# osmr/pytorchcv

Hardware: AMD Instinct MI355X
Metric: images/sec @224x224 (resnet50 bs=256/GPU) (higher is better)
Workload: dtype bf16; 1 GPU; resnet50_bs256; per_gpu_batch=256, global_batch=256, input=fp32 NCHW 224x224 resident in HBM, parallelism=batch-sharded replicas x1, launcher_choice=timed at capture on this GPU

## Files before the change

### include/pcv_amd.h

```cpp
#ifndef PCV_AMD_H
#define PCV_AMD_H

#include <stddef.h>
#include <stdint.h>

#ifdef __cplusplus
extern "C" {
#endif

#define PCV_ABI_VERSION 5

typedef struct pcv_ctx pcv_ctx;

typedef enum pcv_status {
    PCV_OK = 0,
    PCV_ERR_INVALID = -1,
    PCV_ERR_HIP = -2,
    PCV_ERR_NO_DEVICE = -3,
    PCV_ERR_TOO_LARGE = -4
} pcv_status;

typedef enum pcv_dtype { PCV_F32 = 0, PCV_BF16 = 1, PCV_F16 = 2 } pcv_dtype;

typedef enum pcv_act {
    PCV_ACT_NONE = 0, PCV_ACT_RELU = 1, PCV_ACT_RELU6 = 2, PCV_ACT_SIGMOID = 3,
    PCV_ACT_SWISH = 4, PCV_ACT_HSIGMOID = 5, PCV_ACT_HSWISH = 6, PCV_ACT_CLAMP01 = 7
} pcv_act;

typedef struct pcv_conv_desc {
    int32_t struct_size;
    int32_t N, H, W;
    int32_t Cin, Cout;
    int32_t kh, kw;
    int32_t stride_h, stride_w;
    int32_t pad_t, pad_l, pad_b, pad_r;
    int32_t dil_h, dil_w;
    int32_t groups;
    int32_t act;
    int32_t post_act;
    int32_t has_residual;
    int32_t dtype;
    int32_t out_dtype;
    int32_t x_cpitch;
    int32_t x_wpitch;
    int32_t y_cpitch;
} pcv_conv_desc;

int pcv_abi_version(void);
size_t pcv_conv_desc_size(void);
int pcv_create(pcv_ctx** out, int device);
int pcv_destroy(pcv_ctx* ctx);
const char* pcv_last_error(const pcv_ctx* ctx);
int pcv_set_tuning(pcv_ctx* ctx, const char* key, int value);

int pcv_fp16_guard_begin(pcv_ctx* ctx, unsigned* slot, void* stream);
int pcv_fp16_guard_end(pcv_ctx* ctx, const unsigned* slot, float* y, long count, void* stream);
int pcv_fp16_overflow_count(pcv_ctx* ctx, unsigned* count, void* stream);

int pcv_nchw_to_nhwc(pcv_ctx* ctx, const float* x, void* y, int N, int C, int H, int W,
                     int cpitch, int wpitch, int dtype, void* stream);
int pcv_nhwc_to_nchw(pcv_ctx* ctx, const void* x, float* y, int N, int C, int H, int W, int cpitch, int dtype,
                     void* stream);

int pcv_preprocess_u8(pcv_ctx* ctx, const unsigned char* x, void* y, int N, int Hs, int Ws, int C, int top, int left,
                      int H, int W, int wpitch, const float* mean, const float* inv_std, int dtype, void* stream);

int pcv_resize_plan_bytes(int N, const int* hs, const int* ws, int C, int size, int H, int W, size_t* bytes);
int pcv_resize_plan(const void* const* frames, int N, const int* hs, const int* ws, int C, int size, int H, int W, void* blob,
                    size_t bytes);
int pcv_resize_crop_u8(pcv_ctx* ctx, const void* plan_host, const void* plan_dev, size_t bytes, void* y, int wpitch,
                       const float* mean, const float* inv_std, int dtype, void* stream);

int pcv_classify_f32(pcv_ctx* ctx, const float* logits, int N, int J, int k,
                     int* top_idx, float* top_val, float* top_prob,
                     const long long* labels, int* rank, float* nll,
                     void* stream);

int pcv_conv_packed_bytes(const pcv_conv_desc* d, size_t* bytes);
int pcv_conv_pack(pcv_ctx* ctx, const pcv_conv_desc* d, const float* w, void* packed, void* stream);
int pcv_dwconv_packed_bytes(const pcv_conv_desc* d, size_t* bytes);
int pcv_dwconv_pack(pcv_ctx* ctx, const pcv_conv_desc* d, const float* w, void* packed, void* stream);
int pcv_bn_fold(pcv_ctx* ctx, int C, const float* gamma, const float* beta, const float* mean, const float* var,
                float eps, const float* conv_bias, float* scale, float* shift, void* stream);

int pcv_conv2d_fused(pcv_ctx* ctx, const pcv_conv_desc* d, const void* x, const void* packed,
                     const float* scale, const float* shift, const void* residual, void* y, void* stream);

int pcv_conv2d_gated_fused(pcv_ctx* ctx, const pcv_conv_desc* d, const void* x, const void* packed, const float* scale,
                           const float* shift, const float* gate, const void* residual, void* y, void* stream);
int pcv_fc_f32(pcv_ctx* ctx, const float* in, const float* w, const float* b, float* out, int N, int K, int J, int act,
               void* stream);
int pcv_conv2d_maxpool_supported(const pcv_conv_desc* d, int k, int s, int p, int ceil_mode);
int pcv_conv2d_maxpool_fused(pcv_ctx* ctx, const pcv_conv_desc* d, const void* x, const void* packed, const float* scale,
                             const float* shift, void* y, int k, int s, int p, int ceil_mode, void* stream);

int pcv_conv2d_nchw_stem_supported(const pcv_conv_desc* d, int pool);
int pcv_conv2d_nchw_stem_fused(pcv_ctx* ctx, const pcv_conv_desc* d, const float* x_nchw, const void* packed, const float* scale,
                               const float* shift, void* y, int pool, void* stream);
int pcv_dwconv2d_fused(pcv_ctx* ctx, const pcv_conv_desc* d, const void* x, const void* packed,
                       const float* scale, const float* shift, const void* residual, void* y, void* stream);
int pcv_mixconv_packed_bytes(const pcv_conv_desc* d, const int* kernels, int nk, size_t* bytes);
int pcv_mixconv_pack(pcv_ctx* ctx, const pcv_conv_desc* d, const int* kernels, int nk, const float* const* w, void* packed,
                     void* stream);
int pcv_mixconv2d_fused(pcv_ctx* ctx, const pcv_conv_desc* d, const int* kernels, int nk, const void* x, const void* packed,
                        const float* scale, const float* shift, void* y, void* stream);
int pcv_ghost_supported(const pcv_conv_desc* d);
int pcv_ghost_dw_fused(pcv_ctx* ctx, const pcv_conv_desc* d, const void* m, const void* packed, const float* scale,
                       const float* shift, const void* residual, void* y, void* stream);
int pcv_gconvx_supported(const pcv_conv_desc* d);
int pcv_maxpool2d(pcv_ctx* ctx, const void* x, void* y, int N, int H, int W, int C, int k, int s, int p,
                  int ceil_mode, int dtype, void* stream);
int pcv_channel_slice(pcv_ctx* ctx, const void* x, void* y, long rows, int C, int offset, int x_cpitch, int y_cpitch,
                      int dtype, void* stream);
int pcv_channel_interleave2(pcv_ctx* ctx, const void* a, const void* b, void* y, long rows, int Ch, int a_cpitch,
                            int b_cpitch, int y_cpitch, int dtype, void* stream);
int pcv_channel_concat(pcv_ctx* ctx, const void* x, void* y, long rows, int C, int x_cpitch, int y_cpitch, int y_offset,
                       int dtype, void* stream);
int pcv_interpolate(pcv_ctx* ctx, const void* x, void* y, int N, int H, int W, int C, int Ho, int Wo, int bilinear,
                    int align_corners, int dtype, void* stream);
int pcv_hr_fuse_supported(int nsrc, const int* shift, int N, int H, int W, int C, int act, int dtype);
int pcv_hr_fuse(pcv_ctx* ctx, const void* const* src, const int* shift, int nsrc, void* y, int N, int H, int W, int C, int act,
                int dtype, void* stream);
int pcv_avgpool2d(pcv_ctx* ctx, const void* x, void* y, int N, int H, int W, int C, int k, int s,
                  int dtype, int out_dtype, void* stream);
int pcv_global_avgpool(pcv_ctx* ctx, const void* x, void* y, int N, int HW, int C, int dtype, int out_dtype,
                       void* stream);
int pcv_gemm_bias(pcv_ctx* ctx, const void* x, const void* packed, const float* bias, void* y,
                  int N, int Cin, int Cout, int dtype, int out_dtype, void* stream);
int pcv_se_squeeze(pcv_ctx* ctx, const void* x, float* mean, int N, int HW, int C, int dtype, void* stream);
int pcv_se_excite(pcv_ctx* ctx, const float* mean, const float* w1, const float* b1, const float* w2,
                  const float* b2, float* mid, float* gate, int N, int C, int M, int mid_act, int out_act,
                  void* stream);
int pcv_se_scale(pcv_ctx* ctx, const void* x, const float* gate, const void* residual, void* y,
                 int N, int HW, int C, int post_act, int dtype, void* stream);

int pcv_splat_squeeze(pcv_ctx* ctx, const void* x, float* s, int N, int HW, int C, int radix, int dtype, void* stream);
int pcv_splat_excite(pcv_ctx* ctx, const float* s, const float* w1, const float* b1, const float* w2, const float* b2, float* mid,
                     float* logits, float* att, int N, int C, int M, int radix, int groups, void* stream);
int pcv_splat_combine(pcv_ctx* ctx, const void* x, const float* att, const void* residual, void* y, int N, int HW, int C, int radix,
                      int post_act, int dtype, void* stream);
int pcv_avgpool2d_pad(pcv_ctx* ctx, const void* x, void* y, int N, int H, int W, int C, int k, int s, int p, int ceil_mode,
                      int count_include_pad, int dtype, int out_dtype, void* stream);

int pcv_cbam_pool(pcv_ctx* ctx, const void* x, float* s, int N, int HW, int C, int dtype, void* stream);
int pcv_cbam_excite(pcv_ctx* ctx, const float* s, const float* w1, const float* b1, const float* w2, const float* b2, float* mid,
                    float* gate, int N, int C, int M, void* stream);
int pcv_cbam_spatial_pool(pcv_ctx* ctx, const void* x, const float* gate, float* p, int N, int HW, int C, int dtype, void* stream);
int pcv_cbam_apply(pcv_ctx* ctx, const void* x, const float* gate, const float* p, const float* w7, const float* scale,
                   const float* shift, const void* residual, void* y, int N, int H, int W, int C, int post_act, int dtype,
                   void* stream);

int pcv_conv1x1_pair_supported(const pcv_conv_desc* d1, const pcv_conv_desc* d2);
int pcv_conv1x1_pair_fused(pcv_ctx* ctx, const pcv_conv_desc* d1, const pcv_conv_desc* d2, const void* x,
                           const void* packed1, const float* scale1, const float* shift1, const void* residual, void* y1,
                           const void* packed2, const float* scale2, const float* shift2, void* y2, void* stream);

int pcv_conv1x1_pair_gated_supported(const pcv_conv_desc* d1, const pcv_conv_desc* d2);
int pcv_conv1x1_pair_gated_fused(pcv_ctx* ctx, const pcv_conv_desc* d1, const pcv_conv_desc* d2, const void* x,
                                 const void* packed1, const float* scale1, const float* shift1, const float* gate,
                                 const void* residual, void* y1, const void* packed2, const float* scale2, const float* shift2,
                                 void* y2, void* stream);

int pcv_conv1x1_pair_idconv_supported(const pcv_conv_desc* d_id, const pcv_conv_desc* d1, const pcv_conv_desc* d2);
int pcv_conv1x1_pair_idconv_fused(pcv_ctx* ctx, const pcv_conv_desc* d_id, const pcv_conv_desc* d1, const pcv_conv_desc* d2,
                                  const void* x0, const void* packed_id, const float* scale_id, const float* shift_id,
                                  const void* x, const void* packed1, const float* scale1, const float* shift1, void* y1,
                                  const void* packed2, const float* scale2, const float* shift2, void* y2, void* stream);

int pcv_bottleneck_supported(const pcv_conv_desc* d1, const pcv_conv_desc* d2, const pcv_conv_desc* d3, const pcv_conv_desc* d_id);
int pcv_bottleneck_fused(pcv_ctx* ctx, const pcv_conv_desc* d1, const pcv_conv_desc* d2, const pcv_conv_desc* d3,
                         const pcv_conv_desc* d_id, const void* x, const void* packed1, const float* scale1, const float* shift1,
                         const void* packed2, const float* scale2, const float* shift2, const void* packed3, const float* scale3,
                         const float* shift3, const void* packed_id, const float* scale_id, const float* shift_id, void* y,
                         void* stream);

int pcv_mbconv_supported(const pcv_conv_desc* d_exp, const pcv_conv_desc* d_dw, const pcv_conv_desc* d_proj);
int pcv_mbconv_fused(pcv_ctx* ctx, const pcv_conv_desc* d_exp, const pcv_conv_desc* d_dw, const pcv_conv_desc* d_proj,
                     const void* x, const void* packed_exp, const float* scale_e, const float* shift_e,
                     const void* packed_dw, const float* scale_d, const float* shift_d, const void* packed_proj,
                     const float* scale_p, const float* shift_p, const void* residual, void* y, void* stream);

int pcv_bn_act(pcv_ctx* ctx, const void* x, const float* scale, const float* shift, void* y, long rows, int C,
               int x_cpitch, int act, int dtype, void* stream);

int pcv_instnorm_workspace_bytes(int N, int Cn, size_t* bytes);
int pcv_instnorm_act(pcv_ctx* ctx, const void* x, const float* gamma, const float* beta, void* y, void* workspace, int N, int HW,
                     int C, int Cn, int x_cpitch, float eps, int act, int dtype, void* stream);

int pcv_rccl_available(void);
int pcv_rccl_broadcast(pcv_ctx* ctx, void* comm, void* const* bufs, const size_t* bytes, int count, int root, void* stream);
int pcv_rccl_allgather(pcv_ctx* ctx, void* comm, const void* send, void* recv, size_t bytes_per_rank, void* stream);

#ifdef __cplusplus
}
#endif
#endif
```

### pytorchcv_amd/_lib.py

```python

__all__ = ['lib', 'ctx_for', 'check', 'ConvDesc', 'LIB_PATH', 'PcvError', 'PCV_ERR_TOO_LARGE']

import os
import ctypes
import threading

LIB_PATH = os.path.join(os.path.dirname(os.path.abspath(__file__)), "csrc", "libpcv_amd.so")
PCV_ERR_TOO_LARGE = -4

_c = ctypes
_VP = ctypes.c_void_p
_I = ctypes.c_int


class PcvError(RuntimeError):
    def __init__(self, code, msg):
        super(PcvError, self).__init__("pcv_amd error {}: {}".format(code, msg))
        self.code = code


PCV_ABI_VERSION = 5


class ConvDesc(ctypes.Structure):
    _fields_ = [(n, ctypes.c_int32) for n in (
        "struct_size", "N", "H", "W", "Cin", "Cout", "kh", "kw", "stride_h", "stride_w", "pad_t", "pad_l", "pad_b", "pad_r",
        "dil_h", "dil_w", "groups", "act", "post_act", "has_residual", "dtype", "out_dtype", "x_cpitch", "x_wpitch",
        "y_cpitch")]


    def __init__(self, *args, **kw):
        super(ConvDesc, self).__init__(*args, **kw)
        self.struct_size = ctypes.sizeof(ConvDesc)


_SIGS = {
    "pcv_abi_version": (_I, []),
    "pcv_conv_desc_size": (ctypes.c_size_t, []),
    "pcv_create": (_I, [ctypes.POINTER(_VP), _I]),
    "pcv_destroy": (_I, [_VP]),
    "pcv_last_error": (ctypes.c_char_p, [_VP]),
    "pcv_set_tuning": (_I, [_VP, ctypes.c_char_p, _I]),
    "pcv_fp16_guard_begin": (_I, [_VP, _VP, _VP]),
    "pcv_fp16_guard_end": (_I, [_VP, _VP, _VP, ctypes.c_long, _VP]),
    "pcv_fp16_overflow_count": (_I, [_VP, ctypes.POINTER(ctypes.c_uint), _VP]),
    "pcv_rccl_available": (_I, []),
    "pcv_rccl_broadcast": (_I, [_VP, _VP, ctypes.POINTER(_VP), ctypes.POINTER(ctypes.c_size_t), _I, _I, _VP]),
    "pcv_rccl_allgather": (_I, [_VP, _VP, _VP, _VP, ctypes.c_size_t, _VP]),
    "pcv_nchw_to_nhwc": (_I, [_VP, _VP, _VP, _I, _I, _I, _I, _I, _I, _I, _VP]),
    "pcv_nhwc_to_nchw": (_I, [_VP, _VP, _VP, _I, _I, _I, _I, _I, _I, _VP]),
    "pcv_preprocess_u8": (_I, [_VP, _VP, _VP, _I, _I, _I, _I, _I, _I, _I, _I, _I, _VP, _VP, _I, _VP]),
    "pcv_resize_plan_bytes": (_I, [_I, ctypes.POINTER(_I), ctypes.POINTER(_I), _I, _I, _I, _I, ctypes.POINTER(ctypes.c_size_t)]),
    "pcv_resize_plan": (_I, [ctypes.POINTER(_VP), _I, ctypes.POINTER(_I), ctypes.POINTER(_I), _I, _I, _I, _I, _VP, ctypes.c_size_t]),
    "pcv_resize_crop_u8": (_I, [_VP, _VP, _VP, ctypes.c_size_t, _VP, _I, _VP, _VP, _I, _VP]),
    "pcv_classify_f32": (_I, [_VP, _VP, _I, _I, _I, _VP, _VP, _VP, _VP, _VP, _VP, _VP]),
    "pcv_conv_packed_bytes": (_I, [ctypes.POINTER(ConvDesc), ctypes.POINTER(ctypes.c_size_t)]),
    "pcv_conv_pack": (_I, [_VP, ctypes.POINTER(ConvDesc), _VP, _VP, _VP]),
    "pcv_dwconv_packed_bytes": (_I, [ctypes.POINTER(ConvDesc), ctypes.POINTER(ctypes.c_size_t)]),
    "pcv_dwconv_pack": (_I, [_VP, ctypes.POINTER(ConvDesc), _VP, _VP, _VP]),
    "pcv_bn_fold": (_I, [_VP, _I, _VP, _VP, _VP, _VP, ctypes.c_float, _VP, _VP, _VP, _VP]),
    "pcv_conv2d_fused": (_I, [_VP, ctypes.POINTER(ConvDesc), _VP, _VP, _VP, _VP, _VP, _VP, _VP]),
    "pcv_dwconv2d_fused": (_I, [_VP, ctypes.POINTER(ConvDesc), _VP, _VP, _VP, _VP, _VP, _VP, _VP]),
    "pcv_mixconv_packed_bytes": (_I, [ctypes.POINTER(ConvDesc), ctypes.POINTER(_I), _I, ctypes.POINTER(ctypes.c_size_t)]),
    "pcv_mixconv_pack": (_I, [_VP, ctypes.POINTER(ConvDesc), ctypes.POINTER(_I), _I, ctypes.POINTER(_VP), _VP, _VP]),
    "pcv_mixconv2d_fused": (_I, [_VP, ctypes.POINTER(ConvDesc), ctypes.POINTER(_I), _I, _VP, _VP, _VP, _VP, _VP, _VP]),
    "pcv_ghost_supported": (_I, [ctypes.POINTER(ConvDesc)]),
    "pcv_ghost_dw_fused": (_I, [_VP, ctypes.POINTER(ConvDesc), _VP, _VP, _VP, _VP, _VP, _VP, _VP]),
    "pcv_gconvx_supported": (_I, [ctypes.POINTER(ConvDesc)]),
    "pcv_hr_fuse_supported": (_I, [_I, ctypes.POINTER(_I), _I, _I, _I, _I, _I, _I]),
    "pcv_hr_fuse": (_I, [_VP, ctypes.POINTER(_VP), ctypes.POINTER(_I), _I, _VP, _I, _I, _I, _I, _I, _I, _VP]),
    "pcv_maxpool2d": (_I, [_VP, _VP, _VP, _I, _I, _I, _I, _I, _I, _I, _I, _I, _VP]),
    "pcv_channel_slice": (_I, [_VP, _VP, _VP, ctypes.c_long, _I, _I, _I, _I, _I, _VP]),
    "pcv_channel_interleave2": (_I, [_VP, _VP, _VP, _VP, ctypes.c_long, _I, _I, _I, _I, _I, _VP]),
    "pcv_channel_concat": (_I, [_VP, _VP, _VP, ctypes.c_long, _I, _I, _I, _I, _I, _VP]),
    "pcv_interpolate": (_I, [_VP, _VP, _VP, _I, _I, _I, _I, _I, _I, _I, _I, _I, _VP]),
    "pcv_avgpool2d": (_I, [_VP, _VP, _VP, _I, _I, _I, _I, _I, _I, _I, _I, _VP]),
    "pcv_global_avgpool": (_I, [_VP, _VP, _VP, _I, _I, _I, _I, _I, _VP]),
    "pcv_gemm_bias": (_I, [_VP, _VP, _VP, _VP, _VP, _I, _I, _I, _I, _I, _VP]),
    "pcv_se_squeeze": (_I, [_VP, _VP, _VP, _I, _I, _I, _I, _VP]),
    "pcv_se_excite": (_I, [_VP, _VP, _VP, _VP, _VP, _VP, _VP, _VP, _I, _I, _I, _I, _I, _VP]),
    "pcv_conv2d_gated_fused": (_I, [_VP, ctypes.POINTER(ConvDesc), _VP, _VP, _VP, _VP, _VP, _VP, _VP, _VP]),
    "pcv_fc_f32": (_I, [_VP, _VP, _VP, _VP, _VP, _I, _I, _I, _I, _VP]),
    "pcv_conv2d_maxpool_supported": (_I, [ctypes.POINTER(ConvDesc), _I, _I, _I, _I]),
    "pcv_conv2d_maxpool_fused": (_I, [_VP, ctypes.POINTER(ConvDesc), _VP, _VP, _VP, _VP, _VP, _I, _I, _I, _I, _VP]),
    "pcv_conv2d_nchw_stem_supported": (_I, [ctypes.POINTER(ConvDesc), _I]),
    "pcv_conv2d_nchw_stem_fused": (_I, [_VP, ctypes.POINTER(ConvDesc), _VP, _VP, _VP, _VP, _VP, _I, _VP]),
    "pcv_conv1x1_pair_supported": (_I, [ctypes.POINTER(ConvDesc), ctypes.POINTER(ConvDesc)]),
    "pcv_conv1x1_pair_fused": (_I, [_VP, ctypes.POINTER(ConvDesc), ctypes.POINTER(ConvDesc), _VP, _VP, _VP, _VP, _VP, _VP, _VP,
                                    _VP, _VP, _VP, _VP]),
    "pcv_conv1x1_pair_gated_supported": (_I, [ctypes.POINTER(ConvDesc), ctypes.POINTER(ConvDesc)]),
    "pcv_conv1x1_pair_gated_fused": (_I, [_VP, ctypes.POINTER(ConvDesc), ctypes.POINTER(ConvDesc), _VP, _VP, _VP, _VP, _VP, _VP, _VP,
                                          _VP, _VP, _VP, _VP, _VP]),
    "pcv_conv1x1_pair_idconv_supported": (_I, [ctypes.POINTER(ConvDesc), ctypes.POINTER(ConvDesc), ctypes.POINTER(ConvDesc)]),
    "pcv_conv1x1_pair_idconv_fused": (_I, [_VP, ctypes.POINTER(ConvDesc), ctypes.POINTER(ConvDesc), ctypes.POINTER(ConvDesc),
                                           _VP, _VP, _VP, _VP, _VP, _VP, _VP, _VP, _VP, _VP, _VP, _VP, _VP, _VP]),
    "pcv_bottleneck_supported": (_I, [ctypes.POINTER(ConvDesc), ctypes.POINTER(ConvDesc), ctypes.POINTER(ConvDesc), ctypes.POINTER(ConvDesc)]),
    "pcv_bottleneck_fused": (_I, [_VP, ctypes.POINTER(ConvDesc), ctypes.POINTER(ConvDesc), ctypes.POINTER(ConvDesc), ctypes.POINTER(ConvDesc),
                                  _VP, _VP, _VP, _VP, _VP, _VP, _VP, _VP, _VP, _VP, _VP, _VP, _VP, _VP, _VP]),
    "pcv_mbconv_supported": (_I, [ctypes.POINTER(ConvDesc), ctypes.POINTER(ConvDesc), ctypes.POINTER(ConvDesc)]),
    "pcv_mbconv_fused": (_I, [_VP, ctypes.POINTER(ConvDesc), ctypes.POINTER(ConvDesc), ctypes.POINTER(ConvDesc), _VP, _VP, _VP, _VP,
                              _VP, _VP, _VP, _VP, _VP, _VP, _VP, _VP, _VP]),
    "pcv_bn_act": (_I, [_VP, _VP, _VP, _VP, _VP, ctypes.c_long, _I, _I, _I, _I, _VP]),
    "pcv_instnorm_workspace_bytes": (_I, [_I, _I, ctypes.POINTER(ctypes.c_size_t)]),
    "pcv_instnorm_act": (_I, [_VP, _VP, _VP, _VP, _VP, _VP, _I, _I, _I, _I, _I, ctypes.c_float, _I, _I, _VP]),
    "pcv_se_scale": (_I, [_VP, _VP, _VP, _VP, _VP, _I, _I, _I, _I, _I, _VP]),
    "pcv_splat_squeeze": (_I, [_VP, _VP, _VP, _I, _I, _I, _I, _I, _VP]),
    "pcv_splat_excite": (_I, [_VP, _VP, _VP, _VP, _VP, _VP, _VP, _VP, _VP, _I, _I, _I, _I, _I, _VP]),
    "pcv_splat_combine": (_I, [_VP, _VP, _VP, _VP, _VP, _I, _I, _I, _I, _I, _I, _VP]),
    "pcv_avgpool2d_pad": (_I, [_VP, _VP, _VP, _I, _I, _I, _I, _I, _I, _I, _I, _I, _I, _I, _VP]),
    "pcv_cbam_pool": (_I, [_VP, _VP, _VP, _I, _I, _I, _I, _VP]),
    "pcv_cbam_excite": (_I, [_VP, _VP, _VP, _VP, _VP, _VP, _VP, _VP, _I, _I, _I, _VP]),
    "pcv_cbam_spatial_pool": (_I, [_VP, _VP, _VP, _VP, _I, _I, _I, _I, _VP]),
    "pcv_cbam_apply": (_I, [_VP, _VP, _VP, _VP, _VP, _VP, _VP, _VP, _VP, _I, _I, _I, _I, _I, _I, _VP]),
}

_lib = None
_ctxs = {}
_lock = threading.RLock()


def lib():
    global _lib
    if _lib is None:
        with _lock:
            if _lib is None:
                if not os.path.exists(LIB_PATH):
                    raise RuntimeError(
                        "pytorchcv_amd: HIP extension {} is missing - build it with `python -c 'import __graft_entry__ as g; "
                        "g.build()'` or `make -C pytorchcv_amd/csrc`. There is no CPU fallback.".format(LIB_PATH))
                L = ctypes.CDLL(LIB_PATH)
                for name, (res, args) in _SIGS.items():
                    fn = getattr(L, name)
                    fn.restype = res
                    fn.argtypes = args
                if L.pcv_abi_version() != PCV_ABI_VERSION or L.pcv_conv_desc_size() != ctypes.sizeof(ConvDesc):
                    raise RuntimeError("pytorchcv_amd: {} has ABI version {} / a {}-byte pcv_conv_desc, this binding expects "
                                       "version {} / {} bytes - rebuild the library".format(
                                           LIB_PATH, L.pcv_abi_version(), L.pcv_conv_desc_size(), PCV_ABI_VERSION,
                                           ctypes.sizeof(ConvDesc)))
                _lib = L
    return _lib


def exported_symbols():
    return sorted(_SIGS.keys())


def ctx_for(device_index: int):
    c = _ctxs.get(device_index)
    if c is None:
        with _lock:
            c = _ctxs.get(device_index)
            if c is None:
                L = lib()
                h = _VP()
                rc = L.pcv_create(ctypes.byref(h), int(device_index))
                if rc != 0:
                    raise PcvError(rc, (L.pcv_last_error(None) or b"").decode())
                c = h
                _ctxs[device_index] = c
    return c


def check(rc: int, ctx):
    if rc != 0:
        raise PcvError(rc, (lib().pcv_last_error(ctx) or b"").decode())
```

### pytorchcv_amd/csrc/conv_device.hpp

```cpp
#pragma once
#include "pcv_common.hpp"

struct D3Params {
    const void* x;
    const void* w;
    const void* res;
    void* y;
    const float* scale;
    const float* shift;
    uint32_t x_bytes, w_bytes, y_bytes, res_bytes;
    int M;
    int Cout, Ypitch;
    int H, W, Cin, HW;
    FastDiv div_hw, div_w;
    int nk;
    int slices;
    int Kpad;
    int act, post_act;
    int nChTiles, nTiles;
    uint32_t* dbg;
    int stride, Hin, Win;
    uint32_t* ovf;
    int tailN;
    int dbgflags;
};

#if defined(__HIP_DEVICE_COMPILE__)
struct D3Tiles {
    int tile0, tend, tstride, nMine;
};
__device__ __forceinline__ D3Tiles d3q_tiles(const D3Params& p) {
    D3Tiles t;
    const int perXcd = (p.nTiles + 7) >> 3;
    const int xcd = blockIdx.x & 7;
    t.tstride = gridDim.x >> 3;
    t.tile0 = xcd * perXcd + (int)(blockIdx.x >> 3);
    t.tend = min(p.nTiles, (xcd + 1) * perXcd);
    t.nMine = t.tile0 < t.tend ? (t.tend - t.tile0 + t.tstride - 1) / t.tstride : 0;
    return t;
}
__device__ __forceinline__ void d3q_sync() {
    __builtin_amdgcn_sched_barrier(0);
    __builtin_amdgcn_s_barrier();
    __builtin_amdgcn_sched_barrier(0);
}

struct EpiBounds {
    float alo, ahi, plo, phi, clo, chi;
};
__device__ __forceinline__ EpiBounds make_epi_bounds(int act, int post_act) {
    EpiBounds b;
    b.alo = (act == PCV_ACT_RELU || act == PCV_ACT_RELU6) ? 0.f : -INFINITY;
    b.ahi = act == PCV_ACT_RELU6 ? 6.f : INFINITY;
    b.plo = (post_act == PCV_ACT_RELU || post_act == PCV_ACT_RELU6) ? 0.f : -INFINITY;
    b.phi = post_act == PCV_ACT_RELU6 ? 6.f : INFINITY;
    b.clo = b.alo > b.plo ? b.alo : b.plo;
    b.chi = b.ahi < b.phi ? b.ahi : b.phi;
    return b;
}
__device__ __forceinline__ float clamp_nan(float v, float lo, float hi) {
    return __builtin_elementwise_minimum(__builtin_elementwise_maximum(v, lo), hi);
}
template <typename F> __device__ __forceinline__ void epi_dispatch(bool has_res, bool relu_only, F&& f) {
    if (has_res) { if (relu_only) f(std::true_type{}, std::true_type{}); else f(std::true_type{}, std::false_type{}); }
    else { if (relu_only) f(std::false_type{}, std::true_type{}); else f(std::false_type{}, std::false_type{}); }
}

template <int DT, bool HR, bool RO>
__device__ __forceinline__ uint32_t epi2(float v0, float v1, uint32_t skip, const EpiBounds& b, F16Guard<DT>& guard) {
    if constexpr (RO) {
        if constexpr (HR) {
            float lo, hi;
            unpack2<DT>(skip, lo, hi);
            v0 += lo;
            v1 += hi;
        }
        v0 = __builtin_elementwise_maximum(v0, 0.f);
        v1 = __builtin_elementwise_maximum(v1, 0.f);
    } else if constexpr (HR) {
        v0 = clamp_nan(v0, b.alo, b.ahi);
        v1 = clamp_nan(v1, b.alo, b.ahi);
        float lo, hi;
        unpack2<DT>(skip, lo, hi);
        v0 += lo;
        v1 += hi;
        v0 = clamp_nan(v0, b.plo, b.phi);
        v1 = clamp_nan(v1, b.plo, b.phi);
    } else {
        v0 = clamp_nan(v0, b.clo, b.chi);
        v1 = clamp_nan(v1, b.clo, b.chi);
    }
    guard.see2(v0, v1);
    return pack2<DT>(v0, v1);
}

__device__ __forceinline__ void load_bn8(const D3Params& p, int chl, f32x4& s0, f32x4& s1, f32x4& h0, f32x4& h1) {
    s0 = *reinterpret_cast<const f32x4*>(p.scale + chl); s1 = *reinterpret_cast<const f32x4*>(p.scale + chl + 4);
    h0 = *reinterpret_cast<const f32x4*>(p.shift + chl); h1 = *reinterpret_cast<const f32x4*>(p.shift + chl + 4);
}

template <int ROWS> __device__ __forceinline__ void d3r_tile_pos(const D3Params& p, int tilesPerImage, int t, int& chTile, int& n, int& y0) {
    chTile = t % p.nChTiles;
    const int pt = t / p.nChTiles;
    n = pt / tilesPerImage;
    y0 = (pt - n * tilesPerImage) * ROWS;
}
#endif
```

### pytorchcv_amd/csrc/p1r_16bit.hip

```cpp
#include "p1r_conv.hpp"
#define P1R_INST(CW, CIN)                                                   \
    template __global__ void p1r_kernel<PCV_BF16, CW, CIN>(const D3Params); \
    template __global__ void p1r_kernel<PCV_F16, CW, CIN>(const D3Params);
P1R_INST(64, 256)
P1R_INST(32, 512)
P1R_INST(32, 256)
```

### pytorchcv_amd/csrc/p1r_conv.hpp

```cpp
#pragma once
#include "conv_device.hpp"

template <int CW_, int CIN_>
struct P1RCfg {
    static constexpr int CW = CW_;
    static constexpr int CIN = CIN_;
    static constexpr int CWB = CW / 16;
    static constexpr int KH = CIN / 32;
    static constexpr int AREGS = CWB * KH * 4;
    static constexpr int NW = 8;
    static constexpr int THREADS = 64 * NW;
    static constexpr int CG = NW * CW;
    static constexpr int BM = CG;
    static constexpr int UNITB = 16 * CIN * 2;
    static constexpr int SLOT = 65536;
    static constexpr int TP = SLOT / UNITB;
    static constexpr int BP = 16 * TP;
    static constexpr int PPU = CIN / 32;
    static constexpr int NPW = 64 / NW;
    static constexpr int SSOFF = 2 * SLOT;
    static constexpr int LDS = SSOFF + 2 * CG * 4;
    static constexpr int NSTEP = TP * KH;
    static constexpr int NSTORE = TP * (CWB / 2);
    static constexpr bool RES = CW == 32;
    static_assert((CW == 64 && CIN == 256) || (CW == 32 && CIN == 512) || (CW == 32 && CIN == 256), "three configurations");
    static_assert(NSTEP == 64 && TP * PPU == 64 && PPU % NW == 0 && KH % NPW == 0, "tile geometry");
};

#if defined(__HIP_DEVICE_COMPILE__)
template <int DT, int CW, int CIN>
__device__ __forceinline__ void p1r_body(const D3Params& p, char* smem) {
    typedef P1RCfg<CW, CIN> G;
    typedef typename Mma<DT>::frag frag;
    typedef __attribute__((address_space(3))) char lds_char;
    typedef const __attribute__((address_space(3))) frag* lds_fptr;
    constexpr int KH = G::KH, CWB = G::CWB, TP = G::TP;
    const int lane = threadIdx.x & 63;
    const int wave = __builtin_amdgcn_readfirstlane(threadIdx.x >> 6);
    const int fr = lane & 15, fq = lane >> 4;
    const int lrow = lane >> 3;
    const uint32_t lds0 = (uint32_t)__builtin_amdgcn_readfirstlane((int)(uint32_t)(size_t)PCV_LDS(smem));
    const D3Tiles T = d3q_tiles(p);
    if (T.nMine == 0) return;
#ifdef P1R_CYCLES
    const uint64_t cstart__ = __builtin_amdgcn_s_memtime();
#endif

    const __amdgpu_buffer_rsrc_t wrsrc = buffer_rsrc(p.w, p.w_bytes);
    const __amdgpu_buffer_rsrc_t xrsrc = buffer_rsrc(p.x, p.x_bytes);
    const __amdgpu_buffer_rsrc_t yrsrc = buffer_rsrc(p.y, p.y_bytes);
    const bool has_res = p.res != nullptr;
    const __amdgpu_buffer_rsrc_t rrsrc = buffer_rsrc(p.res, has_res ? p.res_bytes : 0u);

    frag A[KH][CWB];
    const uint32_t ssaddr = lds0 + (uint32_t)(G::SSOFF + (wave * CW + 8 * fq) * 4);
    auto load_weights = [&](int cg) __attribute__((always_inline)) {
#pragma unroll
        for (int kh = 0; kh < KH; ++kh)
#pragma unroll
            for (int i = 0; i < CWB; ++i) {
                const uint32_t row = (uint32_t)(cg * G::CG + wave * CW + i * 16 + fr);
                const uint32_t off = (row * (uint32_t)p.Kpad + (uint32_t)((kh >> 1) * 64 + (fq + 4 * (kh & 1)) * 8)) * 2u;
                const u32x4 v = __builtin_amdgcn_raw_buffer_load_b128(wrsrc, off, 0, 0);
                A[kh][i] = __builtin_bit_cast(frag, v);
            }
        if (lane < CW) {
            const int ch = cg * G::CG + wave * CW + lane;
            const float sc = ch < p.Cout ? p.scale[ch] : 0.f, sh = ch < p.Cout ? p.shift[ch] : 0.f;
            *reinterpret_cast<__attribute__((address_space(3))) float*>((size_t)(lds0 + (uint32_t)(G::SSOFF + (wave * CW + lane) * 4))) = sc;
            *reinterpret_cast<__attribute__((address_space(3))) float*>((size_t)(lds0 + (uint32_t)(G::SSOFF + (G::CG + wave * CW + lane) * 4))) = sh;
        }
    };

    const uint32_t fbase = lds0 + (uint32_t)(fr * 128 + ((fq ^ (fr & 7)) << 4));

    const int half8 = wave & 1;
    const uint32_t lanesrc = (uint32_t)((((lane & 7) ^ lrow) << 4));
    int tileP0N = 0;
    bool moreN = false;
    bool pseudoN = false;
    uint32_t pixoff = 0x80000000u;
    auto unit_src = [&](int unit) __attribute__((always_inline)) {
        const int m = tileP0N + unit * 16 + half8 * 8 + lrow;
        uint32_t mi = (uint32_t)m;
        if (p.stride != 1) {
            const uint32_t n = fastdiv((uint32_t)m, p.div_hw);
            const uint32_t rem = (uint32_t)m - n * (uint32_t)p.HW;
            const uint32_t ho = fastdiv(rem, p.div_w);
            const uint32_t wo = rem - ho * (uint32_t)p.W;
            mi = (n * (uint32_t)p.Hin + ho * (uint32_t)p.stride) * (uint32_t)p.Win + wo * (uint32_t)p.stride;
        }
        pixoff = (moreN && m < p.M && !(pseudoN && unit > 0)) ? mi * (uint32_t)(G::CIN * 2) + lanesrc : 0x80000000u;
    };
    auto dma_piece = [&](auto Ic, int slot) __attribute__((always_inline)) {
        constexpr int I = decltype(Ic)::value;
        constexpr int unit = (G::NW * I) / G::PPU, in0 = (G::NW * I) % G::PPU;
        constexpr int sl0 = in0 / 2;
        if constexpr (in0 == 0) unit_src(unit);
        const int slice = (wave >> 1) + sl0;
        const uint32_t dst = lds0 + (uint32_t)(slot * G::SLOT + unit * G::UNITB + slice * 2048 + half8 * 1024);
        __builtin_amdgcn_raw_ptr_buffer_load_lds(xrsrc, (lds_char*)(size_t)dst, 16, pixoff, slice * 128, 0, 0);
    };

    constexpr int RD = 3, RING = 6, KEEP = RING - RD - 1, NSTEP = G::NSTEP;
    f32x4 cacc[2][CWB];
    frag bq[RING];
    uint32_t fs0 = 0, fs1 = 0;
    auto rd = [&](auto STc) __attribute__((always_inline)) {
        constexpr int st = decltype(STc)::value;
        constexpr int u = st / KH, kh = st - KH * u, s = kh >> 1, h = kh & 1;
        bq[st % RING] = *reinterpret_cast<lds_fptr>((size_t)(h ? fs1 : fs0) + (size_t)(u * G::UNITB + s * 2048));
    };
    const EpiBounds B = make_epi_bounds(p.act, p.post_act);
    constexpr int NRR = G::RES ? TP * (CWB / 2) : 1;
    u32x4 rrq[NRR];
    u32x4 opend;
    f32x4 scA, shA, scB, shB;
    typedef const __attribute__((address_space(3))) f32x4* lds_f4ptr;
    auto ss_read = [&](auto IPc, auto Hc) __attribute__((always_inline)) {
        constexpr int ip = decltype(IPc)::value, half = decltype(Hc)::value;
        const f32x4 a = *reinterpret_cast<lds_f4ptr>((size_t)ssaddr + (size_t)((ip * 32 + 4 * half) * 4));
        const f32x4 b = *reinterpret_cast<lds_f4ptr>((size_t)ssaddr + (size_t)((G::CG + ip * 32 + 4 * half) * 4));
        if constexpr (half == 0) { scA = a; shA = b; } else { scB = a; shB = b; }
        __builtin_amdgcn_sched_barrier(0);
    };
    auto epi_part = [&](auto Mc, auto Uc, auto Pc, F16Guard<DT>& guard) __attribute__((always_inline)) {
        constexpr int MODE = decltype(Mc)::value;
        constexpr bool HR = (MODE & 1) != 0, PRE = (MODE & 2) != 0, HI = (MODE & 4) != 0;
        constexpr int u = decltype(Uc)::value, P = decltype(Pc)::value;
        constexpr int ip = P >> 2, e = P & 3, half = e >> 1, k0 = 2 * (e & 1);
        const f32x4& scv = half == 0 ? scA : scB;
        const f32x4& shv = half == 0 ? shA : shB;
        const f32x4& c = cacc[u & 1][2 * ip + half];
        f32x2 v = (f32x2){c[k0], c[k0 + 1]} * (f32x2){scv[k0], scv[k0 + 1]} + (f32x2){shv[k0], shv[k0 + 1]};
        if constexpr (HR) {
            if constexpr (PRE) {
                v[0] = __builtin_elementwise_maximum(v[0], B.alo); v[1] = __builtin_elementwise_maximum(v[1], B.alo);
                if constexpr (HI) { v[0] = __builtin_elementwise_minimum(v[0], B.ahi); v[1] = __builtin_elementwise_minimum(v[1], B.ahi); }
            }
            float lo, hi;
            unpack2<DT>(rrq[(u * (CWB / 2) + ip) % NRR][e], lo, hi);
            v += (f32x2){lo, hi};
            v[0] = __builtin_elementwise_maximum(v[0], B.plo); v[1] = __builtin_elementwise_maximum(v[1], B.plo);
            if constexpr (HI) { v[0] = __builtin_elementwise_minimum(v[0], B.phi); v[1] = __builtin_elementwise_minimum(v[1], B.phi); }
        } else {
            v[0] = __builtin_elementwise_maximum(v[0], B.clo); v[1] = __builtin_elementwise_maximum(v[1], B.clo);
            if constexpr (HI) { v[0] = __builtin_elementwise_minimum(v[0], B.chi); v[1] = __builtin_elementwise_minimum(v[1], B.chi); }
        }
        guard.see2(v[0], v[1]);
        opend[e] = pack2<DT>(v[0], v[1]);
    };
    uint32_t yb[CWB / 2], rb[CWB / 2];
    auto epi_store = [&](int u, int ip) __attribute__((always_inline)) {
        __builtin_amdgcn_raw_buffer_store_b128(opend, yrsrc, yb[ip] + (uint32_t)(u * 32 * p.Ypitch), 0, 0);
    };
    auto tile_steps = [&](auto HRc, auto ONEc, int slot, int ch0, int mTile) __attribute__((always_inline)) {
        constexpr bool ONE = decltype(ONEc)::value;
        constexpr bool HR = (decltype(HRc)::value & 1) != 0;
        F16Guard<DT> guard;
#pragma unroll
        for (int ip = 0; ip < CWB / 2; ++ip) {
            const bool chok = ch0 + 32 * ip < p.Cout;
            yb[ip] = chok ? (uint32_t)(((mTile + fr) * p.Ypitch + ch0 + 32 * ip) * 2) : 0x80000000u;
            if constexpr (HR) rb[ip] = chok ? (uint32_t)(((mTile + fr) * p.Cout + ch0 + 32 * ip) * 2) : 0x80000000u;
        }
        if constexpr (HR) {
#pragma unroll
            for (int u = 0; u < (ONE ? 1 : TP); ++u)
#pragma unroll
                for (int ip = 0; ip < CWB / 2; ++ip) {
                    rrq[(u * (CWB / 2) + ip) % NRR] = __builtin_amdgcn_raw_buffer_load_b128(rrsrc, rb[ip] + (uint32_t)(u * 32 * p.Cout), 0, 0);
                }
        }
        rd(std::integral_constant<int, 0>{}); rd(std::integral_constant<int, 1>{}); rd(std::integral_constant<int, 2>{});
        static_assert(RD == 3, "the three reads above");
        auto step = [&](auto STc) __attribute__((always_inline)) {
            constexpr int st = decltype(STc)::value;
            constexpr int u = st / KH, kh = st - KH * u;
            if constexpr (st + RD < NSTEP) rd(std::integral_constant<int, st + RD>{});
            if constexpr (u == 0 && (kh % (KH / G::NPW)) == 0) dma_piece(std::integral_constant<int, kh / (KH / G::NPW)>{}, slot ^ 1);
#pragma unroll
            for (int i = 0; i < CWB; ++i) {
                if constexpr (kh == 0) cacc[u & 1][i] = Mma<DT>::run(A[0][i], bq[st % RING], (f32x4){0.f, 0.f, 0.f, 0.f});
                else cacc[u & 1][i] = Mma<DT>::run(A[kh][i], bq[st % RING], cacc[u & 1][i]);
            }
            if constexpr (st >= KEEP) asm volatile("" ::"v"(bq[(st - KEEP) % RING]), "v"(cacc[u & 1][CWB - 1]));
            if constexpr (u >= 1) {
                typedef std::integral_constant<int, u - 1> UP;
                typedef std::integral_constant<int, 0> I0;
                typedef std::integral_constant<int, 1> I1;
                auto part = [&](auto Pc) __attribute__((always_inline)) { epi_part(HRc, UP{}, Pc, guard); };
                typedef std::integral_constant<int, 2> I2; typedef std::integral_constant<int, 3> I3; typedef std::integral_constant<int, 4> I4;
                typedef std::integral_constant<int, 5> I5; typedef std::integral_constant<int, 6> I6; typedef std::integral_constant<int, 7> I7;
                if constexpr (CWB == 4 && KH == 8) {
                    if constexpr (kh == 0) { ss_read(I0{}, I0{}); ss_read(I0{}, I1{}); }
                    if constexpr (kh == 2) { part(I0{}); part(I1{}); ss_read(I1{}, I0{}); }
                    if constexpr (kh == 3) { part(I2{}); part(I3{}); ss_read(I1{}, I1{}); epi_store(u - 1, 0); }
                    if constexpr (kh == 5) { part(I4{}); part(I5{}); }
                    if constexpr (kh == 6) { part(I6{}); part(I7{}); }
                    if constexpr (kh == 7) epi_store(u - 1, 1);
                } else if constexpr (KH == 8) {
                    if constexpr (kh == 0) { ss_read(I0{}, I0{}); ss_read(I0{}, I1{}); }
                    if constexpr (kh == 2) part(I0{});
                    if constexpr (kh == 3) part(I1{});
                    if constexpr (kh == 5) part(I2{});
                    if constexpr (kh == 6) part(I3{});
                    if constexpr (kh == 7) epi_store(u - 1, 0);
                } else {
                    if constexpr (kh == 0) { ss_read(I0{}, I0{}); ss_read(I0{}, I1{}); }
                    if constexpr (kh == 3) part(I0{});
                    if constexpr (kh == 5) part(I1{});
                    if constexpr (kh == 8) part(I2{});
                    if constexpr (kh == 10) part(I3{});
                    if constexpr (kh == 12) epi_store(u - 1, 0);
                }
            }
        };
        auto run = [&](auto... Sc) __attribute__((always_inline)) { (step(Sc), ...); };
        auto eight = [&](auto Bc) __attribute__((always_inline)) {
            constexpr int B0 = decltype(Bc)::value * 8;
            run(std::integral_constant<int, B0>{}, std::integral_constant<int, B0 + 1>{}, std::integral_constant<int, B0 + 2>{},
                std::integral_constant<int, B0 + 3>{}, std::integral_constant<int, B0 + 4>{}, std::integral_constant<int, B0 + 5>{},
                std::integral_constant<int, B0 + 6>{}, std::integral_constant<int, B0 + 7>{});
        };
        auto last_epilogue = [&](auto ULc) __attribute__((always_inline)) {
            typedef decltype(ULc) UL;
            constexpr int ul = UL::value;
            ss_read(std::integral_constant<int, 0>{}, std::integral_constant<int, 0>{}); ss_read(std::integral_constant<int, 0>{}, std::integral_constant<int, 1>{});
            epi_part(HRc, UL{}, std::integral_constant<int, 0>{}, guard); epi_part(HRc, UL{}, std::integral_constant<int, 1>{}, guard);
            epi_part(HRc, UL{}, std::integral_constant<int, 2>{}, guard); epi_part(HRc, UL{}, std::integral_constant<int, 3>{}, guard);
            epi_store(ul, 0);
            if constexpr (CWB == 4) {
                ss_read(std::integral_constant<int, 1>{}, std::integral_constant<int, 0>{}); ss_read(std::integral_constant<int, 1>{}, std::integral_constant<int, 1>{});
                epi_part(HRc, UL{}, std::integral_constant<int, 4>{}, guard); epi_part(HRc, UL{}, std::integral_constant<int, 5>{}, guard);
                epi_part(HRc, UL{}, std::integral_constant<int, 6>{}, guard); epi_part(HRc, UL{}, std::integral_constant<int, 7>{}, guard);
                epi_store(ul, 1);
            }
        };
        eight(std::integral_constant<int, 0>{});
        if constexpr (KH == 16) eight(std::integral_constant<int, 1>{});
        if constexpr (ONE) last_epilogue(std::integral_constant<int, 0>{});
        else {
            if constexpr (KH == 8) eight(std::integral_constant<int, 1>{});
            eight(std::integral_constant<int, 2>{});
            eight(std::integral_constant<int, 3>{}); eight(std::integral_constant<int, 4>{}); eight(std::integral_constant<int, 5>{});
            eight(std::integral_constant<int, 6>{}); eight(std::integral_constant<int, 7>{});
            last_epilogue(std::integral_constant<int, TP - 1>{});
        }
        guard.commit(p.ovf);
    };

    int cg = T.tile0 % p.nChTiles;
    int tileP0 = (T.tile0 / p.nChTiles) * G::BP;
    tileP0N = tileP0; moreN = true;
    {
        auto all = [&](auto... Ic) __attribute__((always_inline)) { (dma_piece(Ic, 0), ...); };
        auto eight = [&](auto Bc) __attribute__((always_inline)) {
            constexpr int B0 = decltype(Bc)::value;
            all(std::integral_constant<int, B0>{}, std::integral_constant<int, B0 + 1>{}, std::integral_constant<int, B0 + 2>{},
                std::integral_constant<int, B0 + 3>{}, std::integral_constant<int, B0 + 4>{}, std::integral_constant<int, B0 + 5>{},
                std::integral_constant<int, B0 + 6>{}, std::integral_constant<int, B0 + 7>{});
        };
        eight(std::integral_constant<int, 0>{});
    }

    int tailP0 = -1;
    if (p.tailN > 0) {
        const int nCG = p.nChTiles, B = gridDim.x >> 3, j = blockIdx.x >> 3, xcd = blockIdx.x & 7;
        const int r = xcd * (B / nCG) + j / nCG, k = r / TP, u = r - k * TP;
        if (k < p.tailN / nCG) tailP0 = (p.nTiles / nCG + k) * G::BP + 16 * u;
    }
    bool pseudo = false;
    int slot = 0, t = T.tile0;
    while (t < T.tend) {
#ifdef P1R_CYCLES
        const uint64_t p0__ = __builtin_amdgcn_s_memtime();
#endif
        load_weights(cg);
#ifdef P1R_CYCLES
        const uint64_t p1__ = __builtin_amdgcn_s_memtime();
#endif
        __builtin_amdgcn_s_waitcnt(0x0070);
#ifdef P1R_CYCLES
        const uint64_t p2__ = __builtin_amdgcn_s_memtime();
#endif
        d3q_sync();
#ifdef P1R_CYCLES
        if (p.dbg != nullptr && t == T.tile0 && lane == 0 && wave == 0) {
            uint32_t* e = p.dbg + 256 * 8 * 4 + blockIdx.x * 32 + 30;
            e[0] = (uint32_t)(p0__ - cstart__) | ((uint32_t)(p1__ - p0__) << 16);
            e[1] = (uint32_t)(p2__ - p1__) | ((uint32_t)(__builtin_amdgcn_s_memtime() - p2__) << 16);
        }
#endif
        bool same;
        do {
            const int tn = t + T.tstride;
            moreN = tn < T.tend;
            int cgN = moreN ? tn % p.nChTiles : cg;
            tileP0N = moreN ? (tn / p.nChTiles) * G::BP : 0;
            pseudoN = !moreN && !pseudo && tailP0 >= 0;
            if (pseudoN) { moreN = true; cgN = cg; tileP0N = tailP0; }
            fs0 = fbase + (uint32_t)(slot * G::SLOT);
            fs1 = fs0 ^ 64u;
#ifdef P1R_CYCLES
            const bool stamp__ = p.dbg != nullptr;
            const int tl__ = (t - T.tile0) / T.tstride;
            uint64_t c0__ = 0, c1__ = 0, c2__ = 0;
            if (stamp__) c0__ = __builtin_amdgcn_s_memtime();
#endif
            {
                const int ch0 = cg * G::CG + wave * CW + 8 * fq;
                const bool hi = p.act == PCV_ACT_RELU6 || p.post_act == PCV_ACT_RELU6, pre = p.act != PCV_ACT_NONE;
                auto modes = [&](auto ONEc) __attribute__((always_inline)) {
                    if constexpr (G::RES) {
                        if (has_res) {
                            if (!hi && !pre) tile_steps(std::integral_constant<int, 1>{}, ONEc, slot, ch0, tileP0);
                            else tile_steps(std::integral_constant<int, 7>{}, ONEc, slot, ch0, tileP0);
                        } else if (!hi) tile_steps(std::integral_constant<int, 0>{}, ONEc, slot, ch0, tileP0);
                        else tile_steps(std::integral_constant<int, 4>{}, ONEc, slot, ch0, tileP0);
                    } else {
                        if (!hi) tile_steps(std::integral_constant<int, 0>{}, ONEc, slot, ch0, tileP0);
                        else tile_steps(std::integral_constant<int, 4>{}, ONEc, slot, ch0, tileP0);
                    }
                };
                if (pseudo) modes(std::true_type{});
                else modes(std::false_type{});
            }
#ifdef P1R_CYCLES
            if (stamp__) c1__ = __builtin_amdgcn_s_memtime();
#endif
            if constexpr (G::NSTORE == 16) asm volatile("s_waitcnt vmcnt(16)" ::: "memory");
            else if constexpr (G::NSTORE == 8) asm volatile("s_waitcnt vmcnt(8)" ::: "memory");
            else asm volatile("s_waitcnt vmcnt(4)" ::: "memory");
#ifdef P1R_CYCLES
            if (stamp__) c2__ = __builtin_amdgcn_s_memtime();
#endif
            d3q_sync();
#ifdef P1R_CYCLES
            if (stamp__ && lane == 0) {
                const uint64_t c3 = __builtin_amdgcn_s_memtime();
                if (tl__ == 2) {
                    uint32_t* d = p.dbg + (blockIdx.x * 8 + wave) * 4;
                    d[0] = (uint32_t)(c1__ - c0__); d[1] = (uint32_t)(c2__ - c1__); d[2] = (uint32_t)(c3 - c2__); d[3] = 1u;
                }
                if (wave == 0 && tl__ < 15) {
                    uint32_t* e = p.dbg + 256 * 8 * 4 + blockIdx.x * 32 + 2 * tl__;
                    e[0] = (uint32_t)(c0__ - cstart__); e[1] = (uint32_t)(c3 - c0__);
                }
            }
#endif
            same = moreN && cgN == cg;
            cg = cgN; tileP0 = tileP0N;
            pseudo = pseudoN;
            slot ^= 1;
            t = tn;
        } while (same);
    }
    asm volatile("s_waitcnt vmcnt(0)" ::: "memory");
}
#endif

template <int DT, int CW, int CIN>
__global__ __launch_bounds__((P1RCfg<CW, CIN>::THREADS), 1) void p1r_kernel(const D3Params p) {
#if defined(__HIP_DEVICE_COMPILE__)
    extern __shared__ __attribute__((aligned(16))) char smem[];
    p1r_body<DT, CW, CIN>(p, smem);
#endif
}
```

### pytorchcv_amd/csrc/pcv_api.hip

```cpp
#include <hip/hip_runtime.h>
#include <string>
#include <type_traits>
#include <vector>
#include <cstring>
#include <algorithm>
#include <cstdio>
#include <cstdlib>
#include <dlfcn.h>
#include "pcv_common.hpp"
#include "igemm_inst.hpp"
#include "d3q_inst.hpp"
#include "d3w_inst.hpp"
#include "d3c_conv.hpp"
#include "d3k_conv.hpp"
#include "d3i_conv.hpp"
#include "d1i_conv.hpp"
#include "p1r_conv.hpp"
#include "stem_conv.hpp"
#include "pair1x1.hpp"
#include "wpair1x1.hpp"
#include "bnu.hpp"
#include "gconv3x3.hpp"
#include "gconv3x3r.hpp"
#include "gconvx.hpp"
GCONVX_INSTANCES(GCONVX_DECLARE, PCV_BF16)
GCONVX_INSTANCES(GCONVX_DECLARE, PCV_F16)
#include "mbconv.hpp"
#include "mbw_inst.hpp"
#include "mbr_inst.hpp"
MBW_SHAPES(MBW_DECLARE, PCV_BF16)
MBW_SHAPES(MBW_DECLARE, PCV_F16)
MBW2_SHAPES(MBW2_DECLARE, PCV_BF16)
MBW2_SHAPES(MBW2_DECLARE, PCV_F16)
MBW3_SHAPES(MBW3_DECLARE, PCV_BF16)
MBW3_SHAPES(MBW3_DECLARE, PCV_F16)
MBR_SHAPES(MBR_DECLARE, PCV_BF16)
MBR_SHAPES(MBR_DECLARE, PCV_F16)
#include "dwconv.hpp"
#include "mixconv.hpp"
MIX_INSTANCES(MIX_DECLARE, PCV_F32)
MIX_INSTANCES(MIX_DECLARE, PCV_BF16)
MIX_INSTANCES(MIX_DECLARE, PCV_F16)
#include "ghost.hpp"
GHOST_INSTANCES(GHOST_DECLARE, PCV_F32)
GHOST_INSTANCES(GHOST_DECLARE, PCV_BF16)
GHOST_INSTANCES(GHOST_DECLARE, PCV_F16)
#include "aux_kernels.hpp"
#include "cbam_kernels.hpp"
#include "instnorm.hpp"
#include "hrfuse.hpp"
#include "resize_kernel.hpp"
#include "classify_kernel.hpp"
#include "head_gemm.hpp"


IGEMM_INSTANCES(IGEMM_DECLARE, PCV_BF16)
IGEMM_INSTANCES(IGEMM_DECLARE, PCV_F16)
IGEMM_INSTANCES_SAMETYPE(IGEMM_DECLARE, PCV_F32)
D3Q_SHAPES(D3Q_DECLARE, PCV_BF16)
D3Q_SHAPES(D3Q_DECLARE, PCV_F16)
D3Q1_SHAPES(D3Q1_DECLARE, PCV_BF16)
D3Q1_SHAPES(D3Q1_DECLARE, PCV_F16)
D3W_SHAPES(D3W_DECLARE, PCV_BF16)
D3W_SHAPES(D3W_DECLARE, PCV_F16)
D3WT_SHAPES(D3WT_DECLARE, PCV_BF16)
D3WT_SHAPES(D3WT_DECLARE, PCV_F16)
extern template __global__ void d3c_kernel<PCV_BF16>(const D3Params);
extern template __global__ void d3c_kernel<PCV_F16>(const D3Params);
extern template __global__ void d3k_kernel<PCV_BF16>(const D3Params);
extern template __global__ void d3k_kernel<PCV_F16>(const D3Params);
extern template __global__ void d3i_kernel<PCV_BF16, 256>(const D3Params);
extern template __global__ void d3i_kernel<PCV_F16, 256>(const D3Params);
extern template __global__ void d3i_kernel<PCV_BF16, 512>(const D3Params);
extern template __global__ void d3i_kernel<PCV_F16, 512>(const D3Params);
extern template __global__ void d1i_kernel<PCV_BF16, 1024>(const D3Params);
extern template __global__ void d1i_kernel<PCV_F16, 1024>(const D3Params);
extern template __global__ void d1i_kernel<PCV_BF16, 2048>(const D3Params);
extern template __global__ void d1i_kernel<PCV_F16, 2048>(const D3Params);
#define P1R_DECLARE(CW, CIN)                                                       \
    extern template __global__ void p1r_kernel<PCV_BF16, CW, CIN>(const D3Params); \
    extern template __global__ void p1r_kernel<PCV_F16, CW, CIN>(const D3Params);
P1R_DECLARE(64, 256)
P1R_DECLARE(32, 512)
P1R_DECLARE(32, 256)
#define BNU_DECLARE(DT)                                                          \
    extern template __global__ void bnu_kernel<DT, false>(const BnuParams);      \
    extern template __global__ void bnu_kernel<DT, true>(const BnuParams);
BNU_DECLARE(PCV_BF16)
BNU_DECLARE(PCV_F16)

enum TileCfg { TILE_C32 = 0, TILE_C64 = 1, TILE_C128 = 2, TILE_C256 = 3, TILE_C64S = 4, TILE_C128S = 5, TILE_COUNT = 6 };

struct pcv_ctx {
    int device = 0;
    std::string err;
    int num_cu = 256;
    int persist_mode = 1;
    int force_tile = -1;
    int use_wstat = 1;
    int use_mbr = 1;
    int use_mbr_xl = 1;
    int use_mbw = 1;
    int use_gconvr = 1;
    int use_gconvx = 1;
    int use_d1x1 = -1;
    int use_head = 1;
    int use_stem32 = 1;
    int use_d3x3 = -1;
    unsigned long long dbg_ptr = 0;
    int use_p1r = -1;
    int use_d3k = -1;
    int use_d3i = -1;
    int use_d1i = -1;
    int use_d3c = -1;
    int use_d3w = -1;
    int dbg_flags = 0;
    int dw_flags = 0;
    int dw_th = 0;
    int max_blocks = 0;
    int bnu_band = 0;
    int pair_pb = 2;
    int persist_max_nk = 4;
    uint32_t* ovf = nullptr;
    int igemm_bpc[3][2][TILE_COUNT][3] = {};
    int gconv_bpc[3] = {2, 2, 2};
    int gconvx_bpc[2] = {2, 2};
    int stem_bpc[2] = {1, 1};
    int pair_bpc[2] = {1, 1};
    int pair_idc_bpc = 1;
    int wpair_bpc[4] = {1, 1, 1, 1};
};

static thread_local std::string g_create_err;

static int fail(pcv_ctx* ctx, int code, const std::string& msg) {
    if (ctx) ctx->err = msg; else g_create_err = msg;
    return code;
}
#define HIP_TRY(ctx, expr)                                                                          \
    do {                                                                                            \
        hipError_t e__ = (expr);                                                                    \
        if (e__ != hipSuccess)                                                                      \
            return fail(ctx, PCV_ERR_HIP, std::string(#expr) + ": " + hipGetErrorString(e__));      \
    } while (0)

struct DeviceGuard {
    int prev = -1;
    bool switched = false;
    explicit DeviceGuard(int want) {
        if (hipGetDevice(&prev) == hipSuccess && prev != want) switched = hipSetDevice(want) == hipSuccess;
    }
    ~DeviceGuard() {
        if (switched) (void)hipSetDevice(prev);
    }
};

#define PCV_ENTER(ctx)                       \
    if (!(ctx)) return PCV_ERR_INVALID;      \
    DeviceGuard device_guard((ctx)->device)
static int launched(pcv_ctx* ctx) {
    HIP_TRY(ctx, hipGetLastError());
    return PCV_OK;
}

static inline int round_up(int v, int m) { return (v + m - 1) / m * m; }
static inline long long cap_blocks(const pcv_ctx* ctx, long long blocks) {
    return (ctx->max_blocks > 0 && blocks > ctx->max_blocks) ? ctx->max_blocks : blocks;
}
static inline long long block_slots(const pcv_ctx* ctx, int per_cu) { return cap_blocks(ctx, (long long)ctx->num_cu * per_cu); }
static inline int esize(int dt) { return dt == PCV_F32 ? 4 : 2; }
static inline bool dtype_ok(int dt) { return dt == PCV_F32 || dt == PCV_BF16 || dt == PCV_F16; }
static inline bool aligned16(const void* p) { return (reinterpret_cast<uintptr_t>(p) & 15u) == 0; }
static inline bool in_window(unsigned long long bytes) { return bytes < 0x80000000ull; }
static int too_large(pcv_ctx* ctx, const char* fn, const char* what) {
    return fail(ctx, PCV_ERR_TOO_LARGE, std::string(fn) + ": " + what + " exceeds the 2 GiB window of one launch; split the batch");
}
static const char* const kTensorTooLarge = "tensor exceeds the 2 GiB window";
static int flat_grid(pcv_ctx* ctx, const char* fn, long long total, unsigned* grid, int per_block = 256) {
    const long long blocks = (total + per_block - 1) / per_block;
    if (total < 0 || blocks > 0x7fffffffll) return too_large(ctx, fn, "the grid");
    *grid = (unsigned)blocks;
    return PCV_OK;
}
static int stream_grid(pcv_ctx* ctx, const char* fn, long long total, unsigned* grid) {
    if (int rc = flat_grid(ctx, fn, total, grid)) return rc;
    *grid = (unsigned)cap_blocks(ctx, *grid);
    return PCV_OK;
}
template <int V> using dtype_tag = std::integral_constant<int, V>;
#define DT_OF(tag) decltype(tag)::value
template <class F> static void for_dtype(int dt, F&& f) {
    if (dt == PCV_BF16) f(dtype_tag<PCV_BF16>{});
    else if (dt == PCV_F16) f(dtype_tag<PCV_F16>{});
    else f(dtype_tag<PCV_F32>{});
}
template <class F> static void for_dtype16(int dt, F&& f) {
    if (dt == PCV_BF16) f(dtype_tag<PCV_BF16>{});
    else f(dtype_tag<PCV_F16>{});
}
template <class F> static void for_dtype_out(int dt, int ot, F&& f) {
    for_dtype(dt, [&](auto T) {
        if (ot == PCV_F32) f(T, dtype_tag<PCV_F32>{});
        else f(T, T);
    });
}

struct Kernel { const void* fn; int threads, lds, BM, BP; };
template <class F> static Kernel kernel_of(F* fn, int threads, int lds, int BM = 0, int BP = 0) {
    return Kernel{reinterpret_cast<const void*>(fn), threads, lds, BM, BP};
}
template <class Params> static int launch(pcv_ctx* ctx, const Kernel& k, unsigned grid, hipStream_t stream, Params& q) {
    void* args[] = {&q};
    HIP_TRY(ctx, hipLaunchKernel(k.fn, dim3(grid), dim3((unsigned)k.threads), args, (size_t)k.lds, stream));
    return PCV_OK;
}
static int blocks_per_cu(pcv_ctx* ctx, const Kernel& k, int* nb) {
    HIP_TRY(ctx, hipOccupancyMaxActiveBlocksPerMultiprocessor(nb, k.fn, k.threads, k.lds));
    if (*nb < 1) *nb = 1;
    return PCV_OK;
}

struct ConvPlan {
    bool stem = false;
    bool conv3 = false;
    int ES = 2, CE = 8;
    bool pair = false;
    int Ho = 0, Wo = 0;
    int ngb = 1;
    int Cg_in = 0, Cg_out = 0;
    int cin_blk = 0, cout_blk = 0;
    int nR = 1, nQ = 1;
    int dy[IGEMM_MAX_TAPS], dx[IGEMM_MAX_TAPS];
    int nchunks = 0, nk = 0, Kpad = 0;
    int wrows = 0;
// ... 178 lines not shown
                                P.ksrc[(size_t)j * P.CE + e] = (uint32_t)c | ((uint32_t)(r * d.kw + q) << 16);
                        }
                        put(cc * P.CE, r, q, P.dy[r], P.dx[q]);
                    }
        }
        while (j < P.nk * 8) put(0, 15, 0, 0, 0);
    }
    return nullptr;
}

struct TileInfo { int BM, BP, threads, lds; };
static const TileInfo kTiles[TILE_COUNT] = {
    {32, 256, 256, 2 * (32 + 256) * 128},
    {64, 256, 256, 2 * (64 + 256) * 128},
    {128, 128, 256, 2 * (128 + 128) * 128},
    {256, 64, 256, 2 * (256 + 64) * 128},
    {64, 128, 256, 2 * (64 + 128) * 128},
    {128, 64, 256, 2 * (128 + 64) * 128},
};
typedef void (*igemm_fn)(const IgemmParams);

template <int DT, int KHW> static igemm_fn igemm_for_tile(int tile) {
    switch (tile) {
        case TILE_C32: return igemm_conv_kernel<DT, DT, 2, 4, 1, 4, false, KHW>;
        case TILE_C64: return igemm_conv_kernel<DT, DT, 4, 4, 1, 4, false, KHW>;
        case TILE_C128: return igemm_conv_kernel<DT, DT, 4, 4, 2, 2, false, KHW>;
        case TILE_C256: return igemm_conv_kernel<DT, DT, 4, 4, 4, 1, false, KHW>;
        case TILE_C64S: if constexpr (KHW == 1) return igemm_conv_kernel<DT, DT, 4, 2, 1, 4, false, 1>; else return nullptr;
        case TILE_C128S: if constexpr (KHW == 1) return igemm_conv_kernel<DT, DT, 4, 2, 2, 2, false, 1>; else return nullptr;
        default: return nullptr;
    }
}
template <int DT> static igemm_fn igemm_for_taps(int tile, int khw) {
    if (khw == 1) return igemm_for_tile<DT, 1>(tile);
    if (khw == 9) return igemm_for_tile<DT, 9>(tile);
    return igemm_for_tile<DT, 0>(tile);
}
static igemm_fn igemm_fn_for(int dt, int ot, bool ragged, int tile, int khw) {
    if (!ragged && ot == dt) {
        if (dt == PCV_BF16) return igemm_for_taps<PCV_BF16>(tile, khw);
        if (dt == PCV_F16) return igemm_for_taps<PCV_F16>(tile, khw);
        return igemm_for_taps<PCV_F32>(tile, khw);
    }
    if (tile != TILE_C128) return nullptr;
    if (ot == PCV_F32) {
        if (dt == PCV_BF16) return igemm_conv_kernel<PCV_BF16, PCV_F32, 4, 4, 2, 2, true, 0>;
        if (dt == PCV_F16) return igemm_conv_kernel<PCV_F16, PCV_F32, 4, 4, 2, 2, true, 0>;
        return igemm_conv_kernel<PCV_F32, PCV_F32, 4, 4, 2, 2, true, 0>;
    }
    if (dt == PCV_BF16) return igemm_conv_kernel<PCV_BF16, PCV_BF16, 4, 4, 2, 2, true, 0>;
    if (dt == PCV_F16) return igemm_conv_kernel<PCV_F16, PCV_F16, 4, 4, 2, 2, true, 0>;
    return nullptr;
}

static Kernel igemm_kernel(int dt, int ot, bool ragged, int tile, int khw) {
    const TileInfo& T = kTiles[tile];
    return kernel_of(igemm_fn_for(dt, ot, ragged, tile, khw), T.threads, T.lds, T.BM, T.BP);
}
static inline int khw_slot(int khw) { return khw == 1 ? 1 : (khw == 9 ? 2 : 0); }

static inline int gconv_slot(int W) { return W + 1 <= 16 ? 0 : (W + 1 <= 32 ? 1 : 2); }
static Kernel gconv_kernel(int dt, int slot) {
    const bool bf = dt == PCV_BF16;
    if (slot == 0) return kernel_of(bf ? gconv3x3_kernel<PCV_BF16, 16> : gconv3x3_kernel<PCV_F16, 16>, 256, GConvCfg<16>::LDS);
    if (slot == 1) return kernel_of(bf ? gconv3x3_kernel<PCV_BF16, 32> : gconv3x3_kernel<PCV_F16, 32>, 256, GConvCfg<32>::LDS);
    return kernel_of(bf ? gconv3x3_kernel<PCV_BF16, 64> : gconv3x3_kernel<PCV_F16, 64>, 256, GConvCfg<64>::LDS);
}
static const int kGconvRMaxLds = 160 * 1024;
static Kernel gconvr_kernel(int dt, int stride, int kt, int lds = kGconvRMaxLds) {
    const bool bf = dt == PCV_BF16;
    if (stride == 2) {
        if (kt == 9) return kernel_of(bf ? gconv3x3r_kernel<PCV_BF16, 2, 9> : gconv3x3r_kernel<PCV_F16, 2, 9>, 256, lds);
        return kernel_of(bf ? gconv3x3r_kernel<PCV_BF16, 2, 5> : gconv3x3r_kernel<PCV_F16, 2, 5>, 256, lds);
    }
    return kernel_of(bf ? gconv3x3r_kernel<PCV_BF16, 1, 9> : gconv3x3r_kernel<PCV_F16, 1, 9>, 256, lds);
}
struct GConvRPlan { int R, XH, xl, win; };
static bool plan_gconvr(int stride, int H, int W, int Ho, int Wo, GConvRPlan& g) {
    if (stride == 2 && ((H | W) & 1)) return false;
    if (Wo > 64 || Ho <= 0) return false;
    for (int R = 64 / Wo; R >= 1; --R) {
        const int win = stride == 2 ? (2 * R + 1) * W + 2 : (R + 2) * W + 2;
        const int XH = stride == 2 ? ((win + 1) / 2 + 7) / 8 * 8 : 0;
        const int rows = ((stride == 2 ? 2 * XH : win) + 31) / 32 * 32;
        const int lds = 2 * rows * 128;
        if (lds * 2 <= kGconvRMaxLds || (R == 1 && lds <= kGconvRMaxLds)) {
            g.R = R; g.XH = XH; g.xl = rows / 32; g.win = win;
            return true;
        }
    }
    return false;
}
#define GCONVX_KROW(DT, S, PB)                                                                                               \
    {kernel_of(gconvx_kernel<DT, S, 8, PB>, 256, kGConvXMaxLds), kernel_of(gconvx_kernel<DT, S, 16, PB>, 256, kGConvXMaxLds),  \
     kernel_of(gconvx_kernel<DT, S, 24, PB>, 256, kGConvXMaxLds), kernel_of(gconvx_kernel<DT, S, 40, PB>, 256, kGConvXMaxLds), \
     kernel_of(gconvx_kernel<DT, S, 48, PB>, 256, kGConvXMaxLds), kernel_of(gconvx_kernel<DT, S, 56, PB>, 256, kGConvXMaxLds), \
     kernel_of(gconvx_kernel<DT, S, 64, PB>, 256, kGConvXMaxLds)}
#define GCONVX_KTYPE(DT) {{GCONVX_KROW(DT, 1, 4), GCONVX_KROW(DT, 1, 7)}, {GCONVX_KROW(DT, 2, 4), GCONVX_KROW(DT, 2, 7)}}
static const Kernel kGConvX[2][2][2][7] = {GCONVX_KTYPE(PCV_BF16), GCONVX_KTYPE(PCV_F16)};
struct GConvXPlan { int R, GB, pbi, win, pitch, lds; };
static bool plan_gconvx(int stride, int H, int W, int Ho, int Wo, int groups, int Cg, GConvXPlan& g) {
    if (stride == 2 && ((H | W) & 1)) return false;
    if (W > 112 || Ho <= 0 || Wo <= 0) return false;
    const int cpg = Cg / 8, sl = (Cg + 15) / 16;
    const int min_gb = std::min(groups, (4 + sl - 1) / sl);
    const int want_gb = std::min(groups, std::max(min_gb, 128 / Cg));
    for (int R = 16 * kGConvXPB[1] / Wo; R >= 1; --R) {
        const int win = stride == 2 ? (2 * R + 1) * W + 2 : (R + 2) * W + 2;
        int p16 = kGConvXMaxLds / (16 * win);
        if (p16 % 2 == 0) --p16;
        const int fit_gb = p16 / cpg;
        if (fit_gb < (R == 1 ? 1 : min_gb)) continue;
        int gb = std::min(want_gb, fit_gb);
        const int ncb = (groups + gb - 1) / gb;
        gb = (groups + ncb - 1) / ncb;
        g.R = R; g.GB = gb; g.pbi = R * Wo <= 16 * kGConvXPB[0] ? 0 : 1; g.win = win;
        g.pitch = 16 * ((gb * cpg) | 1);
        g.lds = win * g.pitch;
        return true;
    }
    return false;
}
template <class Cfg, class F> static Kernel tile_kernel(F* fn, int threads) { return kernel_of(fn, threads, Cfg::LDS, Cfg::BM, Cfg::BP); }
#define D3Q_ROW(DT, WC, WP, CBW, PBW, KS)                                                                   \
    {tile_kernel<D3Cfg<WC, WP, CBW, PBW, KS>>(d3q_kernel<PCV_BF16, WC, WP, CBW, PBW, KS>, 768),             \
     tile_kernel<D3Cfg<WC, WP, CBW, PBW, KS>>(d3q_kernel<PCV_F16, WC, WP, CBW, PBW, KS>, 768)},
static const Kernel kD3[][2] = {D3Q_SHAPES(D3Q_ROW, 0)};
static const int kD3Count = (int)(sizeof(kD3) / sizeof(kD3[0]));
#define D3Q1_ROW(DT, WC, WP, CBW, PBW, KS)                                                                  \
    {tile_kernel<D3Cfg<WC, WP, CBW, PBW, KS, true>>(d3q_kernel<PCV_BF16, WC, WP, CBW, PBW, KS, true>, 768), \
     tile_kernel<D3Cfg<WC, WP, CBW, PBW, KS, true>>(d3q_kernel<PCV_F16, WC, WP, CBW, PBW, KS, true>, 768)},
static const Kernel kD1[][2] = {D3Q1_SHAPES(D3Q1_ROW, 0)};
static const int kD1Count = (int)(sizeof(kD1) / sizeof(kD1[0]));
#define D3W_ROW(DT, WC, WP, CBW, PBW, KS, NSA)                                                              \
    {tile_kernel<D3WCfg<WC, WP, CBW, PBW, KS, NSA>>(d3w_kernel<PCV_BF16, WC, WP, CBW, PBW, KS, NSA>, 512),  \
     tile_kernel<D3WCfg<WC, WP, CBW, PBW, KS, NSA>>(d3w_kernel<PCV_F16, WC, WP, CBW, PBW, KS, NSA>, 512)},
#define D3WT_ROW(DT, WC, WP, CBW, PBW, KS, NSA, TRIM)                                                                   \
    {tile_kernel<D3WCfg<WC, WP, CBW, PBW, KS, NSA, TRIM>>(d3w_kernel<PCV_BF16, WC, WP, CBW, PBW, KS, NSA, TRIM>, 512),  \
     tile_kernel<D3WCfg<WC, WP, CBW, PBW, KS, NSA, TRIM>>(d3w_kernel<PCV_F16, WC, WP, CBW, PBW, KS, NSA, TRIM>, 512)},
static const Kernel kD3W[][2] = {D3W_SHAPES(D3W_ROW, 0) D3WT_SHAPES(D3WT_ROW, 0)};
static const int kD3WCount = (int)(sizeof(kD3W) / sizeof(kD3W[0]));
static const Kernel kD3C[1][2] = {{tile_kernel<D3CCfg>(d3c_kernel<PCV_BF16>, 256), tile_kernel<D3CCfg>(d3c_kernel<PCV_F16>, 256)}};
static const Kernel kD3K[1][2] = {{tile_kernel<D3KCfg>(d3k_kernel<PCV_BF16>, 256), tile_kernel<D3KCfg>(d3k_kernel<PCV_F16>, 256)}};
#define D3I_ROW(CIN)                                                                              \
    {kernel_of(d3i_kernel<PCV_BF16, CIN>, D3ICfg::THREADS, D3ICfgT<CIN>::LDS, D3ICfg::BM),        \
     kernel_of(d3i_kernel<PCV_F16, CIN>, D3ICfg::THREADS, D3ICfgT<CIN>::LDS, D3ICfg::BM)}
static const Kernel kD3I[2][2] = {D3I_ROW(256), D3I_ROW(512)};
static const Kernel kD1I[2][2] = {
    {tile_kernel<D1ICfgT<1024>>(d1i_kernel<PCV_BF16, 1024>, 256), tile_kernel<D1ICfgT<1024>>(d1i_kernel<PCV_F16, 1024>, 256)},
    {tile_kernel<D1ICfgT<1024>>(d1i_kernel<PCV_BF16, 2048>, 256), tile_kernel<D1ICfgT<1024>>(d1i_kernel<PCV_F16, 2048>, 256)}};
#define P1R_ROW(CW, CIN) \
    {tile_kernel<P1RCfg<CW, CIN>>(p1r_kernel<PCV_BF16, CW, CIN>, 512), tile_kernel<P1RCfg<CW, CIN>>(p1r_kernel<PCV_F16, CW, CIN>, 512)}
static const Kernel kP1R[3][2] = {P1R_ROW(64, 256), P1R_ROW(32, 512), P1R_ROW(32, 256)};
static const struct { const Kernel (*rows)[2]; int n; } kD3Tables[] = {{kD3, kD3Count}, {kD1, kD1Count}, {kD3W, kD3WCount}, {kD3C, 1},
                                                                       {kD3K, 1},       {kD3I, 2},       {kD1I, 2},         {kP1R, 3}};
static int pick_d1x1(long long M, int Cout, int Cin, long long slots) {
    if (Cin < 256 || Cout < 128) return -1;
    const int shape = Cout % 256 == 0 ? 1 : 0;
    const long long tiles = (long long)((Cout + kD1[shape][0].BM - 1) / kD1[shape][0].BM) * ((M + kD1[shape][0].BP - 1) / kD1[shape][0].BP);
    return tiles * 2 >= slots ? shape : -1;
}
static int pick_d3x3(long long M, int Cout, int nk, long long slots) {
    (void)nk;
    const int wide = Cout <= 64 ? 2 : 1, narrow = Cout <= 64 ? 5 : 4;
    auto tiles = [&](int i) { return ((Cout + kD3[i][0].BM - 1) / kD3[i][0].BM) * ((M + kD3[i][0].BP - 1) / kD3[i][0].BP); };
    if (Cout % 256 == 0 && tiles(0) * 2 >= slots) return 0;
    if (tiles(wide) * 2 >= slots) return wide;
    if (tiles(narrow) * 4 >= slots) return narrow;
    return -1;
}
static int pick_d3w(long long M, int Cout, long long slots) {
    const int shape = Cout % 256 == 0 ? 1 : (Cout % 128 == 0 ? 2 : -1);
    if (shape < 0) return -1;
    const long long tiles = (long long)(Cout / kD3W[shape][0].BM) * ((M + kD3W[shape][0].BP - 1) / kD3W[shape][0].BP);
    return tiles * 4 >= slots * 3 ? shape : -1;
}

static const int kStemLds = 7 * 64 * 64 + 2 * 768 * 16 + 3 * 2 * 64 * 16;
enum StemForm { STEM_PLAIN = 0, STEM_POOLED = 1, STEM_NARROW = 2 };
#define STEM_ROWS(DT)                                                                                                          \
    {{kernel_of(stem_conv_kernel<DT, false>, 256, kStemLds), kernel_of(stem_conv_kernel<DT, true>, 256, kStemLds),             \
      kernel_of(stem_conv_kernel<DT, false, false, 2>, 256, kStemLds)},                                                        \
     {kernel_of(stem_conv_kernel<DT, false, true>, 256, kStemLds + kStemStageBytes),                                           \
      kernel_of(stem_conv_kernel<DT, true, true>, 256, kStemLds + kStemStageBytes),                                            \
      kernel_of(stem_conv_kernel<DT, false, true, 2>, 256, kStemLds + kStemStageBytes)}}
static const Kernel kStem[2][2][3] = {STEM_ROWS(PCV_BF16), STEM_ROWS(PCV_F16)};

static int pair_lds(int pb, bool idc = false) { return (idc ? 6 : 3) * 16 * pb * 64 * 2 + 16 * 1024 * pb + (idc ? 4096 : 0); }
enum PairForm { PAIR_PB4 = 0, PAIR_PB2 = 1, PAIR_GATED = 2, PAIR_IDCONV = 3 };
#define PAIR_ROW(DT)                                                                                                          \
    {kernel_of(pair1x1_kernel<DT, 4>, 256, pair_lds(4)), kernel_of(pair1x1_kernel<DT, 2>, 256, pair_lds(2)),                  \
     kernel_of(pair1x1_kernel<DT, 2, false, true>, 256, pair_lds(2)), kernel_of(pair1x1_kernel<DT, 2, true>, 256, pair_lds(2, true))}
static const Kernel kPair[2][4] = {PAIR_ROW(PCV_BF16), PAIR_ROW(PCV_F16)};
#define BNU_ROW(DT) {kernel_of(bnu_kernel<DT, false>, 512, BnuCfg<false>::LDS), kernel_of(bnu_kernel<DT, true>, 512, BnuCfg<true>::LDS)}
static const Kernel kBnu[2][2] = {BNU_ROW(PCV_BF16), BNU_ROW(PCV_F16)};
static int g_bnu = -1;
static int g_wpair_mask = 3;
static int g_mbw_wide = 1;
struct WPairLaunch { Kernel k; int tileP; bool gate_in_lds; };
template <int CM, int C1> static WPairLaunch wpair_launch_for(int dt, bool gated) {
    typedef WPairCfg<CM, C1> G;
    const bool bf = dt == PCV_BF16;
    const int lds = gated ? G::LDS_GATED : G::LDS;
    const Kernel k = gated ? kernel_of(bf ? wpair1x1_kernel<PCV_BF16, CM, C1, true> : wpair1x1_kernel<PCV_F16, CM, C1, true>, 64 * G::NW, lds)
                           : kernel_of(bf ? wpair1x1_kernel<PCV_BF16, CM, C1, false> : wpair1x1_kernel<PCV_F16, CM, C1, false>, 64 * G::NW, lds);
    return WPairLaunch{k, G::P, gated && G::GATE_LDS};
}
static WPairLaunch wpair_launch(int cfg, int dt, bool gated = false) {
    switch (cfg) {
        case 0: return wpair_launch_for<128, 512>(dt, gated);
        case 1: return wpair_launch_for<256, 1024>(dt, gated);
        case 2: return wpair_launch_for<128, 256>(dt, gated);
        default: return wpair_launch_for<256, 512>(dt, gated);
    }
}
static int wpair_cfg(int cm, int c1) {
    if (cm == 128 && c1 == 512) return 0;
    if (cm == 256 && c1 == 1024) return 1;
    if (cm == 128 && c1 == 256) return 2;
    if (cm == 256 && c1 == 512) return 3;
    return -1;
}
static bool plain_1x1(const pcv_conv_desc& d) {
    return d.kh == 1 && d.kw == 1 && d.stride_h == 1 && d.stride_w == 1 && d.pad_t == 0 && d.pad_l == 0 && d.pad_b == 0 &&
           d.pad_r == 0 && d.groups == 1 && d.dil_h == 1 && d.dil_w == 1 && d.out_dtype == d.dtype &&
           (d.x_cpitch == 0 || d.x_cpitch == d.Cin) && (d.x_wpitch == 0 || d.x_wpitch == d.W) &&
           (d.y_cpitch == 0 || d.y_cpitch == d.Cout);
}
static const char* pair_unsupported(const pcv_conv_desc& a, const pcv_conv_desc& b) {
    if (desc_stale(a) || desc_stale(b)) return kStaleDesc;
    if (!plain_1x1(a) || !plain_1x1(b)) return "both convolutions must be plain 1x1 stride 1";
    if (a.dtype != b.dtype || (a.dtype != PCV_BF16 && a.dtype != PCV_F16)) return "16-bit storage only";
    if (a.N != b.N || a.H != b.H || a.W != b.W || a.Cout != b.Cin) return "shapes do not chain";
    const bool narrow = a.Cin == 64 && a.Cout == 256 && b.Cout == 64;
    const bool wide = ((a.Cin == 128 && (g_wpair_mask & 1)) || (a.Cin == 256 && (g_wpair_mask & 2))) &&
                      wpair_cfg(a.Cin, a.Cout) >= 0 && b.Cout == a.Cin;
    if (!narrow && !wide) return "only 64 -> 256 -> 64, 128 -> 512|256 -> 128 and 256 -> 1024|512 -> 256 are instantiated";
    if (!a.has_residual || b.has_residual || b.post_act != PCV_ACT_NONE) return "first conv must carry the residual, second must not";
    if ((long)a.N * a.H * a.W * a.Cout * 2 >= (1L << 31)) return kTensorTooLarge;
    return nullptr;
}

typedef void (*mbconv_fn)(const MbParams);
template <int DT> static mbconv_fn mbconv_for(int stride, bool expand) {
    if (stride == 1) return expand ? mbconv_kernel<DT, 1, true> : mbconv_kernel<DT, 1, false>;
    return expand ? mbconv_kernel<DT, 2, true> : mbconv_kernel<DT, 2, false>;
}
static const int kMbMaxLds = 150 * 1024, kMbwMaxLds = 160 * 1024;
static Kernel mbconv_kernel(int dt, int stride, bool expand, int lds = kMbMaxLds) {
    return kernel_of(dt == PCV_BF16 ? mbconv_for<PCV_BF16>(stride, expand) : mbconv_for<PCV_F16>(stride, expand), 256, lds);
}
struct MbwEntry { int dt, s, nrt, act, tw, ka, rb; mbconv_fn fn; };
#define MBW_ROW(DT, S, NRT, ACT, TW) {DT, S, NRT, ACT, TW, 1, 0, mbw_kernel<DT, S, NRT, ACT, TW>},
#define MBW2_ROW(DT, S, NRT, ACT, TW, KA) {DT, S, NRT, ACT, TW, KA, 0, mbw_kernel<DT, S, NRT, ACT, TW, KA>},
#define MBW3_ROW(DT, S, NRT, ACT, TW, KA, RB) {DT, S, NRT, ACT, TW, KA, RB, mbw_kernel<DT, S, NRT, ACT, TW, KA, RB>},
static const MbwEntry kMbw[] = {MBW_SHAPES(MBW_ROW, PCV_BF16) MBW_SHAPES(MBW_ROW, PCV_F16) MBW2_SHAPES(MBW2_ROW, PCV_BF16)
                                MBW2_SHAPES(MBW2_ROW, PCV_F16) MBW3_SHAPES(MBW3_ROW, PCV_BF16) MBW3_SHAPES(MBW3_ROW, PCV_F16)};
static const MbwEntry* pick_mbw(int dt, int stride, int nrt, int act, int tw, int ka, int rb) {
    if (act != PCV_ACT_RELU && act != PCV_ACT_RELU6) act = -1;
    for (const MbwEntry& e : kMbw)
        if (e.dt == dt && e.s == stride && e.nrt == nrt && e.act == act && e.tw == tw && e.ka == ka && e.rb == rb) return &e;
    return nullptr;
}
static Kernel mbw_kernel_of(const MbwEntry& e, int waves = 8, int lds = kMbwMaxLds) { return kernel_of(e.fn, 64 * waves, lds); }
struct MbrEntry { int dt, nrt, act, ro, s, ka; bool afl; int waves; bool wel, xl; mbconv_fn fn; };
#define MBR_ROW(DT, NRT, ACT, RO, S, KA, AFL, WV, WEL, XL) {DT, NRT, ACT, RO, S, KA, AFL, WV, WEL, XL, mbr_kernel<DT, NRT, ACT, RO, S, KA, AFL, WV, WEL, XL>},
static int mbr_entry_lds(const MbrEntry& e, int nChunks) {
    const int nr = e.s == 1 ? e.ro + 2 : 2 * e.ro + 1;
    return mbr_lds_layout(e.nrt, nChunks, e.ka, e.afl, e.wel, e.xl ? nr : 0, e.waves).total;
}
static const MbrEntry kMbr[] = {MBR_SHAPES(MBR_ROW, PCV_BF16) MBR_SHAPES(MBR_ROW, PCV_F16)};
static Kernel mbr_kernel_of(const MbrEntry& e, int lds = kMbwMaxLds) { return kernel_of(e.fn, 64 * e.waves, lds); }
static const MbrEntry* pick_mbr(const pcv_ctx* ctx, int dt, int nrt, int act, int stride, int ka, int nChunks) {
    if (act != PCV_ACT_RELU && act != PCV_ACT_RELU6) return nullptr;
    for (const MbrEntry& e : kMbr)
        if (e.dt == dt && e.nrt == nrt && e.act == act && e.s == stride && e.ka == ka &&
            mbr_entry_lds(e, nChunks) <= kMbwMaxLds && (!e.xl || ctx->use_mbr_xl))
            return &e;
    return nullptr;
}
static int mbw_waves(int stride, int nrt, int nChunks, int tw, int ka, int rb) {
    for (int nw = 8; nw >= 4; nw -= 2)
        if (mbw_lds_layout(stride, nrt, nChunks, nw, tw, ka, rb).total <= kMbwMaxLds) return nw;
    return 0;
}
static MbLds mbconv_plan(int stride, bool expand, int ka, int nChunks, int nRowT, int* nbufX) {
    MbLds two = mb_lds_layout(stride, expand, ka, nChunks, nRowT, 2);
    if (!expand || two.total <= 80 * 1024) { *nbufX = 2; return two; }
    MbLds one = mb_lds_layout(stride, expand, ka, nChunks, nRowT, 1);
    if (one.total <= 80 * 1024 || two.total > kMbMaxLds) { *nbufX = 1; return one; }
    *nbufX = 2;
    return two;
}

static int dt_index(int dtype) { return dtype == PCV_F32 ? 0 : (dtype == PCV_BF16 ? 1 : 2); }

#define DW_TYPE(DT)                                                                                                            \
    {{kernel_of(dwconv_kernel<DT, 3, 1, false>, 256, 0), kernel_of(dwconv_kernel<DT, 3, 1, true>, 256, 0)},                    \
     {kernel_of(dwconv_kernel<DT, 3, 2, false>, 256, 0), kernel_of(dwconv_kernel<DT, 3, 2, true>, 256, 0)},                    \
     {kernel_of(dwconv5_kernel<DT, 1, false>, 256, 0), kernel_of(dwconv5_kernel<DT, 1, true>, 256, 0)},                        \
     {kernel_of(dwconv5_kernel<DT, 2, false>, 256, 0), kernel_of(dwconv5_kernel<DT, 2, true>, 256, 0)}}
static const Kernel kDw[3][4][2] = {DW_TYPE(PCV_F32), DW_TYPE(PCV_BF16), DW_TYPE(PCV_F16)};

#define MIX_KERNEL(DT, S, FAST, G) kernel_of(mixdw_kernel<DT, S, FAST, G>, 256, 0)
#define MIX_ROW(DT, S, FAST) {MIX_KERNEL(DT, S, FAST, 2), MIX_KERNEL(DT, S, FAST, 3), MIX_KERNEL(DT, S, FAST, 4), MIX_KERNEL(DT, S, FAST, 5)}
#define MIX_TYPE(DT) {{MIX_ROW(DT, 1, false), MIX_ROW(DT, 1, true)}, {MIX_ROW(DT, 2, false), MIX_ROW(DT, 2, true)}}
static const Kernel kMix[3][2][2][4] = {MIX_TYPE(PCV_F32), MIX_TYPE(PCV_BF16), MIX_TYPE(PCV_F16)};

// ... 47 lines not shown
        for (int s = 0; s < 2; ++s)
            for (int pbi = 0; pbi < 2; ++pbi)
                for (int wi = 0; wi < 7; ++wi) on(kGConvX[t][s][pbi][wi], (t == 1 && s == 0 && wi == 6) ? &ctx->gconvx_bpc[pbi] : nullptr);
    for (int t = 0; t < 2; ++t)
        for (int nchw = 0; nchw < 2; ++nchw)
            for (int form = 0; form < 3; ++form) on(kStem[t][nchw][form], (nchw == 0 && form == STEM_PLAIN) ? &ctx->stem_bpc[t] : nullptr);
    for (int form = 0; form < 4; ++form) {
        on(kPair[0][form]);
        on(kPair[1][form], form == PAIR_GATED ? nullptr : form == PAIR_IDCONV ? &ctx->pair_idc_bpc : &ctx->pair_bpc[form]);
    }
    for (int t = 0; t < 2; ++t)
        for (int form = 0; form < 2; ++form) on(kBnu[t][form]);
    for (int cfg = 0; cfg < 4; ++cfg)
        for (int gated = 0; gated < 2; ++gated) {
            on(wpair_launch(cfg, PCV_BF16, gated != 0).k);
            on(wpair_launch(cfg, PCV_F16, gated != 0).k, gated ? nullptr : &ctx->wpair_bpc[cfg]);
        }
    for (int dt = PCV_BF16; dt <= PCV_F16; ++dt)
        for (int s = 1; s <= 2; ++s)
            for (int e = 0; e < 2; ++e) on(mbconv_kernel(dt, s, e != 0));
    for (const MbwEntry& e : kMbw) on(mbw_kernel_of(e));
    for (const MbrEntry& e : kMbr) on(mbr_kernel_of(e));
    on(classify_kernel_of(1024));
    on(classify_kernel_of(kClassifyMaxJ));
    return rc;
}
static bool mbw_shape(int Cin, int Cout, int stride, int H, int W, int* ka_out, int* nrt_out, int* rb_out = nullptr) {
    const int ka = (Cin + 31) / 32, nrt = Cout <= 32 ? 2 : (Cout <= 64 ? 4 : 6);
    if (ka_out) *ka_out = ka;
    if (nrt_out) *nrt_out = nrt;
    if (rb_out) *rb_out = nrt == 6 ? 2 : 0;
    if (H > 250 || W > 250 || Cout > 96) return false;
    if (nrt == 6) return g_mbw_wide != 0 && stride == 1 && (ka == 2 || ka == 3);
    return ka == 1 || (ka == 2 && stride == 1 && nrt == 4);
}
static const char* mbconv_unsupported(const pcv_conv_desc* de, const pcv_conv_desc& dd, const pcv_conv_desc& dp) {
    if ((de && desc_stale(*de)) || desc_stale(dd) || desc_stale(dp)) return kStaleDesc;
    if (dd.dtype != PCV_BF16 && dd.dtype != PCV_F16) return "16-bit storage only";
    if (dd.kh != 3 || dd.kw != 3 || dd.dil_h != 1 || dd.dil_w != 1 || dd.pad_t != 1 || dd.pad_l != 1 || dd.pad_b != 1 ||
        dd.pad_r != 1 || dd.stride_h != dd.stride_w || (dd.stride_h != 1 && dd.stride_h != 2) || dd.groups != dd.Cin ||
        dd.Cin != dd.Cout || dd.has_residual || dd.out_dtype != dd.dtype || (dd.x_cpitch != 0 && dd.x_cpitch != dd.Cin) ||
        (dd.x_wpitch != 0 && dd.x_wpitch != dd.W))
        return "depthwise stage must be 3x3, pad 1, stride 1 or 2, no residual";
    const int Cmid = dd.Cin;
    if (Cmid % 8 != 0) return "expanded channels must be a multiple of 8";
    if (!plain_1x1(dp) || dp.dtype != dd.dtype || dp.Cin != Cmid || dp.Cout % 8 != 0 || dp.Cout > 96) return "project stage must be a plain 1x1 with at most 96 channels";
    const bool wave_tiles = de && mbw_shape(de->Cin, dp.Cout, dd.stride_h, dd.H, dd.W, nullptr, nullptr);
    if (dp.Cout > (wave_tiles ? 96 : 32)) return "fused unit only pays for narrow projections";
    const int Ho = (dd.H - 1) / dd.stride_h + 1, Wo = (dd.W - 1) / dd.stride_w + 1;
    if (dp.N != dd.N || dp.H != Ho || dp.W != Wo) return "shapes do not chain";
    if (Wo < (wave_tiles ? 14 : 24) || Ho < 8) return "map too small for the fused unit to pay";
    int ka = 0;
    if (de) {
        if (!plain_1x1(*de) || de->dtype != dd.dtype || de->Cout != Cmid || de->Cin % 8 != 0 || de->has_residual ||
            de->N != dd.N || de->H != dd.H || de->W != dd.W)
            return "expand stage must be a plain 1x1 onto the depthwise input";
        ka = (de->Cin + 31) / 32;
        if (ka > 3) return "expand stage input wider than 96 channels";
    }
    int nbuf = 0;
    if (wave_tiles) {
        if (mbw_waves(dd.stride_h, dp.Cout <= 32 ? 2 : (dp.Cout <= 64 ? 4 : 6), (Cmid + 31) / 32, 16, ka, dp.Cout > 64 ? 2 : 0) == 0)
            return "tiles do not fit the LDS budget";
    } else if (mbconv_plan(dd.stride_h, de != nullptr, ka, (Cmid + 31) / 32, (dp.Cout + 31) / 32 * 2, &nbuf).total > kMbMaxLds)
        return "weights + tiles do not fit the LDS budget";
    const long cin = de ? de->Cin : Cmid;
    if ((long)dd.N * dd.H * dd.W * cin * 2 >= (1L << 31) || (long)dd.N * Ho * Wo * dp.Cout * 2 >= (1L << 31)) return kTensorTooLarge;
    return nullptr;
}

static void launch_mean(const void* x, void* y, int N, int HW, int C, int dt, int ot, hipStream_t s, int radix = 1) {
    dim3 grid((unsigned)N, (unsigned)((C / 8 + 511) / 512));
    for_dtype_out(dt, ot, [&](auto T, auto O) { spatial_mean_kernel<DT_OF(T), DT_OF(O)><<<grid, 512, 0, s>>>(x, y, HW, C, radix); });
}
static int launch_avg(pcv_ctx* ctx, const char* fn, const void* x, void* y, int N, int H, int W, int C, int Ho, int Wo, int k, int s,
                      int dt, int ot, hipStream_t st, int pad = 0, int count_pad = 1, uint32_t* ovf = nullptr) {
    unsigned grid = 0;
    if (int rc = flat_grid(ctx, fn, (long long)N * Ho * Wo * (C / 8), &grid)) return rc;
    for_dtype_out(dt, ot, [&](auto T, auto O) {
        avgpool_kernel<DT_OF(T), DT_OF(O)><<<grid, 256, 0, st>>>(x, y, N, H, W, C, Ho, Wo, k, s, pad, count_pad, ovf);
    });
    return launched(ctx);
}


extern "C" {

int pcv_abi_version(void) { return PCV_ABI_VERSION; }

size_t pcv_conv_desc_size(void) { return sizeof(pcv_conv_desc); }

const char* pcv_last_error(const pcv_ctx* ctx) { return ctx ? ctx->err.c_str() : g_create_err.c_str(); }

int pcv_create(pcv_ctx** out, int device) {
    if (out == nullptr) return fail(nullptr, PCV_ERR_INVALID, "pcv_create: out is NULL");
    *out = nullptr;
    int count = 0;
    if (hipGetDeviceCount(&count) != hipSuccess || count <= 0)
        return fail(nullptr, PCV_ERR_NO_DEVICE, "pcv_create: no HIP device visible");
    if (device < 0 || device >= count) return fail(nullptr, PCV_ERR_INVALID, "pcv_create: bad device index");
    hipDeviceProp_t prop;
    HIP_TRY(nullptr, hipGetDeviceProperties(&prop, device));
    if (std::strncmp(prop.gcnArchName, "gfx950", 6) != 0)
        return fail(nullptr, PCV_ERR_NO_DEVICE,
                    std::string("pcv_create: device is ") + prop.gcnArchName + ", this library is built for gfx950 only");
    int prev = 0;
    HIP_TRY(nullptr, hipGetDevice(&prev));
    HIP_TRY(nullptr, hipSetDevice(device));
    pcv_ctx* ctx = new (std::nothrow) pcv_ctx();
    if (ctx == nullptr) return fail(nullptr, PCV_ERR_INVALID, "pcv_create: out of host memory");
    ctx->device = device;
    ctx->num_cu = prop.multiProcessorCount;
    if (const char* e = std::getenv("PCV_AMD_PERSIST")) ctx->persist_mode = std::atoi(e);
    if (const char* e = std::getenv("PCV_AMD_PERSIST_NK")) ctx->persist_max_nk = std::atoi(e);
    int rc = enable_kernels(ctx);
    if (rc == PCV_OK) {
        hipError_t e = hipMalloc(reinterpret_cast<void**>(&ctx->ovf), 256);
        if (e == hipSuccess) e = hipMemset(ctx->ovf, 0, 256);
        if (e != hipSuccess) rc = fail(ctx, PCV_ERR_HIP, std::string("pcv_create: overflow counter: ") + hipGetErrorString(e));
    }
    if (rc != PCV_OK) {
        g_create_err = ctx->err;
        if (ctx->ovf) (void)hipFree(ctx->ovf);
        delete ctx;
        (void)hipSetDevice(prev);
        return rc;
    }
    (void)hipSetDevice(prev);
    *out = ctx;
    return PCV_OK;
}

static const struct { const char* key; int pcv_ctx::*field; } kTuningKeys[] = {
    {"persist", &pcv_ctx::persist_mode}, {"persist_nk", &pcv_ctx::persist_max_nk}, {"tile", &pcv_ctx::force_tile},
    {"pair_pb", &pcv_ctx::pair_pb},      {"max_blocks", &pcv_ctx::max_blocks},     {"d3x3", &pcv_ctx::use_d3x3},
    {"d3w", &pcv_ctx::use_d3w},          {"d3c", &pcv_ctx::use_d3c},               {"d3k", &pcv_ctx::use_d3k},
    {"d3i", &pcv_ctx::use_d3i},          {"d1i", &pcv_ctx::use_d1i},               {"p1r", &pcv_ctx::use_p1r},
    {"head", &pcv_ctx::use_head},        {"stem32", &pcv_ctx::use_stem32},         {"d1x1", &pcv_ctx::use_d1x1},
    {"gconvr", &pcv_ctx::use_gconvr},    {"mbw", &pcv_ctx::use_mbw},               {"mbr", &pcv_ctx::use_mbr},
    {"mbr_xl", &pcv_ctx::use_mbr_xl},    {"dw_th", &pcv_ctx::dw_th},               {"dw_flags", &pcv_ctx::dw_flags},
    {"wstat", &pcv_ctx::use_wstat},      {"bnu_band", &pcv_ctx::bnu_band},         {"gconvx", &pcv_ctx::use_gconvx},
};
int pcv_set_tuning(pcv_ctx* ctx, const char* key, int value) {
    if (!ctx || !key) return PCV_ERR_INVALID;
    const std::string k(key);
    for (const auto& t : kTuningKeys)
        if (k == t.key) {
            ctx->*t.field = value;
            return PCV_OK;
        }
    if (k == "mbw_wide") g_mbw_wide = value;
    else if (k == "wpair") g_wpair_mask = value;
    else if (k == "bnu") g_bnu = value;
    else if (k == "dbg") {
#ifdef PCV_DBG_FLAGS
        ctx->dbg_flags = value;
#else
        if (value != 0)
            return fail(ctx, PCV_ERR_INVALID, "pcv_set_tuning: \"dbg\" (timing experiments that produce wrong results) needs a -DPCV_DBG_FLAGS build");
#endif
    }
    else if (k == "dbg_lo") ctx->dbg_ptr = (ctx->dbg_ptr & 0xFFFFFFFF00000000ull) | (unsigned)value;
    else if (k == "dbg_hi") ctx->dbg_ptr = (ctx->dbg_ptr & 0xFFFFFFFFull) | ((unsigned long long)(unsigned)value << 32);
    else return fail(ctx, PCV_ERR_INVALID, "pcv_set_tuning: unknown key " + k);
    return PCV_OK;
}

int pcv_destroy(pcv_ctx* ctx) {
    if (ctx && ctx->ovf) {
        DeviceGuard device_guard(ctx->device);
        (void)hipFree(ctx->ovf);
    }
    delete ctx;
    return PCV_OK;
}

int pcv_fp16_guard_begin(pcv_ctx* ctx, unsigned* slot, void* stream) {
    PCV_ENTER(ctx);
    if (!slot) return fail(ctx, PCV_ERR_INVALID, "pcv_fp16_guard_begin: slot is NULL");
    f16_guard_begin_kernel<<<1, 1, 0, (hipStream_t)stream>>>(ctx->ovf, slot);
    return launched(ctx);
}

int pcv_fp16_guard_end(pcv_ctx* ctx, const unsigned* slot, float* y, long count, void* stream) {
    PCV_ENTER(ctx);
    if (!slot || !y || count <= 0) return fail(ctx, PCV_ERR_INVALID, "pcv_fp16_guard_end: bad argument");
    const unsigned grid = (unsigned)std::min<long>((count + 255) / 256, 1024);
    f16_guard_end_kernel<<<grid, 256, 0, (hipStream_t)stream>>>(ctx->ovf, slot, y, count);
    return launched(ctx);
}

extern "C++" {
namespace {
typedef int (*nccl_group_fn)(void);
typedef int (*nccl_bcast_fn)(const void*, void*, size_t, int, int, void*, hipStream_t);
typedef int (*nccl_gather_fn)(const void*, void*, size_t, int, void*, hipStream_t);
typedef const char* (*nccl_err_fn)(int);
struct RcclApi {
    nccl_group_fn group_start = nullptr, group_end = nullptr;
    nccl_bcast_fn broadcast = nullptr;
    nccl_gather_fn allgather = nullptr;
    nccl_err_fn error_string = nullptr;
    bool ok = false;
};
const RcclApi& rccl_api() {
    static const RcclApi api = [] {
        RcclApi a;
        void* h = dlopen("librccl.so.1", RTLD_NOW | RTLD_NOLOAD);
        if (!h) h = dlopen("librccl.so.1", RTLD_NOW);
        if (!h) h = dlopen("librccl.so", RTLD_NOW);
        if (!h) return a;
        a.group_start = reinterpret_cast<nccl_group_fn>(dlsym(h, "ncclGroupStart"));
        a.group_end = reinterpret_cast<nccl_group_fn>(dlsym(h, "ncclGroupEnd"));
        a.broadcast = reinterpret_cast<nccl_bcast_fn>(dlsym(h, "ncclBroadcast"));
        a.allgather = reinterpret_cast<nccl_gather_fn>(dlsym(h, "ncclAllGather"));
        a.error_string = reinterpret_cast<nccl_err_fn>(dlsym(h, "ncclGetErrorString"));
        a.ok = a.group_start && a.group_end && a.broadcast && a.allgather;
        return a;
    }();
    return api;
}
const int kNcclUint8 = 1;
int rccl_fail(pcv_ctx* ctx, const char* what, int rc) {
    const RcclApi& R = rccl_api();
    return fail(ctx, PCV_ERR_HIP, std::string(what) + ": " + (R.error_string ? R.error_string(rc) : "RCCL error") + " (" + std::to_string(rc) + ")");
}
}
}

int pcv_rccl_available(void) { return rccl_api().ok ? 1 : 0; }

int pcv_rccl_broadcast(pcv_ctx* ctx, void* comm, void* const* bufs, const size_t* bytes, int count, int root, void* stream) {
    PCV_ENTER(ctx);
    if (!comm || !bufs || !bytes || count <= 0 || root < 0) return fail(ctx, PCV_ERR_INVALID, "pcv_rccl_broadcast: bad argument");
    for (int i = 0; i < count; ++i)
        if (!bufs[i] || bytes[i] == 0) return fail(ctx, PCV_ERR_INVALID, "pcv_rccl_broadcast: NULL or empty buffer");
    const RcclApi& R = rccl_api();
    if (!R.ok) return fail(ctx, PCV_ERR_INVALID, "pcv_rccl_broadcast: no RCCL in this process (librccl.so.1 not found)");
    int rc = R.group_start();
    if (rc != 0) return rccl_fail(ctx, "ncclGroupStart", rc);
    for (int i = 0; i < count && rc == 0; ++i) rc = R.broadcast(bufs[i], bufs[i], bytes[i], kNcclUint8, root, comm, (hipStream_t)stream);
    const int rc_end = R.group_end();
    if (rc != 0) return rccl_fail(ctx, "ncclBroadcast", rc);
    if (rc_end != 0) return rccl_fail(ctx, "ncclGroupEnd", rc_end);
    return PCV_OK;
}

int pcv_rccl_allgather(pcv_ctx* ctx, void* comm, const void* send, void* recv, size_t bytes_per_rank, void* stream) {
    PCV_ENTER(ctx);
    if (!comm || !send || !recv || bytes_per_rank == 0) return fail(ctx, PCV_ERR_INVALID, "pcv_rccl_allgather: bad argument");
    const RcclApi& R = rccl_api();
    if (!R.ok) return fail(ctx, PCV_ERR_INVALID, "pcv_rccl_allgather: no RCCL in this process (librccl.so.1 not found)");
    const int rc = R.allgather(send, recv, bytes_per_rank, kNcclUint8, comm, (hipStream_t)stream);
    if (rc != 0) return rccl_fail(ctx, "ncclAllGather", rc);
    return PCV_OK;
}

int pcv_fp16_overflow_count(pcv_ctx* ctx, unsigned* count, void* stream) {
    PCV_ENTER(ctx);
    if (!count) return fail(ctx, PCV_ERR_INVALID, "pcv_fp16_overflow_count: count is NULL");
    HIP_TRY(ctx, hipMemcpyAsync(count, ctx->ovf, sizeof(unsigned), hipMemcpyDeviceToHost, (hipStream_t)stream));
    HIP_TRY(ctx, hipStreamSynchronize((hipStream_t)stream));
    return PCV_OK;
}

int pcv_nchw_to_nhwc(pcv_ctx* ctx, const float* x, void* y, int N, int C, int H, int W, int cpitch, int wpitch,
                     int dtype, void* stream) {
    PCV_ENTER(ctx);
    if (!x || !y || N <= 0 || C <= 0 || H <= 0 || W <= 0 || cpitch < C || wpitch < W || !dtype_ok(dtype))
        return fail(ctx, PCV_ERR_INVALID, "pcv_nchw_to_nhwc: bad argument");
    if (!(cpitch == 4 || cpitch % 8 == 0) && !(dtype == PCV_F32 && cpitch % 4 == 0))
        return fail(ctx, PCV_ERR_INVALID, "pcv_nchw_to_nhwc: cpitch must be 4 or a multiple of 8");
    dim3 grid(0, (unsigned)((cpitch + 7) / 8));
    if (int rc = flat_grid(ctx, "pcv_nchw_to_nhwc", (long long)N * H * wpitch, &grid.x)) return rc;
    hipStream_t s = (hipStream_t)stream;
    for_dtype(dtype, [&](auto T) { nchw_to_nhwc_kernel<DT_OF(T)><<<grid, 256, 0, s>>>(x, y, N, C, H, W, cpitch, wpitch, ctx->ovf); });
    return launched(ctx);
}

int pcv_nhwc_to_nchw(pcv_ctx* ctx, const void* x, float* y, int N, int C, int H, int W, int cpitch, int dtype, void* stream) {
    PCV_ENTER(ctx);
    if (cpitch <= 0) cpitch = C;
    if (!x || !y || N <= 0 || C <= 0 || H <= 0 || W <= 0 || cpitch < C || !dtype_ok(dtype))
        return fail(ctx, PCV_ERR_INVALID, "pcv_nhwc_to_nchw: bad argument");
    unsigned grid = 0;
    if (int rc = flat_grid(ctx, "pcv_nhwc_to_nchw", (long long)N * C * H * W, &grid)) return rc;
    hipStream_t s = (hipStream_t)stream;
    for_dtype(dtype, [&](auto T) { nhwc_to_nchw_kernel<DT_OF(T)><<<grid, 256, 0, s>>>(x, y, N, C, H, W, cpitch); });
    return launched(ctx);
}

int pcv_conv_packed_bytes(const pcv_conv_desc* d, size_t* bytes) {
    if (!d || !bytes) return PCV_ERR_INVALID;
    ConvPlan P;
    if (plan_conv(*d, P, false) != nullptr) return PCV_ERR_INVALID;
    *bytes = P.total_bytes;
    return PCV_OK;
}

int pcv_conv_pack(pcv_ctx* ctx, const pcv_conv_desc* d, const float* w, void* packed, void* stream) {
    PCV_ENTER(ctx);
    if (!d || !w || !packed) return fail(ctx, PCV_ERR_INVALID, "pcv_conv_pack: NULL argument");
    if (!aligned16(packed)) return fail(ctx, PCV_ERR_INVALID, "pcv_conv_pack: packed buffer must be 16-byte aligned");
    ConvPlan P;
    const char* why = plan_conv(*d, P, true);
    if (why) return fail(ctx, PCV_ERR_INVALID, std::string("pcv_conv_pack: ") + why);
// ... 1101 lines not shown
int pcv_avgpool2d_pad(pcv_ctx* ctx, const void* x, void* y, int N, int H, int W, int C, int k, int s, int p, int ceil_mode,
                      int count_include_pad, int dtype, int out_dtype, void* stream) {
    PCV_ENTER(ctx);
    if (!x || !y || N <= 0 || H <= 0 || W <= 0 || C <= 0 || C % 8 != 0 || k <= 0 || s <= 0 || p < 0 || 2 * p > k ||
        !dtype_ok(dtype) || (out_dtype != dtype && out_dtype != PCV_F32))
        return fail(ctx, PCV_ERR_INVALID, "pcv_avgpool2d_pad: bad argument (C must be a multiple of 8, pad <= k/2)");
    if (H + 2 * p < k || W + 2 * p < k) return fail(ctx, PCV_ERR_INVALID, "pcv_avgpool2d_pad: window wider than the padded map");
    const int Ho = pool_out(H, k, s, p, ceil_mode), Wo = pool_out(W, k, s, p, ceil_mode);
    if (Ho <= 0 || Wo <= 0) return fail(ctx, PCV_ERR_INVALID, "pcv_avgpool2d_pad: empty output");
    hipStream_t st = (hipStream_t)stream;
    const int cp = count_include_pad ? 1 : 0;
    return launch_avg(ctx, "pcv_avgpool2d_pad", x, y, N, H, W, C, Ho, Wo, k, s, dtype, out_dtype, st, p, cp, ctx->ovf);
}

int pcv_conv1x1_pair_supported(const pcv_conv_desc* d1, const pcv_conv_desc* d2) {
    return (d1 && d2 && pair_unsupported(*d1, *d2) == nullptr) ? 1 : 0;
}

static int pair_impl(pcv_ctx* ctx, const pcv_conv_desc* d1, const pcv_conv_desc* d2, const void* x, const void* packed1,
                     const float* scale1, const float* shift1, const float* gate, const void* residual, void* y1,
                     const void* packed2, const float* scale2, const float* shift2, void* y2, void* stream);

int pcv_conv1x1_pair_fused(pcv_ctx* ctx, const pcv_conv_desc* d1, const pcv_conv_desc* d2, const void* x, const void* packed1,
                           const float* scale1, const float* shift1, const void* residual, void* y1, const void* packed2,
                           const float* scale2, const float* shift2, void* y2, void* stream) {
    return pair_impl(ctx, d1, d2, x, packed1, scale1, shift1, nullptr, residual, y1, packed2, scale2, shift2, y2, stream);
}

int pcv_conv1x1_pair_gated_supported(const pcv_conv_desc* d1, const pcv_conv_desc* d2) {
    if (!d1 || !d2 || pair_unsupported(*d1, *d2) != nullptr) return 0;
    const int cfg = wpair_cfg(d1->Cin, d1->Cout);
    if (cfg >= 0 && wpair_launch(cfg, d1->dtype, true).gate_in_lds && d1->H * d1->W < wpair_launch(cfg, d1->dtype, true).tileP) return 0;
    return 1;
}

int pcv_conv1x1_pair_gated_fused(pcv_ctx* ctx, const pcv_conv_desc* d1, const pcv_conv_desc* d2, const void* x,
                                 const void* packed1, const float* scale1, const float* shift1, const float* gate,
                                 const void* residual, void* y1, const void* packed2, const float* scale2, const float* shift2,
                                 void* y2, void* stream) {
    if (!ctx) return PCV_ERR_INVALID;
    if (!gate || !aligned16(gate) || !pcv_conv1x1_pair_gated_supported(d1, d2))
        return fail(ctx, PCV_ERR_INVALID, "pcv_conv1x1_pair_gated_fused: unsupported pair or missing gate");
    return pair_impl(ctx, d1, d2, x, packed1, scale1, shift1, gate, residual, y1, packed2, scale2, shift2, y2, stream);
}

static int pair_impl(pcv_ctx* ctx, const pcv_conv_desc* d1, const pcv_conv_desc* d2, const void* x, const void* packed1,
                     const float* scale1, const float* shift1, const float* gate, const void* residual, void* y1,
                     const void* packed2, const float* scale2, const float* shift2, void* y2, void* stream) {
    PCV_ENTER(ctx);
    if (!d1 || !d2 || !x || !packed1 || !scale1 || !shift1 || !residual || !y1 || !packed2 || !scale2 || !shift2 || !y2)
        return fail(ctx, PCV_ERR_INVALID, "pcv_conv1x1_pair_fused: NULL argument");
    if (const char* why = pair_unsupported(*d1, *d2)) return fail(ctx, PCV_ERR_INVALID, std::string("pcv_conv1x1_pair_fused: ") + why);
    if (!aligned16(x) || !aligned16(packed1) || !aligned16(packed2) || !aligned16(residual) || !aligned16(y1) || !aligned16(y2))
        return fail(ctx, PCV_ERR_INVALID, "pcv_conv1x1_pair_fused: pointers must be 16-byte aligned");
    ConvPlan P1, P2;
    const char* why = plan_conv(*d1, P1, false);
    if (!why) why = plan_conv(*d2, P2, false);
    if (why) return fail(ctx, PCV_ERR_INVALID, std::string("pcv_conv1x1_pair_fused: ") + why);
    const long M = (long)d1->N * d1->H * d1->W;
    hipStream_t st = (hipStream_t)stream;
    if (d1->Cin >= 128) {
        const int CM = d1->Cin, C1 = d1->Cout, cfg = wpair_cfg(CM, C1);
        if (cfg < 0 || P1.wrows != C1 || P1.Kpad != CM || P2.wrows != CM || P2.Kpad != C1 || P1.ngb != 1 || P2.ngb != 1)
            return fail(ctx, PCV_ERR_INVALID, "pcv_conv1x1_pair_fused: unexpected packed layout");
        WPairParams q;
        std::memset(&q, 0, sizeof(q));
        q.x = x; q.res = residual; q.y1 = y1; q.y2 = y2; q.ovf = ctx->ovf;
        q.w1 = static_cast<const char*>(packed1) + P1.ktab_bytes;
        q.w2 = static_cast<const char*>(packed2) + P2.ktab_bytes;
        q.scale1 = scale1; q.shift1 = shift1; q.scale2 = scale2; q.shift2 = shift2;
        q.x_bytes = q.y2_bytes = (uint32_t)(M * CM * 2); q.res_bytes = q.y1_bytes = (uint32_t)(M * C1 * 2);
        q.w1_bytes = q.w2_bytes = (uint32_t)(C1 * CM * 2);
        const WPairLaunch L = wpair_launch(cfg, d1->dtype, gate != nullptr);
        q.gate = gate;
        q.div_hw = make_fastdiv((uint32_t)(d1->H * d1->W));
        q.hw = (uint32_t)(d1->H * d1->W);
        q.M = (int)M; q.nTiles = (int)((M + L.tileP - 1) / L.tileP);
        q.act1 = d1->act; q.post1 = d1->post_act; q.act2 = d2->act;
        const unsigned grid = (unsigned)std::min<long>(q.nTiles, (long)block_slots(ctx, ctx->wpair_bpc[cfg]));
        return launch(ctx, L.k, grid, st, q);
    }
    if (P1.wrows != 256 || P1.Kpad != 64 || P2.wrows != 64 || P2.Kpad != 256 || P1.ngb != 1 || P2.ngb != 1)
        return fail(ctx, PCV_ERR_INVALID, "pcv_conv1x1_pair_fused: unexpected packed layout");
    PairParams p;
    std::memset(&p, 0, sizeof(p));
    p.x = x; p.res = residual; p.y1 = y1; p.y2 = y2; p.ovf = ctx->ovf;
    p.w1 = static_cast<const char*>(packed1) + P1.ktab_bytes;
    p.w2 = static_cast<const char*>(packed2) + P2.ktab_bytes;
    p.scale1 = scale1; p.shift1 = shift1; p.scale2 = scale2; p.shift2 = shift2;
    p.x_bytes = (uint32_t)(M * 64 * 2); p.res_bytes = p.y1_bytes = (uint32_t)(M * 256 * 2); p.y2_bytes = (uint32_t)(M * 64 * 2);
    p.w1_bytes = 256 * 64 * 2; p.w2_bytes = 64 * 256 * 2;
    const int pb = ctx->pair_pb == 4 ? 4 : 2;
    p.M = (int)M; p.nTiles = (int)((M + 16 * pb - 1) / (16 * pb));
    p.act1 = d1->act; p.post1 = d1->post_act; p.act2 = d2->act;
    p.gate = gate;
    p.div_hw = make_fastdiv((uint32_t)(d1->H * d1->W));
    const PairForm form = gate ? PAIR_GATED : (pb == 4 ? PAIR_PB4 : PAIR_PB2);
    if (gate) p.nTiles = (int)((M + 31) / 32);
    const unsigned grid = (unsigned)std::min<long>(p.nTiles, (long)block_slots(ctx, ctx->pair_bpc[form == PAIR_PB4 ? 0 : 1]));
    return launch(ctx, kPair[d1->dtype == PCV_BF16 ? 0 : 1][form], grid, st, p);
}

static const char* pair_idconv_unsupported(const pcv_conv_desc& di, const pcv_conv_desc& a, const pcv_conv_desc& b) {
    if (desc_stale(di)) return kStaleDesc;
    if (const char* why = pair_unsupported(a, b)) return why;
    if (a.Cin != 64) return "identity-convolution variant: only the 64 -> 256 -> 64 pair is instantiated";
    if (!plain_1x1(di) || di.dtype != a.dtype) return "identity convolution must be a plain 1x1 stride 1 of the same dtype";
    if (di.N != a.N || di.H != a.H || di.W != a.W || di.Cin != 64 || di.Cout != a.Cout) return "identity convolution shapes do not match";
    if (di.act != PCV_ACT_NONE || di.has_residual || di.post_act != PCV_ACT_NONE) return "identity convolution must have no activation";
    return nullptr;
}

int pcv_conv1x1_pair_idconv_supported(const pcv_conv_desc* d_id, const pcv_conv_desc* d1, const pcv_conv_desc* d2) {
    return (d_id && d1 && d2 && pair_idconv_unsupported(*d_id, *d1, *d2) == nullptr) ? 1 : 0;
}

int pcv_conv1x1_pair_idconv_fused(pcv_ctx* ctx, const pcv_conv_desc* d_id, const pcv_conv_desc* d1, const pcv_conv_desc* d2,
                                  const void* x0, const void* packed_id, const float* scale_id, const float* shift_id,
                                  const void* x, const void* packed1, const float* scale1, const float* shift1, void* y1,
                                  const void* packed2, const float* scale2, const float* shift2, void* y2, void* stream) {
    PCV_ENTER(ctx);
    if (!d_id || !d1 || !d2 || !x0 || !packed_id || !scale_id || !shift_id || !x || !packed1 || !scale1 || !shift1 || !y1 ||
        !packed2 || !scale2 || !shift2 || !y2)
        return fail(ctx, PCV_ERR_INVALID, "pcv_conv1x1_pair_idconv_fused: NULL argument");
    if (const char* why = pair_idconv_unsupported(*d_id, *d1, *d2))
        return fail(ctx, PCV_ERR_INVALID, std::string("pcv_conv1x1_pair_idconv_fused: ") + why);
    if (!aligned16(x0) || !aligned16(packed_id) || !aligned16(x) || !aligned16(packed1) || !aligned16(packed2) || !aligned16(y1) ||
        !aligned16(y2))
        return fail(ctx, PCV_ERR_INVALID, "pcv_conv1x1_pair_idconv_fused: pointers must be 16-byte aligned");
    ConvPlan Pi, P1, P2;
    const char* why = plan_conv(*d_id, Pi, false);
    if (!why) why = plan_conv(*d1, P1, false);
    if (!why) why = plan_conv(*d2, P2, false);
    if (why) return fail(ctx, PCV_ERR_INVALID, std::string("pcv_conv1x1_pair_idconv_fused: ") + why);
    if (P1.wrows != 256 || P1.Kpad != 64 || P2.wrows != 64 || P2.Kpad != 256 || Pi.wrows != 256 || Pi.Kpad != 64 || P1.ngb != 1 ||
        P2.ngb != 1 || Pi.ngb != 1)
        return fail(ctx, PCV_ERR_INVALID, "pcv_conv1x1_pair_idconv_fused: unexpected packed layout");
    PairParams p;
    std::memset(&p, 0, sizeof(p));
    const long M = (long)d1->N * d1->H * d1->W;
    p.x = x; p.res = nullptr; p.y1 = y1; p.y2 = y2; p.x0 = x0; p.ovf = ctx->ovf;
    p.w1 = static_cast<const char*>(packed1) + P1.ktab_bytes;
    p.w2 = static_cast<const char*>(packed2) + P2.ktab_bytes;
    p.wid = static_cast<const char*>(packed_id) + Pi.ktab_bytes;
    p.scale1 = scale1; p.shift1 = shift1; p.scale2 = scale2; p.shift2 = shift2; p.scale_id = scale_id; p.shift_id = shift_id;
    p.x_bytes = p.x0_bytes = (uint32_t)(M * 64 * 2); p.res_bytes = 0; p.y1_bytes = (uint32_t)(M * 256 * 2); p.y2_bytes = (uint32_t)(M * 64 * 2);
    p.w1_bytes = p.wid_bytes = 256 * 64 * 2; p.w2_bytes = 64 * 256 * 2;
    p.M = (int)M; p.nTiles = (int)((M + 31) / 32);
    p.act1 = d1->act; p.post1 = d1->post_act; p.act2 = d2->act;
    const unsigned grid = (unsigned)std::min<long>(p.nTiles, (long)block_slots(ctx, ctx->pair_idc_bpc));
    return launch(ctx, kPair[d1->dtype == PCV_BF16 ? 0 : 1][PAIR_IDCONV], grid, (hipStream_t)stream, p);
}

static const char* bottleneck_unsupported(const pcv_conv_desc& a, const pcv_conv_desc& b, const pcv_conv_desc& c, const pcv_conv_desc* di) {
    if (desc_stale(a) || desc_stale(b) || desc_stale(c) || (di && desc_stale(*di))) return kStaleDesc;
    if (g_bnu == 0) return "switched off (pcv_set_tuning(\"bnu\", 0))";
    if (a.dtype != PCV_BF16 && a.dtype != PCV_F16) return "16-bit storage only";
    if (b.dtype != a.dtype || c.dtype != a.dtype || (di && di->dtype != a.dtype)) return "one storage type for the whole unit";
    if (!plain_1x1(a) || !plain_1x1(c) || (di && !plain_1x1(*di))) return "conv1, conv3 and the identity convolution must be plain 1x1 stride 1";
    const bool b3x3 = b.kh == 3 && b.kw == 3 && b.stride_h == 1 && b.stride_w == 1 && b.dil_h == 1 && b.dil_w == 1 && b.pad_t == 1 &&
                      b.pad_l == 1 && b.pad_b == 1 && b.pad_r == 1 && b.groups == 1 && b.out_dtype == b.dtype &&
                      (b.x_cpitch == 0 || b.x_cpitch == b.Cin) && (b.x_wpitch == 0 || b.x_wpitch == b.W) && (b.y_cpitch == 0 || b.y_cpitch == b.Cout);
    if (!b3x3) return "conv2 must be a dense 3x3, stride 1, pad 1";
    if (a.Cin != (di ? 64 : 256) || a.Cout != 64 || b.Cin != 64 || b.Cout != 64 || c.Cin != 64 || c.Cout != 256)
        return "only 256 -> 64 -> 64 -> 256 (64 -> .. with an identity convolution) is instantiated";
    if (a.W != BnuCfg<false>::W || a.N < 1 || a.H < 1) return "56-wide maps only";
    if (b.N != a.N || b.H != a.H || b.W != a.W || c.N != a.N || c.H != a.H || c.W != a.W) return "shapes do not chain";
    if (a.has_residual || a.post_act != PCV_ACT_NONE || b.has_residual || b.post_act != PCV_ACT_NONE || !c.has_residual)
        return "conv3 carries the skip add, conv1 and conv2 do not";
    if (a.act > PCV_ACT_RELU6 || b.act > PCV_ACT_RELU6 || c.act > PCV_ACT_RELU6 || c.post_act > PCV_ACT_RELU6 || a.act < 0 || b.act < 0 ||
        c.act < 0 || c.post_act < 0)
        return "clamp activations only (none / ReLU / ReLU6)";
    if (di) {
        if (di->N != a.N || di->H != a.H || di->W != a.W || di->Cin != 64 || di->Cout != 256) return "identity convolution shapes do not match";
        if (di->act != PCV_ACT_NONE || di->has_residual || di->post_act != PCV_ACT_NONE) return "identity convolution must have no activation";
    }
    if ((long)a.N * a.H * a.W * c.Cout * 2 >= (1L << 31)) return kTensorTooLarge;
    return nullptr;
}

int pcv_bottleneck_supported(const pcv_conv_desc* d1, const pcv_conv_desc* d2, const pcv_conv_desc* d3, const pcv_conv_desc* d_id) {
    return (d1 && d2 && d3 && bottleneck_unsupported(*d1, *d2, *d3, d_id) == nullptr) ? 1 : 0;
}

int pcv_bottleneck_fused(pcv_ctx* ctx, const pcv_conv_desc* d1, const pcv_conv_desc* d2, const pcv_conv_desc* d3, const pcv_conv_desc* d_id,
                         const void* x, const void* packed1, const float* scale1, const float* shift1, const void* packed2,
                         const float* scale2, const float* shift2, const void* packed3, const float* scale3, const float* shift3,
                         const void* packed_id, const float* scale_id, const float* shift_id, void* y, void* stream) {
    PCV_ENTER(ctx);
    if (!d1 || !d2 || !d3 || !x || !packed1 || !scale1 || !shift1 || !packed2 || !scale2 || !shift2 || !packed3 || !scale3 || !shift3 || !y ||
        (d_id && (!packed_id || !scale_id || !shift_id)))
        return fail(ctx, PCV_ERR_INVALID, "pcv_bottleneck_fused: NULL argument");
    if (const char* why = bottleneck_unsupported(*d1, *d2, *d3, d_id)) return fail(ctx, PCV_ERR_INVALID, std::string("pcv_bottleneck_fused: ") + why);
    if (!aligned16(x) || !aligned16(packed1) || !aligned16(packed2) || !aligned16(packed3) || !aligned16(y) || (d_id && !aligned16(packed_id)))
        return fail(ctx, PCV_ERR_INVALID, "pcv_bottleneck_fused: pointers must be 16-byte aligned");
    ConvPlan P1, P2, P3, Pi;
    const char* why = plan_conv(*d1, P1, false);
    if (!why) why = plan_conv(*d2, P2, false);
    if (!why) why = plan_conv(*d3, P3, false);
    if (!why && d_id) why = plan_conv(*d_id, Pi, false);
    if (why) return fail(ctx, PCV_ERR_INVALID, std::string("pcv_bottleneck_fused: ") + why);
    if (P1.wrows != 64 || P1.Kpad != d1->Cin || !P2.conv3 || P2.wrows != 64 || P2.Kpad != 9 * 64 || P3.wrows != 256 || P3.Kpad != 64 ||
        P1.ngb != 1 || P2.ngb != 1 || P3.ngb != 1 || (d_id && (Pi.wrows != 256 || Pi.Kpad != 64 || Pi.ngb != 1)))
        return fail(ctx, PCV_ERR_INVALID, "pcv_bottleneck_fused: unexpected packed layout");
    BnuParams p;
    std::memset(&p, 0, sizeof(p));
    p.x = x; p.y = y; p.ovf = ctx->ovf;
    p.w1 = static_cast<const char*>(packed1) + P1.ktab_bytes;
    p.w2 = static_cast<const char*>(packed2) + P2.ktab_bytes;
    p.w3 = static_cast<const char*>(packed3) + P3.ktab_bytes;
    p.scale1 = scale1; p.shift1 = shift1; p.scale2 = scale2; p.shift2 = shift2; p.scale3 = scale3; p.shift3 = shift3;
    p.w1_bytes = (uint32_t)(64 * d1->Cin * 2); p.w2_bytes = 64 * 9 * 64 * 2; p.w3_bytes = 256 * 64 * 2;
    if (d_id) {
        p.wid = static_cast<const char*>(packed_id) + Pi.ktab_bytes;
        p.wid_bytes = 256 * 64 * 2;
        p.scale_id = scale_id; p.shift_id = shift_id;
    }
    p.N = d1->N; p.H = d1->H;
    p.y_bytes = (uint32_t)((long)d1->N * d1->H * d1->W * 256 * 2);
    int band = d1->H;
    if (ctx->bnu_band > 0) band = std::min(ctx->bnu_band, d1->H);
    else if (d1->N < ctx->num_cu) {
        const int nb = std::max(1, std::min((d1->H + 3) / 4, (ctx->num_cu + d1->N - 1) / d1->N));
        band = (d1->H + nb - 1) / nb;
    }
    p.band = band; p.nBands = (d1->H + band - 1) / band;
    const long long items = (long long)d1->N * p.nBands;
    if (items >= 0x7FFFFFFFll) return fail(ctx, PCV_ERR_TOO_LARGE, "pcv_bottleneck_fused: too many items; split the batch");
    p.nItems = (int)items;
    p.act1 = d1->act; p.act2 = d2->act; p.act3 = d3->act; p.post3 = d3->post_act;
    const unsigned grid = (unsigned)std::min<long long>(items, block_slots(ctx, 1));
    return launch(ctx, kBnu[d1->dtype == PCV_BF16 ? 0 : 1][d_id ? 1 : 0], grid, (hipStream_t)stream, p);
}

int pcv_channel_slice(pcv_ctx* ctx, const void* x, void* y, long rows, int C, int offset, int x_cpitch, int y_cpitch, int dtype,
                      void* stream) {
    PCV_ENTER(ctx);
    if (!x || !y || rows <= 0 || C <= 0 || offset < 0 || x_cpitch < offset + C || y_cpitch < C || y_cpitch % 8 != 0 || !dtype_ok(dtype))
        return fail(ctx, PCV_ERR_INVALID, "pcv_channel_slice: bad argument (y_cpitch must be a multiple of 8 and hold C channels)");
    unsigned grid = 0;
    if (int rc = flat_grid(ctx, "pcv_channel_slice", (long long)rows * (y_cpitch / 8), &grid)) return rc;
    hipStream_t st = (hipStream_t)stream;
    for_dtype(dtype, [&](auto T) { channel_slice_kernel<DT_OF(T)><<<grid, 256, 0, st>>>(x, y, rows, C, offset, x_cpitch, y_cpitch); });
    return launched(ctx);
}

int pcv_channel_concat(pcv_ctx* ctx, const void* x, void* y, long rows, int C, int x_cpitch, int y_cpitch, int y_offset, int dtype,
                       void* stream) {
    PCV_ENTER(ctx);
    if (!x || !y || rows <= 0 || C <= 0 || C % 8 != 0 || x_cpitch < C || x_cpitch % 8 != 0 || y_offset < 0 || y_offset % 8 != 0 ||
        y_cpitch < y_offset + C || y_cpitch % 8 != 0 || !dtype_ok(dtype) || !aligned16(x) || !aligned16(y))
        return fail(ctx, PCV_ERR_INVALID, "pcv_channel_concat: bad argument (C, offset and pitches must be multiples of 8, y must hold the slice)");
    unsigned grid = 0;
    if (int rc = flat_grid(ctx, "pcv_channel_concat", (long long)rows * (C / 8), &grid)) return rc;
    hipStream_t st = (hipStream_t)stream;
    for_dtype(dtype, [&](auto T) { channel_concat_kernel<DT_OF(T)><<<grid, 256, 0, st>>>(x, y, rows, C, x_cpitch, y_cpitch, y_offset); });
    return launched(ctx);
}

int pcv_interpolate(pcv_ctx* ctx, const void* x, void* y, int N, int H, int W, int C, int Ho, int Wo, int bilinear,
                    int align_corners, int dtype, void* stream) {
    PCV_ENTER(ctx);
    if (!x || !y || N <= 0 || H <= 0 || W <= 0 || C <= 0 || C % 8 != 0 || Ho <= 0 || Wo <= 0 || !dtype_ok(dtype))
        return fail(ctx, PCV_ERR_INVALID, "pcv_interpolate: bad argument (C must be a multiple of 8)");
    unsigned grid = 0;
    if (int rc = flat_grid(ctx, "pcv_interpolate", (long long)N * Ho * Wo * (C / 8), &grid)) return rc;
    hipStream_t st = (hipStream_t)stream;
    for_dtype(dtype, [&](auto T) { interpolate_kernel<DT_OF(T)><<<grid, 256, 0, st>>>(x, y, N, H, W, C, Ho, Wo, bilinear, align_corners); });
    return launched(ctx);
}

static int check_hr_fuse(int nsrc, const int* shift, int N, int H, int W, int C, int act, int dtype, const char** why) {
    *why = nullptr;
    if (nsrc < 1 || nsrc > kHrMaxSrc) *why = "needs 1 .. 4 sources";
    else if (!shift) *why = "NULL shift array";
    else if (!dtype_ok(dtype)) *why = "unknown dtype";
    else if (act != PCV_ACT_NONE && act != PCV_ACT_RELU) *why = "the activation must be PCV_ACT_NONE or PCV_ACT_RELU";
    else if (N <= 0 || H <= 0 || W <= 0 || C <= 0) *why = "empty output";
    else if (C % 8 != 0) *why = "C (the physical channel pitch) must be a multiple of 8";
    if (*why) return PCV_ERR_INVALID;
    for (int t = 0; t < nsrc; ++t) {
        if (shift[t] < 0 || shift[t] > kHrMaxShift) { *why = "a shift must be in 0 .. 3"; return PCV_ERR_INVALID; }
        const int m = (1 << shift[t]) - 1;
        if ((H & m) != 0 || (W & m) != 0) { *why = "H and W must be exact multiples of 1 << shift (the size does not divide)"; return PCV_ERR_INVALID; }
    }
    unsigned long long ybytes = (unsigned long long)N * (unsigned long long)H;
    if (in_window(ybytes)) ybytes *= (unsigned long long)W;
    if (in_window(ybytes)) ybytes *= (unsigned long long)C * esize(dtype);
    if (!in_window(ybytes)) { *why = kTensorTooLarge; return PCV_ERR_TOO_LARGE; }
    return PCV_OK;
}

int pcv_hr_fuse_supported(int nsrc, const int* shift, int N, int H, int W, int C, int act, int dtype) {
    const char* why = nullptr;
    if (check_hr_fuse(nsrc, shift, N, H, W, C, act, dtype, &why) != PCV_OK) {
        fail(nullptr, PCV_ERR_INVALID, std::string("pcv_hr_fuse_supported: ") + why);
        return 0;
    }
    return 1;
}

int pcv_hr_fuse(pcv_ctx* ctx, const void* const* src, const int* shift, int nsrc, void* y, int N, int H, int W, int C, int act,
                int dtype, void* stream) {
    PCV_ENTER(ctx);
    const char* why = nullptr;
    if (int rc = check_hr_fuse(nsrc, shift, N, H, W, C, act, dtype, &why)) return fail(ctx, rc, std::string("pcv_hr_fuse: ") + why);
// ... 258 lines not shown
```

### pytorchcv_amd/engine.py

```python

__all__ = ['NHWC', 'DTYPES', 'default_dtype', 'set_compute_dtype', 'compute_dtype_of', 'Fp16Guard', 'fp16_overflow_count', 'from_nchw', 'to_nchw', 'ConvRunner',
           'MixConvRunner', 'ghost_dw', 'BnActRunner', 'IBNConvRunner', 'InstNormRunner', 'maxpool2d', 'avgpool2d', 'avgpool2d_pad', 'global_avgpool', 'se_excite', 'se_scale', 'se_forward', 'splat_forward', 'cbam_channel_gate', 'cbam_spatial', 'cbam_forward', 'channel_slice', 'cat_shuffle2', 'act_code',
           'boundary', 'round8', 'channel_concat_into', 'interpolate', 'add', 'hr_fuse', 'hr_fuse_supported', 'classify']

import os
import ctypes
import torch
import torch.nn as nn
import torch.nn.functional as F
from . import _lib
from ._lib import ConvDesc

DTYPES = {"fp32": (0, torch.float32), "bf16": (1, torch.bfloat16), "fp16": (2, torch.float16)}
_CODE_OF_TORCH = {torch.float32: 0, torch.bfloat16: 1, torch.float16: 2}
_NAME_OF_TORCH = {torch.float32: "fp32", torch.bfloat16: "bf16", torch.float16: "fp16"}


def default_dtype() -> str:
    d = os.environ.get("PCV_AMD_DTYPE", "auto")
    if d not in DTYPES and d != "auto":
        raise ValueError("PCV_AMD_DTYPE must be one of {}".format(sorted(DTYPES) + ["auto"]))
    return d


# ... 348 lines not shown
        if self.depthwise or self.pad4 is not None or x.src.numel() * 4 >= (1 << 31):
            return None
        d = self.desc(x, act, 0, False)
        if not _lib.lib().pcv_conv2d_nchw_stem_supported(ctypes.byref(d), 1 if pool else 0):
            return None
        self.prepare(x, d)
        Ho, Wo = _conv_out(d, x.H, x.W)
        if pool:
            Ho, Wo = (Ho + 2 - 3) // 2 + 1, (Wo + 2 - 3) // 2 + 1
        if Ho <= 0 or Wo <= 0:
            return None
        y = torch.empty((x.N, Ho, Wo, d.Cout), dtype=x.dtype, device=x.device)
        _call(x.device, "conv2d_nchw_stem_fused", ctypes.byref(d), _ptr(x.src), _ptr(self.packed), _ptr(self.scale), _ptr(self.shift),
              _ptr(y), 1 if pool else 0)
        return NHWC(y, x.N, Ho, Wo, self.conv.out_channels, cpitch=d.Cout)

    def run_maxpool(self, x: NHWC, act: int, k: int, s: int, p: int, ceil_mode: bool = False):
        if not FUSE_UNITS or self.depthwise or self.pad4 is not None:
            return None
        _require_eval(self)
        if isinstance(x, LazyNCHW) and not x.materialized and (k, s, p) == (3, 2, 1) and not ceil_mode:
            y = self._stem_from_nchw(x, act, pool=True)
            if y is not None:
                return y
        d = self.desc(x, act, 0, False)
        if not _lib.lib().pcv_conv2d_maxpool_supported(ctypes.byref(d), k, s, p, 1 if ceil_mode else 0):
            return None
        self.prepare(x, d)
        Ho, Wo = _conv_out(d, x.H, x.W)
        Hq, Wq = (Ho + 2 * p - k) // s + 1, (Wo + 2 * p - k) // s + 1
        if Hq <= 0 or Wq <= 0:
            return None
        y = torch.empty((x.N, Hq, Wq, d.Cout), dtype=x.dtype, device=x.device)
        _call(x.device, "conv2d_maxpool_fused", ctypes.byref(d), _ptr(x.t), _ptr(self.packed), _ptr(self.scale), _ptr(self.shift),
              _ptr(y), k, s, p, 1 if ceil_mode else 0)
        return NHWC(y, x.N, Hq, Wq, self.conv.out_channels, cpitch=d.Cout)

    def run_pair(self, x: NHWC, residual: NHWC, act: int, post_act: int, nxt: "ConvRunner", nxt_act: int, gate=None):
        if not FUSE_UNITS or residual is None or self.depthwise or nxt.depthwise or self.pad4 is not None or nxt.pad4 is not None:
            return None
        _require_eval(self, nxt)
        c = self.conv
        L = _lib.lib()
        d1 = self.desc(x, act, post_act, True)
        d2 = nxt.desc(_ShapeOnly(x.N, x.H, x.W, c.out_channels, x.dtype), nxt_act, 0, False)
        supported = L.pcv_conv1x1_pair_gated_supported if gate is not None else L.pcv_conv1x1_pair_supported
        if not supported(ctypes.byref(d1), ctypes.byref(d2)):
            return None
        if not residual.dense or residual.dtype != x.dtype or tuple(residual.t.shape) != (x.N, x.H, x.W, d1.Cout):
            raise RuntimeError("residual shape/dtype mismatch")
        if gate is not None and (gate.dtype != torch.float32 or tuple(gate.shape) != (x.N, d1.Cout) or not gate.is_contiguous()):
            raise RuntimeError("gate must be a contiguous fp32 [N, {}] tensor".format(d1.Cout))
        t1 = torch.empty((x.N, x.H, x.W, d1.Cout), dtype=x.dtype, device=x.device)
        t2 = torch.empty((x.N, x.H, x.W, d2.Cout), dtype=x.dtype, device=x.device)
        y1 = NHWC(t1, x.N, x.H, x.W, c.out_channels, cpitch=d1.Cout)
        self.prepare(x, d1)
        nxt.prepare(y1, d2)
        first = (ctypes.byref(d1), ctypes.byref(d2), _ptr(x.t), _ptr(self.packed), _ptr(self.scale), _ptr(self.shift))
        second = (_ptr(residual.t), _ptr(t1), _ptr(nxt.packed), _ptr(nxt.scale), _ptr(nxt.shift), _ptr(t2))
        if gate is not None:
            _call(x.device, "conv1x1_pair_gated_fused", *first, _ptr(gate), *second)
        else:
            _call(x.device, "conv1x1_pair_fused", *first, *second)
        return y1, NHWC(t2, x.N, x.H, x.W, nxt.conv.out_channels, cpitch=d2.Cout)

    def run_pair_idconv(self, x: NHWC, x0: NHWC, idr: "ConvRunner", act: int, post_act: int, nxt: "ConvRunner", nxt_act: int):
        if not FUSE_UNITS or any(r.depthwise or r.pad4 is not None for r in (self, idr, nxt)):
            return None
        _require_eval(self, idr, nxt)
        if not x0.dense or x0.dtype != x.dtype or (x0.N, x0.H, x0.W) != (x.N, x.H, x.W):
            return None
        c = self.conv
        di = idr.desc(x0, 0, 0, False)
        d1 = self.desc(x, act, post_act, True)
        d2 = nxt.desc(_ShapeOnly(x.N, x.H, x.W, c.out_channels, x.dtype), nxt_act, 0, False)
        if not _lib.lib().pcv_conv1x1_pair_idconv_supported(ctypes.byref(di), ctypes.byref(d1), ctypes.byref(d2)):
            return None
        t1 = torch.empty((x.N, x.H, x.W, d1.Cout), dtype=x.dtype, device=x.device)
        t2 = torch.empty((x.N, x.H, x.W, d2.Cout), dtype=x.dtype, device=x.device)
        y1 = NHWC(t1, x.N, x.H, x.W, c.out_channels, cpitch=d1.Cout)
        idr.prepare(x0, di)
        self.prepare(x, d1)
        nxt.prepare(y1, d2)
        _call(x.device, "conv1x1_pair_idconv_fused", ctypes.byref(di), ctypes.byref(d1), ctypes.byref(d2), _ptr(x0.t), _ptr(idr.packed),
              _ptr(idr.scale), _ptr(idr.shift), _ptr(x.t), _ptr(self.packed), _ptr(self.scale), _ptr(self.shift), _ptr(t1),
              _ptr(nxt.packed), _ptr(nxt.scale), _ptr(nxt.shift), _ptr(t2))
        return y1, NHWC(t2, x.N, x.H, x.W, nxt.conv.out_channels, cpitch=d2.Cout)

    def _launch(self, x: NHWC, d: ConvDesc, residual, out=None, gate=None):
        c = self.conv
        Ho, Wo = _conv_out(d, x.H, x.W)
        if Ho <= 0 or Wo <= 0:
            raise RuntimeError("convolution output would be empty")
        out_dt = torch.float32 if d.out_dtype == 0 else x.dtype
        if out is not None:
            buf, coff = out
            if self.depthwise or tuple(buf.shape[:3]) != (x.N, Ho, Wo) or buf.dtype != out_dt or not buf.is_contiguous() or \
                    coff % 8 != 0 or c.out_channels % 8 != 0 or coff + c.out_channels > buf.shape[3] or buf.device != x.device:
                raise RuntimeError("bad concatenation slice for a convolution output (channel counts must be multiples of 8)")
            d.y_cpitch = int(buf.shape[3])
            y = buf[:, :, :, coff:]
        else:
            y = torch.empty((x.N, Ho, Wo, d.Cout), dtype=out_dt, device=x.device)
        if residual is not None:
            if not residual.dense or tuple(residual.t.shape) != (x.N, Ho, Wo, d.Cout) or residual.dtype != x.dtype:
                raise RuntimeError("residual shape/dtype mismatch: {} vs {}".format(
                    tuple(residual.t.shape), (x.N, Ho, Wo, d.Cout)))
        if gate is not None:
            if self.depthwise or gate.dtype != torch.float32 or tuple(gate.shape) != (x.N, d.Cout) or not gate.is_contiguous():
                raise RuntimeError("gate must be a contiguous fp32 [N, {}] tensor of a dense convolution".format(d.Cout))
        self._launch_range(x, d, residual, y, 0, x.N, gate)
        return None if out is not None else NHWC(y, x.N, Ho, Wo, c.out_channels, cpitch=d.Cout)

    def _launch_range(self, x, d, residual, y, n0, n1, gate=None):
        d.N = n1 - n0
        args = (ctypes.byref(d), _ptr(x.t[n0:n1]), _ptr(self.packed), _ptr(self.scale), _ptr(self.shift))
        rest = (_ptr(residual.t[n0:n1]) if residual is not None else None, _ptr(y[n0:n1]))
        halve = (_lib.PCV_ERR_TOO_LARGE,) if n1 - n0 > 1 else ()
        if gate is not None:
            rc = _call(x.device, "conv2d_gated_fused", *args, _ptr(gate[n0:n1]), *rest, accept=halve)
        else:
            rc = _call(x.device, "dwconv2d_fused" if self.depthwise else "conv2d_fused", *args, *rest, accept=halve)
        if rc != 0:
            mid = (n0 + n1) // 2
            self._launch_range(x, d, residual, y, n0, mid, gate)
            self._launch_range(x, d, residual, y, mid, n1, gate)

    def squeezed_excite(self, z: NHWC, w1, b1, w2, b2, mid_act: int, out_act: int) -> torch.Tensor:
        c = self.conv
        if self.depthwise or c.groups != 1 or tuple(_pair(c.kernel_size)) != (1, 1) or tuple(_pair(c.stride)) != (1, 1) or \
                self.pad4 is not None or tuple(_pair(c.padding)) != (0, 0):
            raise RuntimeError("squeezed_excite needs a plain 1x1 stride-1 convolution")
        d = self.desc(z, 0, 0, False)
        self.prepare(z, d)
        key = ("sq", self._key) + tuple((t.data_ptr(), t._version) for t in (w1, w2, b1, b2))
        if getattr(self, "_sq_key", None) != key:
            Cl, CP = c.out_channels, d.Cout
            w = c.weight.detach().float().reshape(Cl, -1)
            w = F.pad(w, (0, d.Cin - w.shape[1], 0, CP - Cl)) * self.scale[:, None]
            w1p = F.pad(w1.float(), (0, CP - Cl))
            self._sq_w1 = (w1p @ w).contiguous()
            self._sq_b1 = (w1p @ self.shift + b1.float()).contiguous()
            self._sq_w2 = F.pad(w2.float(), (0, 0, 0, CP - Cl)).contiguous()
            self._sq_b2 = F.pad(b2.float(), (0, CP - Cl)).contiguous()
            self._sq_key = key
        M = self._sq_w1.shape[0]
        mean = torch.empty((z.N, d.Cin), dtype=torch.float32, device=z.device)
        _call(z.device, "se_squeeze", _ptr(z.t), _ptr(mean), z.N, z.H * z.W, d.Cin, _CODE_OF_TORCH[z.dtype])
        mid = torch.empty((z.N, M), dtype=torch.float32, device=z.device)
        gate = torch.empty((z.N, d.Cout), dtype=torch.float32, device=z.device)
        _call(z.device, "fc_f32", _ptr(mean), _ptr(self._sq_w1), _ptr(self._sq_b1), _ptr(mid), z.N, d.Cin, M, mid_act)
        _call(z.device, "fc_f32", _ptr(mid), _ptr(self._sq_w2), _ptr(self._sq_b2), _ptr(gate), z.N, M, d.Cout, out_act)
        return gate


class MixConvRunner(ConvRunner):
    def __init__(self, convs, bn):
        self.convs = list(convs)
        self.conv, self.bn, self.pad4 = self.convs[0], bn, None
        self._key = None
        self._foreign = False
        self.packed = self.scale = self.shift = None
        self.depthwise = True
        G = len(self.convs)
        for g, c in enumerate(self.convs):
            k = 3 + 2 * g
            if _pair(c.kernel_size) != (k, k) or _pair(c.padding) != (k // 2, k // 2) or _pair(c.dilation) != (1, 1) or \
                    c.groups != c.in_channels or c.in_channels != c.out_channels or _pair(c.stride) != _pair(self.conv.stride) or \
                    c.padding_mode != "zeros":
                raise NotImplementedError("MixConv on the MI355X path: depthwise groups with windows 3, 5, ... and padding k // 2, "
                                          "got group {} = {}".format(g, c))
        if not 2 <= G <= 5:
            raise NotImplementedError("MixConv with {} kernels: the MI355X path takes 2 to 5".format(G))
        self.channels = sum(c.out_channels for c in self.convs)
        self.kernels = (ctypes.c_int * G)(*[3 + 2 * g for g in range(G)])

    def _sources(self):
        ts = []
        for c in self.convs:
            ts += [c.weight, c.bias]
        if self.bn is not None:
            ts += [self.bn.weight, self.bn.bias, self.bn.running_mean, self.bn.running_var]
        return ts

    def desc(self, x: NHWC, act: int) -> ConvDesc:
        C, G = self.channels, len(self.convs)
        if not x.dense or x.C != C or x.cpitch != C:
            raise RuntimeError("MixConv expects a dense handle of {} channels (a multiple of 8), got {} / pitch {}".format(C, x.C, x.cpitch))
        k = 3 + 2 * (G - 1)
        s = _pair(self.conv.stride)
        code = _CODE_OF_TORCH[x.dtype]
        return ConvDesc(N=x.N, H=x.H, W=x.W, Cin=C, Cout=C, kh=k, kw=k, stride_h=s[0], stride_w=s[1], pad_t=k // 2, pad_l=k // 2,
                        pad_b=k // 2, pad_r=k // 2, dil_h=1, dil_w=1, groups=C, act=act, post_act=0, has_residual=0, dtype=code,
                        out_dtype=code, x_cpitch=C, x_wpitch=x.W)

    def prepare(self, x: NHWC, d: ConvDesc):
        key = (x.dtype, d.Cin) + tuple((t.data_ptr(), t._version) if t is not None else None for t in self._sources())
        if key == self._key:
            return
        if self._foreign:
            raise RuntimeError("this MixConv's packed weights were received by parallel.broadcast_packed_state and would have to be "
                               "re-packed: call parallel.broadcast_module_state(net) first")
        dev, C, G = x.device, d.Cin, len(self.convs)
        if self.conv.weight.device != dev:
            raise RuntimeError("model parameters are on {} but the input is on {}".format(self.conv.weight.device, dev))
        L = _lib.lib()
        nbytes = ctypes.c_size_t(0)
        if L.pcv_mixconv_packed_bytes(ctypes.byref(d), self.kernels, G, ctypes.byref(nbytes)) != 0:
            raise _lib.PcvError(-1, "unsupported MixConv configuration: {}".format((L.pcv_last_error(None) or b"").decode()))
        packed = torch.empty((nbytes.value + 15) // 16 * 16, dtype=torch.uint8, device=dev)
        ws = [c.weight.detach().float().contiguous() for c in self.convs]
        _call(dev, "mixconv_pack", ctypes.byref(d), self.kernels, G, (ctypes.c_void_p * G)(*[w.data_ptr() for w in ws]), _ptr(packed))
        scale = torch.empty(C, dtype=torch.float32, device=dev)
        shift = torch.empty(C, dtype=torch.float32, device=dev)
        bias = None
        if any(c.bias is not None for c in self.convs):
            bias = torch.cat([c.bias.detach().float() if c.bias is not None else torch.zeros(c.out_channels, device=dev)
                              for c in self.convs]).contiguous()
        bn = self.bn
        if bn is not None:
            if not isinstance(bn, nn.BatchNorm2d):
                raise NotImplementedError("only BatchNorm2d folds into the conv epilogue, got {}".format(type(bn).__name__))
            g = (bn.weight if bn.weight is not None else torch.ones(C, device=dev)).detach().float().contiguous()
            b = (bn.bias if bn.bias is not None else torch.zeros(C, device=dev)).detach().float().contiguous()
            m, v = bn.running_mean.detach().float().contiguous(), bn.running_var.detach().float().contiguous()
            _call(dev, "bn_fold", C, _ptr(g), _ptr(b), _ptr(m), _ptr(v), ctypes.c_float(bn.eps), _ptr(bias), _ptr(scale), _ptr(shift))
        else:
            _call(dev, "bn_fold", C, None, None, None, None, ctypes.c_float(0.0), _ptr(bias), _ptr(scale), _ptr(shift))
        torch.cuda.current_stream(dev).synchronize()
        self.packed, self.scale, self.shift, self._key = packed, scale, shift, key

    def run(self, x: NHWC, act: int = 0) -> NHWC:
        _require_eval(self)
        d = self.desc(x, act)
        self.prepare(x, d)
        Ho, Wo = _conv_out(d, x.H, x.W)
        y = torch.empty((x.N, Ho, Wo, d.Cout), dtype=x.dtype, device=x.device)
        self._launch_range(x, d, None, y, 0, x.N)
        return NHWC(y, x.N, Ho, Wo, self.channels, cpitch=d.Cout)

    def _launch_range(self, x, d, residual, y, n0, n1, gate=None):
        d.N = n1 - n0
        rc = _call(x.device, "mixconv2d_fused", ctypes.byref(d), self.kernels, len(self.convs), _ptr(x.t[n0:n1]), _ptr(self.packed),
                   _ptr(self.scale), _ptr(self.shift), _ptr(y[n0:n1]), accept=(_lib.PCV_ERR_TOO_LARGE,) if n1 - n0 > 1 else ())
        if rc != 0:
            mid = (n0 + n1) // 2
            self._launch_range(x, d, None, y, n0, mid)
            self._launch_range(x, d, None, y, mid, n1)


def ghost_dw(runner: ConvRunner, m: NHWC, act: int, residual: NHWC | None = None) -> NHWC:
    _require_eval(runner)
    c = runner.conv
    Cm = c.out_channels
    if not runner.depthwise or c.in_channels != Cm:
        raise NotImplementedError("ghost module: the cheap convolution must be depthwise with as many outputs as inputs, got {}".format(c))
    if not m.dense or m.C != Cm:
        raise RuntimeError("ghost module: expected a dense handle of {} channels, got {} / pitch {} / row pitch {}".format(
            Cm, m.C, m.cpitch, m.wpitch))
    dp = runner.desc(m, act, 0, False)
    d = runner.desc(m, act, 0, residual is not None)
    d.Cin = d.Cout = d.groups = Cm
    d.y_cpitch = 2 * Cm
    L = _lib.lib()
    if not L.pcv_ghost_supported(ctypes.byref(d)):
        raise NotImplementedError("ghost module ({} + {} channels on a {}x{} map) is not covered by the MI355X path: {}".format(
            Cm, Cm, m.H, m.W, (L.pcv_last_error(None) or b"").decode()))
    runner.prepare(m, dp)
    if residual is not None:
        if not residual.dense or tuple(residual.t.shape) != (m.N, m.H, m.W, 2 * Cm) or residual.dtype != m.dtype:
            raise RuntimeError("residual shape/dtype mismatch: {} vs {}".format(tuple(residual.t.shape), (m.N, m.H, m.W, 2 * Cm)))
    y = torch.empty((m.N, m.H, m.W, 2 * Cm), dtype=m.dtype, device=m.device)

    def launch(n0, n1):
        d.N = n1 - n0
        rc = _call(m.device, "ghost_dw_fused", ctypes.byref(d), _ptr(m.t[n0:n1]), _ptr(runner.packed), _ptr(runner.scale),
                   _ptr(runner.shift), _ptr(residual.t[n0:n1]) if residual is not None else None, _ptr(y[n0:n1]),
                   accept=(_lib.PCV_ERR_TOO_LARGE,) if n1 - n0 > 1 else ())
        if rc != 0:
            mid = (n0 + n1) // 2
            launch(n0, mid)
            launch(mid, n1)
    launch(0, m.N)
    return NHWC(y, m.N, m.H, m.W, 2 * Cm, cpitch=2 * Cm)


def _pool_out(n: int, k: int, s: int, p: int, ceil_mode: bool) -> int:
    o = (n + 2 * p - k + (s - 1 if ceil_mode else 0)) // s + 1
    if ceil_mode and (o - 1) * s >= n + p:
        o -= 1
    return o


def channel_slice(x: NHWC, offset: int, count: int) -> NHWC:
    if x.wpitch != x.W or offset < 0 or offset + count > x.C:
        raise RuntimeError("bad channel slice")
    cp = round8(count)
    y = torch.empty((x.N, x.H, x.W, cp), dtype=x.dtype, device=x.device)
    _call(x.device, "channel_slice", _ptr(x.t), _ptr(y), x.N * x.H * x.W, count, offset, x.cpitch, cp, _CODE_OF_TORCH[x.dtype])
    return NHWC(y, x.N, x.H, x.W, count, cpitch=cp)


def channel_concat_into(x: NHWC, buf: torch.Tensor, coff: int):
    if x.wpitch != x.W or x.C % 8 or coff % 8 or tuple(buf.shape[:3]) != (x.N, x.H, x.W) or buf.dtype != x.dtype or \
            coff + x.C > buf.shape[3] or not buf.is_contiguous():
        raise RuntimeError("channel concatenation needs channel counts / offsets that are multiples of 8 and equal maps")
# ... 433 lines not shown
```

### pytorchcv_amd/models/common/conv.py

```python

__all__ = ['conv1x1', 'conv3x3', 'depthwise_conv3x3', 'ConvBlock', 'conv1x1_block', 'conv3x3_block', 'conv5x5_block',
           'conv7x7_block', 'dwconv_block', 'dwconv3x3_block', 'dwconv5x5_block', 'DwsConvBlock', 'dwsconv3x3_block', 'BareConv', 'PreConvBlock',
           'pre_conv1x1_block', 'pre_conv3x3_block', 'conv_block_pair', 'conv_block_maxpool', 'mbconv_chain', 'conv_block_bottleneck']

import torch.nn as nn
from .activ import lambda_relu, create_activation_layer
from .norm import lambda_batchnorm2d, create_normalization_layer
from ... import engine


class BareConv(nn.Conv2d):
    def forward(self, x, out_fp32: bool = False, act: int = 0):
        if getattr(self, "_pcv_runner", None) is None:
            self._pcv_runner = engine.ConvRunner(self, None)
        return engine.boundary(self, x, lambda a: self._pcv_runner.run(a, act=act, out_fp32=out_fp32))


def conv1x1(in_channels, out_channels, stride=1, groups=1, bias=False):
    return BareConv(in_channels=in_channels, out_channels=out_channels, kernel_size=1, stride=stride, groups=groups, bias=bias)


def conv3x3(in_channels, out_channels, stride=1, padding=1, dilation=1, groups=1, bias=False):
    return BareConv(in_channels=in_channels, out_channels=out_channels, kernel_size=3, stride=stride, padding=padding,
                    dilation=dilation, groups=groups, bias=bias)


def depthwise_conv3x3(channels, stride=1, padding=1, dilation=1, bias=False):
    return BareConv(in_channels=channels, out_channels=channels, kernel_size=3, stride=stride, padding=padding,
                    dilation=dilation, groups=channels, bias=bias)


class ConvBlock(nn.Module):
    def __init__(self, in_channels, out_channels, kernel_size, stride=1, padding=0, dilation=1, groups=1, bias=False,
                 normalization=lambda_batchnorm2d(), activation=lambda_relu()):
        super(ConvBlock, self).__init__()
        self.normalize = (normalization is not None)
        self.activate = (activation is not None)
        self.use_pad = (isinstance(padding, (list, tuple)) and (len(padding) == 4))
        self._pad4 = tuple(int(p) for p in padding) if self.use_pad else None
        self.conv = nn.Conv2d(in_channels=in_channels, out_channels=out_channels, kernel_size=kernel_size, stride=stride,
                              padding=(0 if self.use_pad else padding), dilation=dilation, groups=groups, bias=bias)
        if self.normalize:
            self.bn = create_normalization_layer(normalization=normalization, num_features=out_channels)
            if self.bn is None:
                self.normalize = False
            else:
                assert isinstance(self.bn, nn.Module)
        if self.activate:
            self.activ = create_activation_layer(activation)
            if self.activ is None:
                self.activate = False
            else:
                assert isinstance(self.activ, nn.Module)
        self._pcv_runner = None

    def forward(self, x, residual=None, post_act=None, pad4=None, out=None):
        if self._pcv_runner is None:
            self._pcv_runner = engine.ConvRunner(self.conv, self.bn if self.normalize else None, pad4=self._pad4)
        act = engine.act_code(self.activ) if self.activate else 0
        pact = engine.act_code(post_act)
        return engine.boundary(self, x, lambda a: self._pcv_runner.run(a, act=act, residual=residual, post_act=pact,
                                                                       pad4=pad4, out=out))


def conv_block_maxpool(block, x, pool):
    if isinstance(block, ConvBlock) and isinstance(x, engine.NHWC) and not block.use_pad:
        if block._pcv_runner is None:
            block._pcv_runner = engine.ConvRunner(block.conv, block.bn if block.normalize else None, pad4=block._pad4)
        y = block._pcv_runner.run_maxpool(x, engine.act_code(block.activ) if block.activate else 0, pool.kernel_size,
                                          pool.stride, pool.padding, pool.ceil_mode)
        if y is not None:
            return y
    return pool(block(x))


def conv_block_pair(first, x, residual, post_act, second, id_block=None, x0=None):
    if not (isinstance(first, ConvBlock) and isinstance(second, ConvBlock) and isinstance(x, engine.NHWC)):
        return None
    for blk in (first, second) + ((id_block,) if id_block is not None else ()):
        if not isinstance(blk, ConvBlock):
            return None
        if blk._pcv_runner is None:
            blk._pcv_runner = engine.ConvRunner(blk.conv, blk.bn if blk.normalize else None, pad4=blk._pad4)
    if id_block is not None:
        if id_block.activate or not isinstance(x0, engine.NHWC):
            return None
        return first._pcv_runner.run_pair_idconv(x, x0, id_block._pcv_runner, engine.act_code(first.activ) if first.activate else 0,
                                                 engine.act_code(post_act), second._pcv_runner,
                                                 engine.act_code(second.activ) if second.activate else 0)
    return first._pcv_runner.run_pair(x, residual, engine.act_code(first.activ) if first.activate else 0,
                                      engine.act_code(post_act), second._pcv_runner,
                                      engine.act_code(second.activ) if second.activate else 0)


def mbconv_chain(exp_block, dw_block, proj_block, x, residual=None, post_act=None):
    blocks = [b for b in (exp_block, dw_block, proj_block) if b is not None]
    if not isinstance(x, engine.NHWC) or not all(isinstance(b, ConvBlock) for b in blocks):
        return None
    for blk in blocks:
        if blk._pcv_runner is None:
            blk._pcv_runner = engine.ConvRunner(blk.conv, blk.bn if blk.normalize else None, pad4=blk._pad4)

    def code(blk):
        return engine.act_code(blk.activ) if blk.activate else 0
    return engine.mbconv_fused(exp_block._pcv_runner if exp_block is not None else None,
                               code(exp_block) if exp_block is not None else 0, dw_block._pcv_runner, code(dw_block),
                               proj_block._pcv_runner, code(proj_block), x, residual, engine.act_code(post_act))


def conv_block_bottleneck(conv1, conv2, conv3, x, post_act, id_block=None, probe=False):
    blocks = (conv1, conv2, conv3) + ((id_block,) if id_block is not None else ())
    if not isinstance(x, engine.ShapeOnly if probe else engine.NHWC) or not all(isinstance(b, ConvBlock) for b in blocks):
        return None
    if id_block is not None and id_block.activate:
        return None
    for blk in blocks:
        if blk._pcv_runner is None:
            blk._pcv_runner = engine.ConvRunner(blk.conv, blk.bn if blk.normalize else None, pad4=blk._pad4)

    def code(blk):
        return engine.act_code(blk.activ) if blk.activate else 0
    return engine.bottleneck_fused(conv1._pcv_runner, code(conv1), conv2._pcv_runner, code(conv2), conv3._pcv_runner, code(conv3), x,
                                   engine.act_code(post_act), id_block._pcv_runner if id_block is not None else None, probe=probe)


def conv1x1_block(padding=0, **kwargs):
    return ConvBlock(kernel_size=1, padding=padding, **kwargs)


def conv3x3_block(padding=1, **kwargs):
    return ConvBlock(kernel_size=3, padding=padding, **kwargs)


def conv5x5_block(padding=2, **kwargs):
    return ConvBlock(kernel_size=5, padding=padding, **kwargs)


def conv7x7_block(padding=3, **kwargs):
    return ConvBlock(kernel_size=7, padding=padding, **kwargs)


def dwconv_block(out_channels, padding=1, **kwargs):
    return ConvBlock(out_channels=out_channels, padding=padding, groups=out_channels, **kwargs)


def dwconv3x3_block(padding=1, **kwargs):
    return dwconv_block(kernel_size=3, padding=padding, **kwargs)


def dwconv5x5_block(padding=2, **kwargs):
    return dwconv_block(kernel_size=5, padding=padding, **kwargs)


class DwsConvBlock(nn.Module):
    def __init__(self, in_channels, out_channels, kernel_size, stride=1, padding=0, dilation=1, bias=False,
                 dw_normalization=lambda_batchnorm2d(), pw_normalization=lambda_batchnorm2d(), dw_activation=lambda_relu(),
                 pw_activation=lambda_relu()):
        super(DwsConvBlock, self).__init__()
        self.dw_conv = dwconv_block(in_channels=in_channels, out_channels=in_channels, kernel_size=kernel_size, stride=stride,
                                    padding=padding, dilation=dilation, bias=bias, normalization=dw_normalization,
                                    activation=dw_activation)
        self.pw_conv = conv1x1_block(in_channels=in_channels, out_channels=out_channels, bias=bias,
                                     normalization=pw_normalization, activation=pw_activation)

    def _run(self, a):
        y = mbconv_chain(None, self.dw_conv, self.pw_conv, a)
        return y if y is not None else self.pw_conv(self.dw_conv(a))

    def forward(self, x):
        return engine.boundary(self, x, self._run)


def dwsconv3x3_block(padding=1, **kwargs):
    return DwsConvBlock(kernel_size=3, padding=padding, **kwargs)


class PreConvBlock(nn.Module):
    def __init__(self, in_channels, out_channels, kernel_size, stride, padding, dilation=1, bias=False,
                 normalization=lambda_batchnorm2d(), activation=lambda_relu(), return_preact=False):
        super(PreConvBlock, self).__init__()
        self.normalize = (normalization is not None)
        self.activate = (activation is not None)
        self.return_preact = return_preact
        if self.normalize:
            self.bn = create_normalization_layer(normalization=normalization, num_features=in_channels)
            if self.bn is None:
                self.normalize = False
            else:
                assert isinstance(self.bn, nn.BatchNorm2d)
        if self.activate:
            self.activ = create_activation_layer(activation)
            if self.activ is None:
                self.activate = False
            else:
                assert isinstance(self.activ, nn.Module)
        self.conv = nn.Conv2d(in_channels=in_channels, out_channels=out_channels, kernel_size=kernel_size, stride=stride,
                              padding=padding, dilation=dilation, bias=bias)
        self._pcv_pre = None
        self._pcv_runners = {}

    def act_code(self):
        return engine.act_code(self.activ) if self.activate else 0

    def preact(self, a):
        if not self.normalize:
            raise NotImplementedError("PreConvBlock without normalization on the MI355X path")
        if self._pcv_pre is None:
            self._pcv_pre = engine.BnActRunner(self.bn)
        return self._pcv_pre.run(a, self.act_code())

    def conv_then(self, a, next_block=None, residual=None, out=None, se=None):
        key = id(next_block)
        if key not in self._pcv_runners:
            bn = next_block.bn if (next_block is not None and next_block.normalize) else None
            self._pcv_runners[key] = engine.ConvRunner(self.conv, bn)
        act = next_block.act_code() if next_block is not None else 0
        runner = self._pcv_runners[key]
        gate = None
        c = self.conv
        if se is not None and next_block is None and out is None and engine.FUSE_UNITS and tuple(c.kernel_size) == (1, 1) and \
                tuple(c.stride) == (1, 1) and tuple(c.padding) == (0, 0) and a.dense:
            w1, b1, w2, b2 = se._mlp()
            gate = runner.squeezed_excite(a, w1, b1, w2, b2, engine.act_code(se.activ), engine.act_code(se.sigmoid))
        elif se is not None:
            return se(runner.run(a, act=act, out=out), residual=residual)
        return runner.run(a, act=act, residual=residual, out=out, gate=gate)

    def _run(self, a):
        pre = self.preact(a) if (self.normalize or self.activate) else a
        y = self.conv_then(pre)
        return (y, pre) if self.return_preact else y

    def forward(self, x):
        return engine.boundary(self, x, self._run)


def pre_conv1x1_block(stride=1, padding=0, **kwargs):
    return PreConvBlock(kernel_size=1, stride=stride, padding=padding, **kwargs)


def pre_conv3x3_block(stride=1, padding=1, **kwargs):
    return PreConvBlock(kernel_size=3, stride=stride, padding=padding, **kwargs)
```

### pytorchcv_amd/models/resnet.py

```python

__all__ = ['ResNet', 'resnet10', 'resnet12', 'resnet14', 'resnetbc14b', 'resnet16', 'resnet18', 'resnet26', 'resnetbc26b',
           'resnet34', 'resnetbc38b', 'resnet50', 'resnet50b', 'resnet101', 'resnet101b', 'resnet152', 'resnet152b',
           'ResBlock', 'ResBottleneck', 'SkipUnit', 'ResUnit', 'ResStage', 'ResInitBlock', 'get_resnet']

import torch.nn as nn
from .common.activ import lambda_relu
from .common.norm import lambda_batchnorm2d
from .common.conv import conv1x1_block, conv3x3_block, conv7x7_block, conv_block_pair, conv_block_maxpool, conv_block_bottleneck
from ._build import ClassifierNet, add_stages, register_variants, stage_table
from ._tail import MaxPool2dNHWC, maybe_load_pretrained, DEFAULT_ROOT
from .. import engine


class ResBlock(nn.Module):
    def __init__(self, in_channels, out_channels, stride, bias=False, normalization=lambda_batchnorm2d(),
                 activation=lambda_relu(), final_activation=None):
        super(ResBlock, self).__init__()
        self.conv1 = conv3x3_block(in_channels=in_channels, out_channels=out_channels, stride=stride, bias=bias,
                                   normalization=normalization, activation=activation)
        self.conv2 = conv3x3_block(in_channels=out_channels, out_channels=out_channels, bias=bias,
                                   normalization=normalization, activation=final_activation)

    def forward(self, x, residual=None, post_act=None):
        return engine.boundary(self, x, lambda a: self.conv2(self.conv1(a), residual=residual, post_act=post_act))


class ResBottleneck(nn.Module):
    def __init__(self, in_channels, out_channels, stride, padding=1, dilation=1, bias=False,
                 normalization=lambda_batchnorm2d(), conv1_stride=False, bottleneck_factor=4, activation=lambda_relu(),
                 final_activation=None):
        super(ResBottleneck, self).__init__()
        mid_channels = out_channels // bottleneck_factor
        self.conv1 = conv1x1_block(in_channels=in_channels, out_channels=mid_channels, stride=(stride if conv1_stride else 1),
                                   bias=bias, normalization=normalization, activation=activation)
        self.conv2 = conv3x3_block(in_channels=mid_channels, out_channels=mid_channels,
                                   stride=(1 if conv1_stride else stride), padding=padding, dilation=dilation, bias=bias,
                                   normalization=normalization, activation=activation)
        self.conv3 = conv1x1_block(in_channels=mid_channels, out_channels=out_channels, bias=bias,
                                   normalization=normalization, activation=final_activation)

    def forward(self, x, residual=None, post_act=None):
        return engine.boundary(self, x, lambda a: self.conv3(self.conv2(self.conv1(a)), residual=residual, post_act=post_act))


class SkipUnit(nn.Module):
    pcv_chainable = False

    def add_skip(self, in_channels, out_channels, stride, block=conv1x1_block, activation=lambda_relu(), name="identity_conv",
                 **block_args):
        self.resize_identity = (in_channels != out_channels) or (stride != 1)
        if self.resize_identity:
            if block is conv1x1_block:
                block_args["activation"] = None
            self.add_module(name, block(in_channels=in_channels, out_channels=out_channels, stride=stride, **block_args))
        if activation is not None:
            self.activ = activation()

    def _identity(self, a):
        return self.identity_conv(a) if self.resize_identity else a

    def _run(self, a):
        return self.body(a, residual=self._identity(a), post_act=self.activ)

    def forward(self, x):
        return engine.boundary(self, x, self._run)


class ResUnit(SkipUnit):
    def __init__(self, in_channels, out_channels, stride=1, padding=1, dilation=1, bias=False,
                 normalization=lambda_batchnorm2d(), bottleneck=True, conv1_stride=False, activation=lambda_relu(),
                 final_body_activation=None, final_activation=lambda_relu()):
        super(ResUnit, self).__init__()
        if bottleneck:
            self.body = ResBottleneck(in_channels=in_channels, out_channels=out_channels, stride=stride, padding=padding,
                                      dilation=dilation, bias=bias, normalization=normalization, conv1_stride=conv1_stride,
                                      activation=activation, final_activation=final_body_activation)
        else:
            self.body = ResBlock(in_channels=in_channels, out_channels=out_channels, stride=stride, bias=bias,
                                 normalization=normalization, activation=activation, final_activation=final_body_activation)
        self.add_skip(in_channels, out_channels, stride, activation=final_activation, bias=bias, normalization=normalization)
        self.pcv_chainable = bool(bottleneck)

    def run_chained(self, a, conv1_out=None, next_unit=None):
        body = self.body
        fused = conv_block_bottleneck(body.conv1, body.conv2, body.conv3, a, self.activ,
                                      id_block=self.identity_conv if self.resize_identity else None)
        if fused is not None:
            return fused, None
        if next_unit is not None and isinstance(next_unit, ResUnit) and self._stride1() and next_unit.fuses_whole(a):
            next_unit = None
        y = body.conv2(conv1_out if conv1_out is not None else body.conv1(a))
        if next_unit is not None and self.resize_identity:
            pair = conv_block_pair(body.conv3, y, None, self.activ, next_unit.body.conv1, id_block=self.identity_conv, x0=a)
            if pair is not None:
                return pair
        identity = self._identity(a)
        if next_unit is not None:
            pair = conv_block_pair(body.conv3, y, identity, self.activ, next_unit.body.conv1)
            if pair is not None:
                return pair
        return body.conv3(y, residual=identity, post_act=self.activ), None

    def _stride1(self):
        return all(tuple(b.conv.stride) == (1, 1) for b in (self.body.conv1, self.body.conv2, self.body.conv3))

    def fuses_whole(self, a_prev):
        if not isinstance(self.body, ResBottleneck) or not isinstance(a_prev, engine.NHWC):
            return False
        body = self.body
        x = engine.ShapeOnly(a_prev.N, a_prev.H, a_prev.W, body.conv1.conv.in_channels, a_prev.dtype)
        return conv_block_bottleneck(body.conv1, body.conv2, body.conv3, x, self.activ,
                                     id_block=self.identity_conv if self.resize_identity else None, probe=True)


class ResStage(nn.Sequential):
    def forward(self, x):
        units = list(self.children())
        chainable = all(getattr(u, "pcv_chainable", False) for u in units)
        if not isinstance(x, engine.NHWC) or not chainable:
            return super(ResStage, self).forward(x)
        conv1_out = None
        for i, unit in enumerate(units):
            x, conv1_out = unit.run_chained(x, conv1_out, units[i + 1] if i + 1 < len(units) else None)
        return x


class ResInitBlock(nn.Module):
    def __init__(self, in_channels, out_channels, normalization=lambda_batchnorm2d()):
        super(ResInitBlock, self).__init__()
        self.conv = conv7x7_block(in_channels=in_channels, out_channels=out_channels, stride=2, normalization=normalization)
        self.pool = MaxPool2dNHWC(kernel_size=3, stride=2, padding=1)

    def forward(self, x):
        return engine.boundary(self, x, lambda a: conv_block_maxpool(self.conv, a, self.pool), stem=True)


class ResNet(ClassifierNet):
    def __init__(self, channels, init_block_channels, bottleneck, conv1_stride, in_channels=3, in_size=(224, 224),
                 num_classes=1000):
        super(ResNet, self).__init__(in_size, num_classes)
        self.features.add_module("init_block", ResInitBlock(in_channels=in_channels, out_channels=init_block_channels))
        self.finish(add_stages(
            self.features, init_block_channels, channels, container=ResStage,
            make_unit=lambda cin, cout, stride, i, j: ResUnit(in_channels=cin, out_channels=cout, stride=stride,
                                                              bottleneck=bottleneck, conv1_stride=conv1_stride)))


_LAYERS = {10: [1, 1, 1, 1], 12: [2, 1, 1, 1], 16: [2, 2, 2, 1], 18: [2, 2, 2, 2], 34: [3, 4, 6, 3], 50: [3, 4, 6, 3],
           101: [3, 4, 23, 3], 152: [3, 8, 36, 3], 200: [3, 24, 36, 3], 269: [3, 30, 48, 8]}
RESNET_DEPTHS = (10, 12, 14, 16, 18, 26, 34, 38, 50, 101, 152, 200)


def resnet_layers(blocks, bottleneck, what="ResNet", depths=RESNET_DEPTHS):
    if blocks not in depths:
        layers = None
    elif blocks == 14:
        layers = [1, 1, 1, 1] if bottleneck else [2, 2, 1, 1]
    elif blocks == 26:
        layers = [2, 2, 2, 2] if bottleneck else [3, 3, 3, 3]
    elif blocks == 38:
        layers = [3, 3, 3, 3] if bottleneck else None
    else:
        layers = _LAYERS[blocks]
    if layers is None:
        raise ValueError("Unsupported {} with number of blocks: {}".format(what, blocks))
    assert (sum(layers) * (3 if bottleneck else 2) + 2 == blocks)
    return layers


def resnet_channels(blocks, bottleneck, what="ResNet", depths=RESNET_DEPTHS, width_scale=1.0):
    table = stage_table([w * (4 if bottleneck else 1) for w in (64, 128, 256, 512)], resnet_layers(blocks, bottleneck, what, depths))
    if width_scale != 1.0:
        table = [[int(c * width_scale) for c in stage] for stage in table]
        table[-1][-1] = 512 * (4 if bottleneck else 1)
    return table


def get_resnet(blocks, bottleneck=None, conv1_stride=True, width_scale=1.0, model_name=None, pretrained=False,
               root=DEFAULT_ROOT, **kwargs):
    if bottleneck is None:
        bottleneck = (blocks >= 50)
    net = ResNet(channels=resnet_channels(blocks, bottleneck, width_scale=width_scale),
                 init_block_channels=(64 if width_scale == 1.0 else int(64 * width_scale)), bottleneck=bottleneck,
                 conv1_stride=conv1_stride, **kwargs)
    return maybe_load_pretrained(net, model_name, pretrained, root)


_B = dict(conv1_stride=False)
_BC = dict(bottleneck=True, conv1_stride=False)
register_variants(__name__, get_resnet, {
    "resnet10": dict(blocks=10), "resnet12": dict(blocks=12), "resnet14": dict(blocks=14), "resnetbc14b": dict(blocks=14, **_BC),
    "resnet16": dict(blocks=16), "resnet18": dict(blocks=18), "resnet26": dict(blocks=26, bottleneck=False),
    "resnetbc26b": dict(blocks=26, **_BC), "resnet34": dict(blocks=34), "resnetbc38b": dict(blocks=38, **_BC),
    "resnet50": dict(blocks=50), "resnet50b": dict(blocks=50, **_B), "resnet101": dict(blocks=101),
    "resnet101b": dict(blocks=101, **_B), "resnet152": dict(blocks=152), "resnet152b": dict(blocks=152, **_B)})
```

### pytorchcv_amd/models/resnext.py

```python

__all__ = ['ResNeXt', 'ResNeXtBottleneck', 'ResNeXtUnit', 'get_resnext']

import math
import torch.nn as nn
from .common.conv import conv1x1_block, conv3x3_block, conv_block_pair
from .resnet import SkipUnit, ResInitBlock, ResStage, resnet_channels
from ._build import ClassifierNet, add_stages, register_variants
from ._tail import maybe_load_pretrained, DEFAULT_ROOT
from .. import engine


class ResNeXtBottleneck(nn.Module):
    def __init__(self, in_channels, out_channels, stride, cardinality, bottleneck_width, bottleneck_factor=4):
        super(ResNeXtBottleneck, self).__init__()
        mid_channels = out_channels // bottleneck_factor
        D = int(math.floor(mid_channels * (bottleneck_width / 64.0)))
        group_width = cardinality * D
        self.conv1 = conv1x1_block(in_channels=in_channels, out_channels=group_width)
        self.conv2 = conv3x3_block(in_channels=group_width, out_channels=group_width, stride=stride, groups=cardinality)
        self.conv3 = conv1x1_block(in_channels=group_width, out_channels=out_channels, activation=None)

    def forward(self, x, residual=None, post_act=None):
        return engine.boundary(self, x, lambda a: self.conv3(self.conv2(self.conv1(a)), residual=residual, post_act=post_act))


class ResNeXtUnit(SkipUnit):
    def __init__(self, in_channels, out_channels, stride, cardinality, bottleneck_width):
        super(ResNeXtUnit, self).__init__()
        self.body = ResNeXtBottleneck(in_channels=in_channels, out_channels=out_channels, stride=stride,
                                      cardinality=cardinality, bottleneck_width=bottleneck_width)
        self.add_skip(in_channels, out_channels, stride)

    pcv_chainable = True

    def run_chained(self, a, conv1_out=None, next_unit=None):
        identity = self._identity(a)
        body = self.body
        y = body.conv2(conv1_out if conv1_out is not None else body.conv1(a))
        if next_unit is not None:
            pair = conv_block_pair(body.conv3, y, identity, self.activ, next_unit.body.conv1)
            if pair is not None:
                return pair
        return body.conv3(y, residual=identity, post_act=self.activ), None


class ResNeXt(ClassifierNet):
    def __init__(self, channels, init_block_channels, cardinality, bottleneck_width, in_channels=3, in_size=(224, 224),
                 num_classes=1000):
        super(ResNeXt, self).__init__(in_size, num_classes)
        self.features.add_module("init_block", ResInitBlock(in_channels=in_channels, out_channels=init_block_channels))
        self.finish(add_stages(
            self.features, init_block_channels, channels, container=ResStage,
            make_unit=lambda cin, cout, stride, i, j: ResNeXtUnit(in_channels=cin, out_channels=cout, stride=stride,
                                                                  cardinality=cardinality, bottleneck_width=bottleneck_width)))


def get_resnext(blocks, cardinality, bottleneck_width, model_name=None, pretrained=False, root=DEFAULT_ROOT, **kwargs):
    net = ResNeXt(channels=resnet_channels(blocks, True, what="ResNeXt", depths=(14, 26, 38, 50, 101)), init_block_channels=64,
                  cardinality=cardinality, bottleneck_width=bottleneck_width, **kwargs)
    return maybe_load_pretrained(net, model_name, pretrained, root)


def _variant(name):
    depth, shape = name[len("resnext"):].split("_")
    card, width = shape[:-1].split("x")
    return dict(blocks=int(depth), cardinality=int(card), bottleneck_width=int(width))


register_variants(__name__, get_resnext, {n: _variant(n) for n in (
    "resnext14_16x4d", "resnext14_32x2d", "resnext14_32x4d", "resnext26_32x4d", "resnext50_32x4d", "resnext101_32x4d",
    "resnext101_64x4d")})
```

### pytorchcv_amd/models/seresnet.py

```python

__all__ = ['SEResNet', 'seresnet10', 'seresnet18', 'seresnet26', 'seresnetbc26b', 'seresnetbc38b', 'seresnet50', 'seresnet50b',
           'seresnet101', 'seresnet101b', 'seresnet152', 'SEResUnit', 'get_seresnet']

from .common.att import SEBlock
from .resnet import SkipUnit, ResStage, ResBlock, ResBottleneck, ResInitBlock, resnet_channels
from ._build import ClassifierNet, add_stages, register_variants
from ._tail import maybe_load_pretrained, DEFAULT_ROOT


class SEResUnit(SkipUnit):
    def __init__(self, in_channels, out_channels, stride, bottleneck, conv1_stride):
        super(SEResUnit, self).__init__()
        if bottleneck:
            self.body = ResBottleneck(in_channels=in_channels, out_channels=out_channels, stride=stride,
                                      conv1_stride=conv1_stride)
        else:
            self.body = ResBlock(in_channels=in_channels, out_channels=out_channels, stride=stride)
        self.se = SEBlock(channels=out_channels)
        self.add_skip(in_channels, out_channels, stride)

    pcv_chainable = True

    def run_chained(self, a, conv1_out=None, next_unit=None):
        identity = self._identity(a)
        body = self.body
        if not hasattr(body, "conv3"):
            return self.se(body(a), residual=identity, post_act=self.activ), None
        z = body.conv2(conv1_out if conv1_out is not None else body.conv1(a))
        nxt = next_unit.body.conv1 if (next_unit is not None and hasattr(next_unit.body, "conv3")) else None
        y = self.se.run_behind(body.conv3, z, residual=identity, post_act=self.activ, next_conv=nxt)
        if y is None:
            y = self.se(body.conv3(z), residual=identity, post_act=self.activ)
        return y if isinstance(y, tuple) else (y, None)

    def _run(self, a):
        return self.run_chained(a)[0]


class SEResNet(ClassifierNet):
    def __init__(self, channels, init_block_channels, bottleneck, conv1_stride, in_channels=3, in_size=(224, 224),
                 num_classes=1000):
        super(SEResNet, self).__init__(in_size, num_classes)
        self.features.add_module("init_block", ResInitBlock(in_channels=in_channels, out_channels=init_block_channels))
        self.finish(add_stages(
            self.features, init_block_channels, channels, container=ResStage,
            make_unit=lambda cin, cout, stride, i, j: SEResUnit(in_channels=cin, out_channels=cout, stride=stride,
                                                                bottleneck=bottleneck, conv1_stride=conv1_stride)))


def get_seresnet(blocks, bottleneck=None, conv1_stride=True, model_name=None, pretrained=False, root=DEFAULT_ROOT, **kwargs):
    if bottleneck is None:
        bottleneck = (blocks >= 50)
    net = SEResNet(channels=resnet_channels(blocks, bottleneck, what="SE-ResNet"), init_block_channels=64, bottleneck=bottleneck,
                   conv1_stride=conv1_stride, **kwargs)
    return maybe_load_pretrained(net, model_name, pretrained, root)


_BC = dict(bottleneck=True, conv1_stride=False)
register_variants(__name__, get_seresnet, {
    "seresnet10": dict(blocks=10), "seresnet18": dict(blocks=18), "seresnet26": dict(blocks=26, bottleneck=False),
    "seresnetbc26b": dict(blocks=26, **_BC), "seresnetbc38b": dict(blocks=38, **_BC), "seresnet50": dict(blocks=50),
    "seresnet50b": dict(blocks=50, conv1_stride=False), "seresnet101": dict(blocks=101),
    "seresnet101b": dict(blocks=101, conv1_stride=False), "seresnet152": dict(blocks=152)})
```

Before: 96910 images/sec.

## Fuse conv1 and projection-shortcut 1x1 convs into one dual-output kernel

Adds a dual-output variant of the p1r 1x1 conv kernel that concatenates the packed weights of a bottleneck's conv1 and its identity (downsample) conv. Both read the same input once and write to two separate outputs, each with its own activation. ResNet, ResNeXt and SE-ResNet units with a resized identity use it when conv1 output has not already been produced. By default only the 512-input-channel case is routed. This aims to save one kernel launch and a second read of the input activation, in exchange for per-channel-group output selection logic in the kernel and losing the previous conv3+identity pair fusion path for those units.

```diff
diff --git a/include/pcv_amd.h b/include/pcv_amd.h
--- a/include/pcv_amd.h
+++ b/include/pcv_amd.h
@@ -167,6 +167,13 @@
                                   const void* x, const void* packed1, const float* scale1, const float* shift1, void* y1,
                                   const void* packed2, const float* scale2, const float* shift2, void* y2, void* stream);
 
+int pcv_conv1x1_dual_supported(const pcv_conv_desc* dA, const pcv_conv_desc* dB);
+int pcv_conv1x1_dual_packed_bytes(const pcv_conv_desc* dA, const pcv_conv_desc* dB, size_t* bytes);
+int pcv_conv1x1_dual_pack(pcv_ctx* ctx, const pcv_conv_desc* dA, const pcv_conv_desc* dB, const void* packedA, const void* packedB,
+                          void* packed, void* stream);
+int pcv_conv1x1_dual_fused(pcv_ctx* ctx, const pcv_conv_desc* dA, const pcv_conv_desc* dB, const void* x, const void* packed,
+                           const float* scale, const float* shift, void* yA, void* yB, void* stream);
+
 int pcv_bottleneck_supported(const pcv_conv_desc* d1, const pcv_conv_desc* d2, const pcv_conv_desc* d3, const pcv_conv_desc* d_id);
 int pcv_bottleneck_fused(pcv_ctx* ctx, const pcv_conv_desc* d1, const pcv_conv_desc* d2, const pcv_conv_desc* d3,
                          const pcv_conv_desc* d_id, const void* x, const void* packed1, const float* scale1, const float* shift1,
diff --git a/pytorchcv_amd/_lib.py b/pytorchcv_amd/_lib.py
--- a/pytorchcv_amd/_lib.py
+++ b/pytorchcv_amd/_lib.py
@@ -94,6 +94,10 @@
     "pcv_conv1x1_pair_idconv_supported": (_I, [ctypes.POINTER(ConvDesc), ctypes.POINTER(ConvDesc), ctypes.POINTER(ConvDesc)]),
     "pcv_conv1x1_pair_idconv_fused": (_I, [_VP, ctypes.POINTER(ConvDesc), ctypes.POINTER(ConvDesc), ctypes.POINTER(ConvDesc),
                                            _VP, _VP, _VP, _VP, _VP, _VP, _VP, _VP, _VP, _VP, _VP, _VP, _VP, _VP]),
+    "pcv_conv1x1_dual_supported": (_I, [ctypes.POINTER(ConvDesc), ctypes.POINTER(ConvDesc)]),
+    "pcv_conv1x1_dual_packed_bytes": (_I, [ctypes.POINTER(ConvDesc), ctypes.POINTER(ConvDesc), ctypes.POINTER(ctypes.c_size_t)]),
+    "pcv_conv1x1_dual_pack": (_I, [_VP, ctypes.POINTER(ConvDesc), ctypes.POINTER(ConvDesc), _VP, _VP, _VP, _VP]),
+    "pcv_conv1x1_dual_fused": (_I, [_VP, ctypes.POINTER(ConvDesc), ctypes.POINTER(ConvDesc), _VP, _VP, _VP, _VP, _VP, _VP, _VP]),
     "pcv_bottleneck_supported": (_I, [ctypes.POINTER(ConvDesc), ctypes.POINTER(ConvDesc), ctypes.POINTER(ConvDesc), ctypes.POINTER(ConvDesc)]),
     "pcv_bottleneck_fused": (_I, [_VP, ctypes.POINTER(ConvDesc), ctypes.POINTER(ConvDesc), ctypes.POINTER(ConvDesc), ctypes.POINTER(ConvDesc),
                                   _VP, _VP, _VP, _VP, _VP, _VP, _VP, _VP, _VP, _VP, _VP, _VP, _VP, _VP, _VP]),
diff --git a/pytorchcv_amd/csrc/conv_device.hpp b/pytorchcv_amd/csrc/conv_device.hpp
--- a/pytorchcv_amd/csrc/conv_device.hpp
+++ b/pytorchcv_amd/csrc/conv_device.hpp
@@ -23,6 +23,14 @@
     uint32_t* ovf;
     int tailN;
     int dbgflags;
+};
+
+struct D3DualParams : D3Params {
+    void* y2;
+    uint32_t y2_bytes;
+    int Ypitch2;
+    int CoutA;
+    int act2;
 };
 
 #if defined(__HIP_DEVICE_COMPILE__)
diff --git a/pytorchcv_amd/csrc/p1r_16bit.hip b/pytorchcv_amd/csrc/p1r_16bit.hip
--- a/pytorchcv_amd/csrc/p1r_16bit.hip
+++ b/pytorchcv_amd/csrc/p1r_16bit.hip
@@ -1,7 +1,9 @@
 #include "p1r_conv.hpp"
-#define P1R_INST(CW, CIN)                                                   \
-    template __global__ void p1r_kernel<PCV_BF16, CW, CIN>(const D3Params); \
-    template __global__ void p1r_kernel<PCV_F16, CW, CIN>(const D3Params);
+#define P1R_INST(CW, CIN)                                                                \
+    template __global__ void p1r_kernel<PCV_BF16, CW, CIN>(const D3Params);              \
+    template __global__ void p1r_kernel<PCV_F16, CW, CIN>(const D3Params);               \
+    template __global__ void p1r_kernel<PCV_BF16, CW, CIN, true>(const D3DualParams);    \
+    template __global__ void p1r_kernel<PCV_F16, CW, CIN, true>(const D3DualParams);
 P1R_INST(64, 256)
 P1R_INST(32, 512)
 P1R_INST(32, 256)
diff --git a/pytorchcv_amd/csrc/p1r_conv.hpp b/pytorchcv_amd/csrc/p1r_conv.hpp
--- a/pytorchcv_amd/csrc/p1r_conv.hpp
+++ b/pytorchcv_amd/csrc/p1r_conv.hpp
@@ -27,9 +27,11 @@
     static_assert(NSTEP == 64 && TP * PPU == 64 && PPU % NW == 0 && KH % NPW == 0, "tile geometry");
 };
 
+template <bool DUAL> using P1RParams = std::conditional_t<DUAL, D3DualParams, D3Params>;
+
 #if defined(__HIP_DEVICE_COMPILE__)
-template <int DT, int CW, int CIN>
-__device__ __forceinline__ void p1r_body(const D3Params& p, char* smem) {
+template <int DT, int CW, int CIN, bool DUAL = false>
+__device__ __forceinline__ void p1r_body(const P1RParams<DUAL>& p, char* smem) {
     typedef P1RCfg<CW, CIN> G;
     typedef typename Mma<DT>::frag frag;
     typedef __attribute__((address_space(3))) char lds_char;
@@ -48,7 +50,8 @@
 
     const __amdgpu_buffer_rsrc_t wrsrc = buffer_rsrc(p.w, p.w_bytes);
     const __amdgpu_buffer_rsrc_t xrsrc = buffer_rsrc(p.x, p.x_bytes);
-    const __amdgpu_buffer_rsrc_t yrsrc = buffer_rsrc(p.y, p.y_bytes);
+    __amdgpu_buffer_rsrc_t yrsrc = buffer_rsrc(p.y, p.y_bytes);
+    int ypitch = p.Ypitch, ycout = p.Cout, ych0 = 0;
     const bool has_res = p.res != nullptr;
     const __amdgpu_buffer_rsrc_t rrsrc = buffer_rsrc(p.res, has_res ? p.res_bytes : 0u);
 
@@ -111,7 +114,17 @@
         constexpr int u = st / KH, kh = st - KH * u, s = kh >> 1, h = kh & 1;
         bq[st % RING] = *reinterpret_cast<lds_fptr>((size_t)(h ? fs1 : fs0) + (size_t)(u * G::UNITB + s * 2048));
     };
-    const EpiBounds B = make_epi_bounds(p.act, p.post_act);
+    EpiBounds B = make_epi_bounds(p.act, p.post_act);
+    auto pick_output = [&](int cg) __attribute__((always_inline)) {
+        if constexpr (DUAL) {
+            const bool second = cg * G::CG + wave * CW >= p.CoutA;
+            yrsrc = buffer_rsrc(second ? p.y2 : p.y, second ? p.y2_bytes : p.y_bytes);
+            ypitch = second ? p.Ypitch2 : p.Ypitch;
+            ycout = second ? p.Cout - p.CoutA : p.CoutA;
+            ych0 = second ? p.CoutA : 0;
+            B = make_epi_bounds(second ? p.act2 : p.act, PCV_ACT_NONE);
+        }
+    };
     constexpr int NRR = G::RES ? TP * (CWB / 2) : 1;
     u32x4 rrq[NRR];
     u32x4 opend;
@@ -152,7 +165,7 @@
     };
     uint32_t yb[CWB / 2], rb[CWB / 2];
     auto epi_store = [&](int u, int ip) __attribute__((always_inline)) {
-        __builtin_amdgcn_raw_buffer_store_b128(opend, yrsrc, yb[ip] + (uint32_t)(u * 32 * p.Ypitch), 0, 0);
+        __builtin_amdgcn_raw_buffer_store_b128(opend, yrsrc, yb[ip] + (uint32_t)(u * 32 * ypitch), 0, 0);
     };
     auto tile_steps = [&](auto HRc, auto ONEc, int slot, int ch0, int mTile) __attribute__((always_inline)) {
         constexpr bool ONE = decltype(ONEc)::value;
@@ -160,8 +173,8 @@
         F16Guard<DT> guard;
 #pragma unroll
         for (int ip = 0; ip < CWB / 2; ++ip) {
-            const bool chok = ch0 + 32 * ip < p.Cout;
-            yb[ip] = chok ? (uint32_t)(((mTile + fr) * p.Ypitch + ch0 + 32 * ip) * 2) : 0x80000000u;
+            const bool chok = ch0 + 32 * ip < ycout;
+            yb[ip] = chok ? (uint32_t)(((mTile + fr) * ypitch + ch0 + 32 * ip) * 2) : 0x80000000u;
             if constexpr (HR) rb[ip] = chok ? (uint32_t)(((mTile + fr) * p.Cout + ch0 + 32 * ip) * 2) : 0x80000000u;
         }
         if constexpr (HR) {
@@ -277,6 +290,7 @@
         const uint64_t p0__ = __builtin_amdgcn_s_memtime();
 #endif
         load_weights(cg);
+        pick_output(cg);
 #ifdef P1R_CYCLES
         const uint64_t p1__ = __builtin_amdgcn_s_memtime();
 #endif
@@ -309,8 +323,10 @@
             if (stamp__) c0__ = __builtin_amdgcn_s_memtime();
 #endif
             {
-                const int ch0 = cg * G::CG + wave * CW + 8 * fq;
-                const bool hi = p.act == PCV_ACT_RELU6 || p.post_act == PCV_ACT_RELU6, pre = p.act != PCV_ACT_NONE;
+                const int ch0 = cg * G::CG + wave * CW + 8 * fq - ych0;
+                bool hi = p.act == PCV_ACT_RELU6 || p.post_act == PCV_ACT_RELU6;
+                if constexpr (DUAL) hi = hi || p.act2 == PCV_ACT_RELU6;
+                const bool pre = p.act != PCV_ACT_NONE;
                 auto modes = [&](auto ONEc) __attribute__((always_inline)) {
                     if constexpr (G::RES) {
                         if (has_res) {
@@ -360,10 +376,10 @@
 }
 #endif
 
-template <int DT, int CW, int CIN>
-__global__ __launch_bounds__((P1RCfg<CW, CIN>::THREADS), 1) void p1r_kernel(const D3Params p) {
+template <int DT, int CW, int CIN, bool DUAL = false>
+__global__ __launch_bounds__((P1RCfg<CW, CIN>::THREADS), 1) void p1r_kernel(const P1RParams<DUAL> p) {
 #if defined(__HIP_DEVICE_COMPILE__)
     extern __shared__ __attribute__((aligned(16))) char smem[];
-    p1r_body<DT, CW, CIN>(p, smem);
+    p1r_body<DT, CW, CIN, DUAL>(p, smem);
 #endif
 }
diff --git a/pytorchcv_amd/csrc/pcv_api.hip b/pytorchcv_amd/csrc/pcv_api.hip
--- a/pytorchcv_amd/csrc/pcv_api.hip
+++ b/pytorchcv_amd/csrc/pcv_api.hip
@@ -77,9 +77,11 @@
 extern template __global__ void d1i_kernel<PCV_F16, 1024>(const D3Params);
 extern template __global__ void d1i_kernel<PCV_BF16, 2048>(const D3Params);
 extern template __global__ void d1i_kernel<PCV_F16, 2048>(const D3Params);
-#define P1R_DECLARE(CW, CIN)                                                       \
-    extern template __global__ void p1r_kernel<PCV_BF16, CW, CIN>(const D3Params); \
-    extern template __global__ void p1r_kernel<PCV_F16, CW, CIN>(const D3Params);
+#define P1R_DECLARE(CW, CIN)                                                                    \
+    extern template __global__ void p1r_kernel<PCV_BF16, CW, CIN>(const D3Params);              \
+    extern template __global__ void p1r_kernel<PCV_F16, CW, CIN>(const D3Params);               \
+    extern template __global__ void p1r_kernel<PCV_BF16, CW, CIN, true>(const D3DualParams);    \
+    extern template __global__ void p1r_kernel<PCV_F16, CW, CIN, true>(const D3DualParams);
 P1R_DECLARE(64, 256)
 P1R_DECLARE(32, 512)
 P1R_DECLARE(32, 256)
@@ -564,8 +566,12 @@
 #define P1R_ROW(CW, CIN) \
     {tile_kernel<P1RCfg<CW, CIN>>(p1r_kernel<PCV_BF16, CW, CIN>, 512), tile_kernel<P1RCfg<CW, CIN>>(p1r_kernel<PCV_F16, CW, CIN>, 512)}
 static const Kernel kP1R[3][2] = {P1R_ROW(64, 256), P1R_ROW(32, 512), P1R_ROW(32, 256)};
-static const struct { const Kernel (*rows)[2]; int n; } kD3Tables[] = {{kD3, kD3Count}, {kD1, kD1Count}, {kD3W, kD3WCount}, {kD3C, 1},
-                                                                       {kD3K, 1},       {kD3I, 2},       {kD1I, 2},         {kP1R, 3}};
+#define P1R_DUAL_ROW(CW, CIN)                                                         \
+    {tile_kernel<P1RCfg<CW, CIN>>(p1r_kernel<PCV_BF16, CW, CIN, true>, 512), tile_kernel<P1RCfg<CW, CIN>>(p1r_kernel<PCV_F16, CW, CIN, true>, 512)}
+static const Kernel kP1RDual[3][2] = {P1R_DUAL_ROW(64, 256), P1R_DUAL_ROW(32, 512), P1R_DUAL_ROW(32, 256)};
+static int g_dual = -1;
+static const struct { const Kernel (*rows)[2]; int n; } kD3Tables[] = {{kD3, kD3Count}, {kD1, kD1Count}, {kD3W, kD3WCount}, {kD3C, 1},       {kD3K, 1},
+                                                                       {kD3I, 2},       {kD1I, 2},       {kP1R, 3},         {kP1RDual, 3}};
 static int pick_d1x1(long long M, int Cout, int Cin, long long slots) {
     if (Cin < 256 || Cout < 128) return -1;
     const int shape = Cout % 256 == 0 ? 1 : 0;
@@ -919,6 +925,7 @@
     if (k == "mbw_wide") g_mbw_wide = value;
     else if (k == "wpair") g_wpair_mask = value;
     else if (k == "bnu") g_bnu = value;
+    else if (k == "dual") g_dual = value;
     else if (k == "dbg") {
 #ifdef PCV_DBG_FLAGS
         ctx->dbg_flags = value;
@@ -2326,6 +2333,112 @@
     return launch(ctx, kPair[d1->dtype == PCV_BF16 ? 0 : 1][PAIR_IDCONV], grid, (hipStream_t)stream, p);
 }
 
+static int dual_shape(int Cin, int cout_total) { return Cin == 512 ? 1 : ((cout_total < 384 || g_dual == 2) ? 2 : 0); }
+static bool dual_1x1(const pcv_conv_desc& d) {
+    return d.kh == 1 && d.kw == 1 && d.stride_h == d.stride_w && (d.stride_h == 1 || d.stride_h == 2) && d.pad_t == 0 && d.pad_l == 0 &&
+           d.pad_b == 0 && d.pad_r == 0 && d.groups == 1 && d.dil_h == 1 && d.dil_w == 1 && d.out_dtype == d.dtype;
+}
+static const char* dual_unsupported(const pcv_conv_desc& a, const pcv_conv_desc& b) {
+    if (desc_stale(a) || desc_stale(b)) return kStaleDesc;
+    if (g_dual == 0) return "switched off (pcv_set_tuning(\"dual\", 0))";
+    if (((g_dual < 0 || g_dual == 5) && a.Cin != 512) || (g_dual == 4 && a.Cin != 256))
+        return "256 input channels are not on the automatic route (pcv_set_tuning(\"dual\", 1) takes every covered pair; 4 / 5: 256 / 512 input channels only)";
+    if (a.dtype != b.dtype || (a.dtype != PCV_BF16 && a.dtype != PCV_F16)) return "16-bit storage only, one type for both convolutions";
+    if (!dual_1x1(a) || !dual_1x1(b)) return "both convolutions must be 1x1, stride 1 or 2, no padding, one group, out_dtype == dtype";
+    if (a.N != b.N || a.H != b.H || a.W != b.W || a.Cin != b.Cin || a.stride_h != b.stride_h) return "the two convolutions must read the same input at the same stride";
+    if (a.N <= 0 || a.H <= 0 || a.W <= 0) return "empty input";
+    for (const pcv_conv_desc* d : {&a, &b})
+        if ((d->x_cpitch != 0 && d->x_cpitch != d->Cin) || (d->x_wpitch != 0 && d->x_wpitch != d->W) || (d->y_cpitch != 0 && d->y_cpitch != d->Cout))
+            return "plain pitches only";
+    if (a.Cin != 256 && a.Cin != 512) return "256 or 512 input channels";
+    if (a.has_residual || b.has_residual || a.post_act != PCV_ACT_NONE || b.post_act != PCV_ACT_NONE) return "no skip tensor, no post_act";
+    if (a.act < 0 || a.act > PCV_ACT_RELU6 || b.act < 0 || b.act > PCV_ACT_RELU6) return "activations none, ReLU or ReLU6 only";
+    if (a.Cout <= 0 || b.Cout <= 0 || a.Cout % 8 != 0 || b.Cout % 8 != 0) return "channel counts must be multiples of 8";
+    const int cw = kP1RDual[dual_shape(a.Cin, a.Cout + b.Cout)][0].BM / 8;
+    if (a.Cout % cw != 0) return "the first convolution's channel count must be a multiple of the channels one wave owns (32, or 64 with 256 input channels and 384 or more output channels)";
+    const unsigned long long M = (unsigned long long)a.N * ((a.H - 1) / a.stride_h + 1) * ((a.W - 1) / a.stride_h + 1);
+    if (!in_window((unsigned long long)a.N * a.H * a.W * a.Cin * 2ull) || M >= 0x7FFFFFFFull || !in_window(M * a.Cout * 2ull) ||
+        !in_window(M * b.Cout * 2ull))
+        return kTensorTooLarge;
+    return nullptr;
+}
+
+static size_t dual_rows(const pcv_conv_desc& a, const pcv_conv_desc& b) { return (size_t)a.Cout + (size_t)round_up(b.Cout, 32); }
+
+int pcv_conv1x1_dual_supported(const pcv_conv_desc* dA, const pcv_conv_desc* dB) {
+    return (dA && dB && dual_unsupported(*dA, *dB) == nullptr) ? 1 : 0;
+}
+
+int pcv_conv1x1_dual_packed_bytes(const pcv_conv_desc* dA, const pcv_conv_desc* dB, size_t* bytes) {
+    if (!dA || !dB || !bytes || dual_unsupported(*dA, *dB) != nullptr) return PCV_ERR_INVALID;
+    *bytes = dual_rows(*dA, *dB) * dA->Cin * 2;
+    return PCV_OK;
+}
+
+int pcv_conv1x1_dual_pack(pcv_ctx* ctx, const pcv_conv_desc* dA, const pcv_conv_desc* dB, const void* packedA, const void* packedB,
+                          void* packed, void* stream) {
+    PCV_ENTER(ctx);
+    if (!dA || !dB || !packedA || !packedB || !packed) return fail(ctx, PCV_ERR_INVALID, "pcv_conv1x1_dual_pack: NULL argument");
+    if (const char* why = dual_unsupported(*dA, *dB)) return fail(ctx, PCV_ERR_INVALID, std::string("pcv_conv1x1_dual_pack: ") + why);
+    if (!aligned16(packedA) || !aligned16(packedB) || !aligned16(packed))
+        return fail(ctx, PCV_ERR_INVALID, "pcv_conv1x1_dual_pack: pointers must be 16-byte aligned");
+    ConvPlan PA, PB;
+    const char* why = plan_conv(*dA, PA, false);
+    if (!why) why = plan_conv(*dB, PB, false);
+    if (why) return fail(ctx, PCV_ERR_INVALID, std::string("pcv_conv1x1_dual_pack: ") + why);
+    if (PA.Kpad != dA->Cin || PB.Kpad != dA->Cin || PA.wrows < dA->Cout || PB.wrows < dB->Cout || PA.ngb != 1 || PB.ngb != 1)
+        return fail(ctx, PCV_ERR_INVALID, "pcv_conv1x1_dual_pack: unexpected packed layout");
+    if (PA.wrows != dA->Cout || PB.wrows != round_up(dB->Cout, 32)) return fail(ctx, PCV_ERR_INVALID, "pcv_conv1x1_dual_pack: unexpected packed layout");
+    const size_t rowb = (size_t)dA->Cin * 2, bytesA = (size_t)dA->Cout * rowb, bytesB = (size_t)PB.wrows * rowb;
+    hipStream_t s = (hipStream_t)stream;
+    HIP_TRY(ctx, hipMemcpyAsync(packed, static_cast<const char*>(packedA) + PA.ktab_bytes, bytesA, hipMemcpyDeviceToDevice, s));
+    HIP_TRY(ctx, hipMemcpyAsync(static_cast<char*>(packed) + bytesA, static_cast<const char*>(packedB) + PB.ktab_bytes, bytesB, hipMemcpyDeviceToDevice, s));
+    return PCV_OK;
+}
+
+int pcv_conv1x1_dual_fused(pcv_ctx* ctx, const pcv_conv_desc* dA, const pcv_conv_desc* dB, const void* x, const void* packed,
+                           const float* scale, const float* shift, void* yA, void* yB, void* stream) {
+    PCV_ENTER(ctx);
+    if (!dA || !dB || !x || !packed || !scale || !shift || !yA || !yB) return fail(ctx, PCV_ERR_INVALID, "pcv_conv1x1_dual_fused: NULL argument");
+    if (const char* why = dual_unsupported(*dA, *dB)) return fail(ctx, PCV_ERR_INVALID, std::string("pcv_conv1x1_dual_fused: ") + why);
+    if (!aligned16(x) || !aligned16(packed) || !aligned16(scale) || !aligned16(shift) || !aligned16(yA) || !aligned16(yB))
+        return fail(ctx, PCV_ERR_INVALID, "pcv_conv1x1_dual_fused: pointers must be 16-byte aligned");
+    const int stride = dA->stride_h, Ho = (dA->H - 1) / stride + 1, Wo = (dA->W - 1) / stride + 1, Cin = dA->Cin, total = dA->Cout + dB->Cout;
+    const unsigned long long M64 = (unsigned long long)dA->N * Ho * Wo;
+    const Kernel& K = kP1RDual[dual_shape(Cin, total)][dA->dtype == PCV_BF16 ? 0 : 1];
+    D3DualParams q;
+    std::memset(&q, 0, sizeof(q));
+    q.x = x; q.w = packed; q.scale = scale; q.shift = shift; q.ovf = ctx->ovf;
+    q.y = yA; q.y2 = yB;
+    q.dbgflags = ctx->dbg_flags;
+    q.dbg = reinterpret_cast<uint32_t*>(ctx->dbg_ptr);
+    q.x_bytes = (uint32_t)((unsigned long long)dA->N * dA->H * dA->W * Cin * 2ull);
+    q.w_bytes = (uint32_t)(dual_rows(*dA, *dB) * Cin * 2);
+    q.y_bytes = (uint32_t)(M64 * dA->Cout * 2ull); q.y2_bytes = (uint32_t)(M64 * dB->Cout * 2ull);
+    q.M = (int)M64; q.Cout = total; q.CoutA = dA->Cout; q.Ypitch = dA->Cout; q.Ypitch2 = dB->Cout; q.Cin = Cin; q.Kpad = Cin;
+    q.Hin = dA->H; q.Win = dA->W; q.H = Ho; q.W = Wo; q.HW = Ho * Wo;
+    q.div_w = make_fastdiv((uint32_t)Wo); q.div_hw = make_fastdiv((uint32_t)q.HW);
+    q.stride = stride; q.nk = Cin / 64; q.slices = q.nk;
+    q.act = dA->act; q.act2 = dB->act; q.post_act = PCV_ACT_NONE;
+    q.nChTiles = (total + K.BM - 1) / K.BM;
+    const long long nT = (long long)((M64 + K.BP - 1) / K.BP) * q.nChTiles;
+    if (nT >= 0x7FFFFFFFll) return fail(ctx, PCV_ERR_TOO_LARGE, "pcv_conv1x1_dual_fused: too many tiles; split the batch");
+    q.nTiles = (int)nT;
+    const long long slots = block_slots(ctx, 1);
+    long long nb = slots < nT ? slots : nT;
+    nb = (nb + 7) / 8 * 8;
+    const long long per_round = 8ll * q.nChTiles;
+    if (nT > nb && nb % per_round != 0 && nb >= per_round) nb = nb / per_round * per_round;
+    if (nT > nb) {
+        const long long nCG = q.nChTiles, TP = K.BP / 16, rem = nT % nb;
+        if (rem > 0 && nb % (8 * nCG) == 0 && rem % nCG == 0 && rem * TP <= nb && ctx->use_p1r != 3 && ctx->use_p1r != -3) {
+            q.nTiles = (int)(nT - rem);
+            q.tailN = (int)rem;
+        }
+    }
+    return launch(ctx, K, (unsigned)nb, (hipStream_t)stream, q);
+}
+
 static const char* bottleneck_unsupported(const pcv_conv_desc& a, const pcv_conv_desc& b, const pcv_conv_desc& c, const pcv_conv_desc* di) {
     if (desc_stale(a) || desc_stale(b) || desc_stale(c) || (di && desc_stale(*di))) return kStaleDesc;
     if (g_bnu == 0) return "switched off (pcv_set_tuning(\"bnu\", 0))";
diff --git a/pytorchcv_amd/engine.py b/pytorchcv_amd/engine.py
--- a/pytorchcv_amd/engine.py
+++ b/pytorchcv_amd/engine.py
@@ -524,6 +524,56 @@
         _call(z.device, "fc_f32", _ptr(mean), _ptr(self._sq_w1), _ptr(self._sq_b1), _ptr(mid), z.N, d.Cin, M, mid_act)
         _call(z.device, "fc_f32", _ptr(mid), _ptr(self._sq_w2), _ptr(self._sq_b2), _ptr(gate), z.N, M, d.Cout, out_act)
         return gate
+
+
+class DualConvRunner(ConvRunner):
+    def __init__(self, ra: ConvRunner, rb: ConvRunner):
+        super(DualConvRunner, self).__init__(ra.conv, ra.bn)
+        self.ra, self.rb = ra, rb
+
+    def _sources(self):
+        return self.ra._sources() + self.rb._sources()
+
+    def _state_key(self, dtype, cpitch, da: ConvDesc, db: ConvDesc):
+        return (dtype, cpitch, da.Cin, da.Cout, db.Cout) + \
+            tuple((t.data_ptr(), t._version) if t is not None else None for t in self._sources())
+
+    def prepare(self, x: NHWC, da: ConvDesc, db: ConvDesc):
+        key = self._state_key(x.dtype, x.cpitch, da, db)
+        if key == self._key:
+            return
+        if self._foreign:
+            raise RuntimeError(
+                "this pair of convolutions' packed weights were received by parallel.broadcast_packed_state and would have to be "
+                "re-packed, but this rank's fp32 parameters are not the source's. Call parallel.broadcast_module_state(net) (or "
+                "load_state_dict on every rank) before running another configuration.")
+        self.ra.prepare(x, da)
+        self.rb.prepare(x, db)
+        nbytes = ctypes.c_size_t(0)
+        if _lib.lib().pcv_conv1x1_dual_packed_bytes(ctypes.byref(da), ctypes.byref(db), ctypes.byref(nbytes)) != 0:
+            raise _lib.PcvError(-1, "pcv_conv1x1_dual_packed_bytes refused a pair that pcv_conv1x1_dual_supported accepted")
+        packed = torch.empty((nbytes.value + 15) // 16 * 16, dtype=torch.uint8, device=x.device)
+        _call(x.device, "conv1x1_dual_pack", ctypes.byref(da), ctypes.byref(db), _ptr(self.ra.packed), _ptr(self.rb.packed), _ptr(packed))
+        scale = torch.cat((self.ra.scale, self.rb.scale)).contiguous()
+        shift = torch.cat((self.ra.shift, self.rb.shift)).contiguous()
+        self.packed, self.scale, self.shift, self._key = packed, scale, shift, key
+
+    def run(self, x: NHWC, act_a: int, act_b: int):
+        ra, rb = self.ra, self.rb
+        if not FUSE_UNITS or not isinstance(x, NHWC) or any(r.depthwise or r.pad4 is not None for r in (ra, rb)):
+            return None
+        _require_eval(ra, rb)
+        da = ra.desc(x, act_a, 0, False)
+        db = rb.desc(x, act_b, 0, False)
+        if not _lib.lib().pcv_conv1x1_dual_supported(ctypes.byref(da), ctypes.byref(db)):
+            return None
+        self.prepare(x, da, db)
+        Ho, Wo = _conv_out(da, x.H, x.W)
+        ta = torch.empty((x.N, Ho, Wo, da.Cout), dtype=x.dtype, device=x.device)
+        tb = torch.empty((x.N, Ho, Wo, db.Cout), dtype=x.dtype, device=x.device)
+        _call(x.device, "conv1x1_dual_fused", ctypes.byref(da), ctypes.byref(db), _ptr(x.t), _ptr(self.packed), _ptr(self.scale),
+              _ptr(self.shift), _ptr(ta), _ptr(tb))
+        return (NHWC(ta, x.N, Ho, Wo, ra.conv.out_channels, cpitch=da.Cout), NHWC(tb, x.N, Ho, Wo, rb.conv.out_channels, cpitch=db.Cout))
 
 
 class MixConvRunner(ConvRunner):
diff --git a/pytorchcv_amd/models/common/conv.py b/pytorchcv_amd/models/common/conv.py
--- a/pytorchcv_amd/models/common/conv.py
+++ b/pytorchcv_amd/models/common/conv.py
@@ -1,7 +1,7 @@
 
 __all__ = ['conv1x1', 'conv3x3', 'depthwise_conv3x3', 'ConvBlock', 'conv1x1_block', 'conv3x3_block', 'conv5x5_block',
            'conv7x7_block', 'dwconv_block', 'dwconv3x3_block', 'dwconv5x5_block', 'DwsConvBlock', 'dwsconv3x3_block', 'BareConv', 'PreConvBlock',
-           'pre_conv1x1_block', 'pre_conv3x3_block', 'conv_block_pair', 'conv_block_maxpool', 'mbconv_chain', 'conv_block_bottleneck']
+           'pre_conv1x1_block', 'pre_conv3x3_block', 'conv_block_pair', 'conv_block_dual', 'conv_block_maxpool', 'mbconv_chain', 'conv_block_bottleneck']
 
 import torch.nn as nn
 from .activ import lambda_relu, create_activation_layer
@@ -91,6 +91,23 @@
     return first._pcv_runner.run_pair(x, residual, engine.act_code(first.activ) if first.activate else 0,
                                       engine.act_code(post_act), second._pcv_runner,
                                       engine.act_code(second.activ) if second.activate else 0)
+
+
+def conv_block_dual(first, second, x, owner):
+    if not (type(first) is ConvBlock and type(second) is ConvBlock and isinstance(x, engine.NHWC)):
+        return None
+    if first.use_pad or second.use_pad or tuple(first.conv.stride) != tuple(second.conv.stride):
+        return None
+    for blk in (first, second):
+        if blk._pcv_runner is None:
+            blk._pcv_runner = engine.ConvRunner(blk.conv, blk.bn if blk.normalize else None, pad4=blk._pad4)
+    dual = getattr(owner, "_pcv_dual", None)
+    if dual is None or dual.ra is not first._pcv_runner or dual.rb is not second._pcv_runner:
+        dual = engine.DualConvRunner(first._pcv_runner, second._pcv_runner)
+    out = dual.run(x, engine.act_code(first.activ) if first.activate else 0, engine.act_code(second.activ) if second.activate else 0)
+    if out is not None:
+        owner._pcv_dual = dual
+    return out
 
 
 def mbconv_chain(exp_block, dw_block, proj_block, x, residual=None, post_act=None):
diff --git a/pytorchcv_amd/models/resnet.py b/pytorchcv_amd/models/resnet.py
--- a/pytorchcv_amd/models/resnet.py
+++ b/pytorchcv_amd/models/resnet.py
@@ -6,7 +6,8 @@
 import torch.nn as nn
 from .common.activ import lambda_relu
 from .common.norm import lambda_batchnorm2d
-from .common.conv import conv1x1_block, conv3x3_block, conv7x7_block, conv_block_pair, conv_block_maxpool, conv_block_bottleneck
+from .common.conv import conv1x1_block, conv3x3_block, conv7x7_block, conv_block_pair, conv_block_dual, conv_block_maxpool, \
+    conv_block_bottleneck
 from ._build import ClassifierNet, add_stages, register_variants, stage_table
 from ._tail import MaxPool2dNHWC, maybe_load_pretrained, DEFAULT_ROOT
 from .. import engine
@@ -58,6 +59,11 @@
 
     def _identity(self, a):
         return self.identity_conv(a) if self.resize_identity else a
+
+    def _conv1_and_identity(self, a):
+        if not self.resize_identity or not hasattr(self.body, "conv3"):
+            return None
+        return conv_block_dual(self.body.conv1, self.identity_conv, a, self)
 
     def _run(self, a):
         return self.body(a, residual=self._identity(a), post_act=self.activ)
@@ -89,12 +95,18 @@
             return fused, None
         if next_unit is not None and isinstance(next_unit, ResUnit) and self._stride1() and next_unit.fuses_whole(a):
             next_unit = None
+        identity = None
+        if conv1_out is None:
+            dual = self._conv1_and_identity(a)
+            if dual is not None:
+                conv1_out, identity = dual
         y = body.conv2(conv1_out if conv1_out is not None else body.conv1(a))
-        if next_unit is not None and self.resize_identity:
+        if next_unit is not None and self.resize_identity and identity is None:
             pair = conv_block_pair(body.conv3, y, None, self.activ, next_unit.body.conv1, id_block=self.identity_conv, x0=a)
             if pair is not None:
                 return pair
-        identity = self._identity(a)
+        if identity is None:
+            identity = self._identity(a)
         if next_unit is not None:
             pair = conv_block_pair(body.conv3, y, identity, self.activ, next_unit.body.conv1)
             if pair is not None:
diff --git a/pytorchcv_amd/models/resnext.py b/pytorchcv_amd/models/resnext.py
--- a/pytorchcv_amd/models/resnext.py
+++ b/pytorchcv_amd/models/resnext.py
@@ -34,8 +34,12 @@
     pcv_chainable = True
 
     def run_chained(self, a, conv1_out=None, next_unit=None):
-        identity = self._identity(a)
         body = self.body
+        dual = self._conv1_and_identity(a) if conv1_out is None else None
+        if dual is not None:
+            conv1_out, identity = dual
+        else:
+            identity = self._identity(a)
         y = body.conv2(conv1_out if conv1_out is not None else body.conv1(a))
         if next_unit is not None:
             pair = conv_block_pair(body.conv3, y, identity, self.activ, next_unit.body.conv1)
diff --git a/pytorchcv_amd/models/seresnet.py b/pytorchcv_amd/models/seresnet.py
--- a/pytorchcv_amd/models/seresnet.py
+++ b/pytorchcv_amd/models/seresnet.py
@@ -22,8 +22,12 @@
     pcv_chainable = True
 
     def run_chained(self, a, conv1_out=None, next_unit=None):
-        identity = self._identity(a)
         body = self.body
+        dual = self._conv1_and_identity(a) if conv1_out is None else None
+        if dual is not None:
+            conv1_out, identity = dual
+        else:
+            identity = self._identity(a)
         if not hasattr(body, "conv3"):
             return self.se(body(a), residual=identity, post_act=self.activ), None
         z = body.conv2(conv1_out if conv1_out is not None else body.conv1(a))
```

After: 97540 images/sec (median of 2 runs). No clear change (+0.7%).
